# afiaka87/clip-guided-diffusion

Hardware: AMD Instinct MI355X
Metric: diffusion steps/sec (UNet+CLIP+grad) at 256x256 cutn=16 (higher is better)
Workload: dtype bf16x3 (split-bf16 MFMA, fp32 accumulate, fp32 storage); 1 GPU; BASELINE configs[1]: 256x256 class-cond UNet (554M), respace 250, cutn 16, batch 1/GPU, CLIP ViT-B/32, cgs 1000 tv 150 range 50, randomize_class, p_sample; global_batch=1, world_size_checked=1, collectives=none (single process)

## Files before the change

### clip-guided-diffusion_amd/csrc/capi.hip

```cpp
#include "../../include/cgd_mi355x.h"
#include "common.h"
#include "guidance.h"
#include "kernels.h"
#include "mfma_stage.h"

#define S(stream) ((hipStream_t)(stream))

extern "C" {

const char* cgd_version(void) { return "cgd_mi355x 0.1 (gfx950)"; }

int cgd_ctx_create(cgd_ctx** out, int device) {
  if (!out) return -3;
  cgd_ctx* ctx = new cgd_ctx();
  ctx->device = device;
  int prev = -1;
  (void)hipGetDevice(&prev);
  if (hipSetDevice(device) != hipSuccess) {
    delete ctx;
    return -1;
  }
  struct Restore {
    int d;
    ~Restore() {
      if (d >= 0) (void)hipSetDevice(d);
    }
  } restore{prev};
  hipDeviceProp_t prop;
  if (hipGetDeviceProperties(&prop, device) == hipSuccess) {
    ctx->num_cu = prop.multiProcessorCount;
    if (std::string(prop.gcnArchName).find("gfx950") == std::string::npos) {
      fprintf(stderr, "cgd_mi355x: device %d is %s, this library is built for gfx950 only\n", device, prop.gcnArchName);
      delete ctx;
      return -4;
    }
  }
  if (const char* e = getenv("CGD_DEFER")) ctx->defer_mode = atoi(e);
  if (const char* e = getenv("CGD_HGEMM_VAR")) ctx->hgemm_var = atoi(e);
  if (const char* e = getenv("CGD_HGEMM_EPI")) ctx->hgemm_epi = atoi(e);
  if (const char* e = getenv("CGD_TILE_ORDER")) ctx->tile_order = atoi(e);
  if (const char* e = getenv("CGD_FUSE_GN")) sscanf(e, "%d,%d,%d,%d", &ctx->fuse_gn, &ctx->fuse_gn_max_m, &ctx->fuse_gn_min_m, &ctx->fuse_gn_skip_m);
  if (const char* e = getenv("CGD_FUSE_ACT")) ctx->fuse_act = atoi(e);
  if (const char* e = getenv("CGD_HCONV_W8")) ctx->hconv_w8 = atoi(e);
  if (const char* e = getenv("CGD_ATTN_X3")) ctx->attn_x3 = atoi(e);
  if (const char* e = getenv("CGD_ATTN_FLASH")) ctx->attn_flash = atoi(e);
  int wino_env_mode = -1;
  if (const char* e = getenv("CGD_WINO")) sscanf(e, "%d,%d", &wino_env_mode, &ctx->wino_min_m);
  if (const char* e = getenv("CGD_THIN")) ctx->thin_direct = atoi(e);
  if (const char* e = getenv("CGD_GEMV")) ctx->gemv_mode = atoi(e);
  if (const char* e = getenv("CGD_WINO_NC")) ctx->wino_nc = atoi(e);
  ctx->wino_nc_default = ctx->wino_nc;
  if (wino_env_mode >= 0) cgd_apply_wino_mode(ctx, wino_env_mode);
  if (const char* e = getenv("CGD_GN_EPI")) ctx->gn_epi = atoi(e);
  if (const char* e = getenv("CGD_HGEMM_KG")) ctx->hgemm_kg = atoi(e) < 0 || atoi(e) > 2 ? 1 : atoi(e);
  if (const char* e = getenv("CGD_HGEMM_TM96")) ctx->hgemm_tm96 = atoi(e);
  if (const char* e = getenv("CGD_NT")) ctx->weight_nt = atoi(e);
  if (const char* e = getenv("CGD_KGEMM")) sscanf(e, "%d,%d,%d,%d,%d", &ctx->kgemm_mode, &ctx->kgemm_max_m, &ctx->kgemm_var, &ctx->kgemm_big_m, &ctx->kgemm_big_n);
  if (const char* e = getenv("CGD_EMBED_FUSE")) ctx->embed_fuse = atoi(e);
  if (const char* e = getenv("CGD_KCONV")) sscanf(e, "%d,%d,%d,%d,%d,%d,%d", &ctx->kconv_mode, &ctx->kconv_max_m, &ctx->kconv_min_chunks, &ctx->kconv_tw8, &ctx->kconv_slots, &ctx->kconv_ring, &ctx->kconv_th16);
  if (const char* e = getenv("CGD_HCONV_SPLIT")) sscanf(e, "%d,%d", &ctx->hconv_slots, &ctx->hconv_min_chunks);
  if (ctx->kconv_min_chunks < 1) ctx->kconv_min_chunks = 1;
  if (ctx->hconv_min_chunks < 1) ctx->hconv_min_chunks = 1;
  if (const char* e = getenv("CGD_HCONV_SMALL")) sscanf(e, "%d,%d,%d", &ctx->hconv_small_m, &ctx->hconv_small_slots, &ctx->hconv_small_min_chunks);
  ctx->ws_bytes = (size_t)256 << 20;
  if (hipMalloc((void**)&ctx->ws, ctx->ws_bytes) != hipSuccess) {
    delete ctx;
    return -1;
  }
  *out = ctx;
  return 0;
}

void cgd_ctx_destroy(cgd_ctx* ctx) {
  if (!ctx) return;
  {
  DeviceScope dev_scope(ctx);
  if (ctx->ws) (void)hipFree(ctx->ws);
  cgd_frag_cache_clear(ctx);
  cgd_chanstats_clear(ctx);
  if (ctx->frag_tmp) (void)hipFree(ctx->frag_tmp);
  for (ProfRec& r : ctx->prof_recs) {
    (void)hipEventDestroy(r.a);
    (void)hipEventDestroy(r.b);
  }
  for (hipEvent_t e : ctx->prof_pool) (void)hipEventDestroy(e);
  }
  delete ctx;
}

const char* cgd_last_error(cgd_ctx* ctx) { return ctx ? ctx->err.c_str() : "null context"; }

#define CGD_NEED_CTX(ctx)   \
  if (!(ctx)) return -3;    \
  DeviceScope dev_scope__(ctx)

int cgd_set_precision(cgd_ctx* ctx, int mode) {
  CGD_NEED_CTX(ctx);
  if (mode < 0 || mode > 2) CGD_FAIL(ctx, "precision mode must be 0 (f32), 1 (bf16x3) or 2 (bf16)");
  ctx->precision = mode;
  return 0;
}
int cgd_get_precision(cgd_ctx* ctx) { return ctx ? ctx->precision : -3; }
int64_t cgd_ctx_device_allocs(cgd_ctx* ctx) { return ctx ? (int64_t)ctx->device_allocs : -3; }

int cgd_set_tiles(cgd_ctx* ctx, int large, int small) {
  CGD_NEED_CTX(ctx);
  ctx->tile_huge = large >= 1000000 ? large / 1000000 : ctx->tile_huge;
  ctx->tile_large = large % 1000000;
  ctx->tile_small = small;
  return 0;
}

int cgd_set_hgemm(cgd_ctx* ctx, int mode, int min_m, int min_chunks) {
  CGD_NEED_CTX(ctx);
  ctx->hgemm_mode = mode;
  if (min_m > 0) ctx->hgemm_min_m = min_m;
  if (min_chunks > 0) ctx->hgemm_min_chunks = min_chunks;
  return 0;
}

int cgd_profile(cgd_ctx* ctx, int enable) {
  CGD_NEED_CTX(ctx);
  ctx->prof_on = enable != 0;
  return 0;
}

int cgd_profile_read(cgd_ctx* ctx, double* out) {
  CGD_NEED_CTX(ctx);
  if (!out) CGD_FAIL(ctx, "cgd_profile_read: out is null");
  CGD_HIP(ctx, hipDeviceSynchronize());
  CGD_TRY(cgd_prof_fold(ctx, 0));
  for (int k = 0; k < CGD_PROF_KINDS; ++k) {
    out[3 * k + 0] = ctx->prof_ms[k];
    out[3 * k + 1] = ctx->prof_flops[k];
    out[3 * k + 2] = ctx->prof_n[k];
    ctx->prof_ms[k] = ctx->prof_flops[k] = ctx->prof_n[k] = 0.0;
  }
  return 0;
}

int cgd_profile_kinds(void) { return CGD_PROF_KINDS; }

int cgd_launch_counts(unsigned long long* out2) {
  if (!out2) return -3;
  out2[0] = g_cgd_launches.load(std::memory_order_relaxed);
  out2[1] = g_cgd_reduces.load(std::memory_order_relaxed);
  return 0;
}
}

int cgd_prof_fold(cgd_ctx* ctx, size_t keep_last) {
  CGD_NEED_CTX(ctx);
  if (ctx->prof_recs.size() <= keep_last) return 0;
  const size_t n = ctx->prof_recs.size() - keep_last;
  for (size_t i = 0; i < n; ++i) {
    ProfRec& r = ctx->prof_recs[i];
    float t = 0.f;
    CGD_HIP(ctx, hipEventSynchronize(r.b));
    CGD_HIP(ctx, hipEventElapsedTime(&t, r.a, r.b));
    ctx->prof_ms[r.kind] += t;
    ctx->prof_flops[r.kind] += r.flops;
    ctx->prof_n[r.kind] += 1.0;
    ctx->prof_pool.push_back(r.a);
    ctx->prof_pool.push_back(r.b);
  }
  ctx->prof_recs.erase(ctx->prof_recs.begin(), ctx->prof_recs.begin() + n);
  return 0;
}

int cgd_prof_begin(cgd_ctx* ctx, ProfRec* pr, int kind, double work, hipStream_t s) {
  pr->live = false;
  if (!ctx->prof_on) return 0;
  if (ctx->prof_recs.size() >= 3072) CGD_TRY(cgd_prof_fold(ctx, 1024));
  for (hipEvent_t* e : {&pr->a, &pr->b}) {
    if (!ctx->prof_pool.empty()) {
      *e = ctx->prof_pool.back();
      ctx->prof_pool.pop_back();
    } else {
      CGD_HIP(ctx, hipEventCreate(e));
    }
  }
  pr->flops = work;
  pr->kind = kind;
  pr->live = true;
  CGD_HIP(ctx, hipEventRecord(pr->a, s));
  return 0;
}
int cgd_prof_stamp(cgd_ctx* ctx, ProfRec* pr, hipStream_t s) {
  if (pr->live) CGD_HIP(ctx, hipEventRecord(pr->b, s));
  return 0;
}
void cgd_prof_push(cgd_ctx* ctx, ProfRec* pr) {
  if (pr->live) ctx->prof_recs.push_back(*pr);
  pr->live = false;
}

// ... 195 lines not shown
  GemmParams p;
  p.A = A; p.lda = lda; p.B = Wt; p.ldb = ldw; p.C = dx; p.ldc = lddx;
  p.M = Bn * HW; p.N = N; p.K = K; p.force_tile = 513; p.no_split = 1;
  p.gnf_x = x; p.gnf_ldx = ldx; p.gnf_dz = dz; p.gnf_lddz = lddz; p.gnf_add = add; p.gnf_ldadd = ldadd;
  p.gnf_coef = coef; p.gnf_bcoef = bcoef; p.gnf_hw = HW;
  return p;
}
int cgd_op_gemm_gn_bwd_accepts(int precision, int lda, int ldw, int lddx, int ldx, int lddz, int ldadd, int x_misalign, int Bn, int HW, int N, int K) {
  if (Bn <= 0 || HW <= 0 || (long)Bn * HW > 0x7fffffffL) return 0;
  cgd_ctx ctx;
  ctx.precision = precision;
  float* const dummy = (float*)(uintptr_t)4096;
  const float* xs = (const float*)((uintptr_t)4096 + (uintptr_t)x_misalign);
  return cgd_gemm_fuses_gnb(&ctx, gemm_gn_bwd_params(dummy, lda, dummy, ldw, dummy, lddx, xs, ldx, dummy, lddz, ldadd ? dummy : nullptr, ldadd, dummy, dummy,
                                                     Bn, HW, N, K)) ? 1 : 0;
}
int cgd_op_gemm_gn_bwd(cgd_ctx* ctx, const float* A, int lda, const float* Wt, int ldw, float* dx, int lddx, const float* x, int ldx,
                       const float* dz, int lddz, const float* add, int ldadd, const float* coef, const float* bcoef, int Bn, int HW, int N, int K,
                       void* stream) {
  CGD_NEED_CTX(ctx);
  if (Bn <= 0 || HW <= 0 || (long)Bn * HW > 0x7fffffffL) CGD_FAIL(ctx, "cgd_op_gemm_gn_bwd: bad sample count / rows per sample");
  const GemmParams p = gemm_gn_bwd_params(A, lda, Wt, ldw, dx, lddx, x, ldx, dz, lddz, add, ldadd, coef, bcoef, Bn, HW, N, K);
  if (!x || !dz || !coef || !bcoef) CGD_FAIL(ctx, "cgd_op_gemm_gn_bwd: x, dz, coef and bcoef are required");
  if (!cgd_gemm_fuses_gnb(ctx, p))
    CGD_FAIL(ctx, "cgd_op_gemm_gn_bwd: needs a bf16x3 context, K a multiple of 64, N of 32, row strides multiples of 4, 16-byte aligned operands and "
                  "samples of a multiple of 128 rows (or one sample)");
  return cgd_launch_gemm(ctx, p, S(stream));
}
int cgd_op_pack_conv3x3_frag(cgd_ctx* ctx, const float* w, float* out, int Co, int Ci, int dgrad, void* stream) {
  CGD_NEED_CTX(ctx);
  return cgd_pack_conv3x3_frag(ctx, w, out, Co, Ci, dgrad, S(stream));
}
int cgd_op_pack_conv3x3_wino(cgd_ctx* ctx, const float* w, float* out, int Co, int Ci, int dgrad, void* stream) {
  CGD_NEED_CTX(ctx);
  return cgd_pack_conv3x3_wino(ctx, w, out, Co, Ci, dgrad, S(stream));
}
int cgd_op_conv3x3_wino(cgd_ctx* ctx, const float* x, int ldx, const float* w_wino, float* y, int ldy, const float* bias, const float* R,
                        int ldr, const float* gn_ab, int Bn, int H, int W, int Cin, int Cout, int ups, void* stream) {
  CGD_NEED_CTX(ctx);
  GemmParams p;
  p.Bwk = w_wino;
  p.bwk_prec = ctx->precision;
  p.A = x; p.lda = ldx; p.B = x ; p.ldb = 9 * Cin; p.C = y; p.ldc = ldy;
  p.bias = bias; p.R = R; p.ldr = ldr; p.gn_ab = gn_ab;
  p.M = Bn * H * W; p.N = Cout; p.conv = 1; p.H = H; p.W = W; p.Cin = Cin; p.ups = ups; p.force_tile = 515;
  return cgd_launch_gemm(ctx, p, S(stream));
}
int cgd_op_conv3x3_wino_ex(cgd_ctx* ctx, const float* x, int ldx, const float* w_wino, float* y, int ldy, const float* bias, const float* R,
                           int ldr, const float* gn_ab, int Bn, int H, int W, int Cin, int Cout, int ups, int stats, const float* gnb_x,
                           int gnb_ldx, const float* gnb_scratch, void* stream) {
  CGD_NEED_CTX(ctx);
  GemmParams p;
  p.Bwk = w_wino;
  p.bwk_prec = ctx->precision;
  p.A = x; p.lda = ldx; p.B = x ; p.ldb = 9 * Cin; p.C = y; p.ldc = ldy;
  p.bias = bias; p.R = R; p.ldr = ldr; p.gn_ab = gn_ab;
  p.M = Bn * H * W; p.N = Cout; p.conv = 1; p.H = H; p.W = W; p.Cin = Cin; p.ups = ups; p.force_tile = 515;
  p.stats = stats;
  if (gnb_x && gnb_scratch) {
    p.gnb_x = gnb_x; p.gnb_ldx = gnb_ldx; p.gnb_coef = cgd_gn_coef(gnb_scratch, Bn, H * W, Cout); p.gnb_act = 1;
  }
  return cgd_launch_gemm(ctx, p, S(stream));
}
}
namespace {
__global__ __launch_bounds__(256) void mfma_peak_kernel(float* out, int iters) {
  cgd_f32x16 acc[4];
  for (int a = 0; a < 4; ++a)
    for (int e = 0; e < 16; ++e) acc[a][e] = 0.f;
  cgd_bf16x8 x, y;
  for (int e = 0; e < 8; ++e) {
    x[e] = (__bf16)(float)((threadIdx.x * 7 + e) % 13 - 6);
    y[e] = (__bf16)(0.001f * (float)((threadIdx.x * 3 + e) % 11 - 5));
  }
  for (int it = 0; it < iters; ++it) {
#pragma unroll
    for (int r = 0; r < 3; ++r)
#pragma unroll
      for (int a = 0; a < 4; ++a) acc[a] = __builtin_amdgcn_mfma_f32_32x32x16_bf16(x, y, acc[a], 0, 0, 0);
  }
  float s = 0.f;
  for (int a = 0; a < 4; ++a)
    for (int e = 0; e < 16; ++e) s += acc[a][e];
  if (s == 12345.678f) out[blockIdx.x * blockDim.x + threadIdx.x] = s;
}
}
extern "C" {
int cgd_op_mfma_peak(cgd_ctx* ctx, int iters, double* flop_out, void* stream) {
  CGD_NEED_CTX(ctx);
  if (iters <= 0) CGD_FAIL(ctx, "cgd_op_mfma_peak: iters must be positive");
  const int blocks = ctx->num_cu;
  if (flop_out) *flop_out = 2.0 * 32 * 32 * 16 * 12.0 * iters * blocks * 4;
  CGD_LAUNCH(mfma_peak_kernel, dim3(blocks), dim3(256), 0, S(stream), ctx->ws, iters);
  CGD_HIP(ctx, hipGetLastError());
  return 0;
}
int cgd_op_new_pass(cgd_ctx* ctx) {
  CGD_NEED_CTX(ctx);
  ++ctx->stats_serial;
  return 0;
}
int64_t cgd_op_gn_stats_offset(int B, int HW, int C) { return (int64_t)cgd_gn_stats_offset(B, HW, C); }
int64_t cgd_op_gn_record_merges(cgd_ctx* ctx) { return ctx ? (int64_t)ctx->gn_record_merges : -3; }
int cgd_op_gn_records(cgd_ctx* ctx, const float* y, int ldy, int64_t rows, int C, int kind, float* out, int64_t cap, int* pixels, void* stream) {
  CGD_NEED_CTX(ctx);
  if (!out || !pixels) return -3;
  *pixels = 0;
  ChanSrc cs;
  if (!(cgd_chanstats_find(ctx, y, ldy, (long)rows, C, S(stream), &cs, kind) && cs.n0 == C)) return 0;
  const int64_t n = rows / cs.c0 * C * 2;
  if (n > cap) CGD_FAIL(ctx, "cgd_op_gn_records: out is too small");
  CGD_HIP(ctx, hipMemcpyAsync(out, cs.p0, (size_t)n * sizeof(float), hipMemcpyDeviceToDevice, S(stream)));
  *pixels = cs.c0;
  return 0;
}
int cgd_set_wino(cgd_ctx* ctx, int mode, int min_m) {
  CGD_NEED_CTX(ctx);
  if (mode < 0 || (mode > 3 && mode != 5)) CGD_FAIL(ctx, "cgd_set_wino: mode must be 0, 1, 2, 3 or 5");
  cgd_apply_wino_mode(ctx, mode);
  if (min_m > 0) ctx->wino_min_m = min_m;
  return 0;
}
int cgd_set_hconv(cgd_ctx* ctx, int mode, int min_m) {
  CGD_NEED_CTX(ctx);
  ctx->hconv_mode = mode & 15;
  ctx->hconv_var = mode >> 4;
  ctx->hconv_min_m = min_m;
  return 0;
}
int cgd_op_conv3x3(cgd_ctx* ctx, const float* x, int ldx, const float* w, const float* w_frag, float* y, int ldy, const float* bias,
                   const float* R, int ldr, int Bn, int H, int W, int Cin, int Cout, int ups, int force_tile, int splitk, void* stream) {
  CGD_NEED_CTX(ctx);
  GemmParams p;
  p.Bpk = w_frag;
  p.A = x; p.lda = ldx; p.B = w; p.ldb = 9 * Cin; p.C = y; p.ldc = ldy; p.bias = bias; p.R = R; p.ldr = ldr;
  p.M = Bn * H * W; p.N = Cout; p.conv = 1; p.H = H; p.W = W; p.Cin = Cin; p.ups = ups; p.force_tile = force_tile; p.splitk = splitk;
  return cgd_launch_gemm(ctx, p, S(stream));
}
int cgd_op_conv3x3_ex(cgd_ctx* ctx, const float* x, int ldx, const float* w, const float* w_frag, float* y, int ldy, const float* bias,
                      const float* R, int ldr, const float* gn_ab, int Bn, int H, int W, int Cin, int Cout, int ups, int force_tile, int splitk,
                      int defer, int stats, const float* gnb_x, int gnb_ldx, const float* gnb_scratch, void* stream) {
  CGD_NEED_CTX(ctx);
  GemmParams p;
  p.Bpk = w_frag;
  p.A = x; p.lda = ldx; p.B = w; p.ldb = 9 * Cin; p.C = y; p.ldc = ldy; p.bias = bias; p.R = R; p.ldr = ldr; p.gn_ab = gn_ab;
  p.M = Bn * H * W; p.N = Cout; p.conv = 1; p.H = H; p.W = W; p.Cin = Cin; p.ups = ups; p.force_tile = force_tile; p.splitk = splitk;
  p.defer = defer;
  p.stats = stats;
  if (gnb_x && gnb_scratch) {
    p.gnb_x = gnb_x; p.gnb_ldx = gnb_ldx; p.gnb_coef = cgd_gn_coef(gnb_scratch, Bn, H * W, Cout); p.gnb_act = 1;
  }
  return cgd_launch_gemm(ctx, p, S(stream));
}
int cgd_op_conv_in(cgd_ctx* ctx, const float* x, const float* w, const float* bias, float* y, int Bn, int H, int W, int Cin, int Cout,
                   void* stream) {
  CGD_NEED_CTX(ctx);
  return cgd_launch_conv_in(ctx, x, w, bias, y, Bn, H, W, Cin, Cout, S(stream));
}
int cgd_op_sr_stem(cgd_ctx* ctx, const float* x, const float* low, int B_low, int h, int w, const float* wpacked, const float* bias, float* y,
                   int ldy, int B, int H, int W, int Cout, void* stream) {
  CGD_NEED_CTX(ctx);
  return cgd_launch_sr_stem(ctx, x, low, B_low, h, w, wpacked, bias, y, ldy, B, H, W, Cout, S(stream));
}
int cgd_op_conv_thin_out(cgd_ctx* ctx, const float* x, int ldx, const float* w, const float* bias, float* y, int Bn, int H, int W,
                         int Cin, int Cout, void* stream) {
  CGD_NEED_CTX(ctx);
  return cgd_launch_conv_thin_out(ctx, x, ldx, w, bias, y, Bn, H, W, Cin, Cout, S(stream));
}
int64_t cgd_op_gn_scratch_floats(int B, int HW, int C) { return (int64_t)cgd_gn_scratch_floats(B, HW, C); }
int cgd_op_gn_fwd(cgd_ctx* ctx, const float* x, int ldx, float* y, int ldy, int B, int HW, int C, const float* gamma, const float* beta,
                  const float* film, int act, float eps, float* scratch, void* stream) {
  CGD_NEED_CTX(ctx);
  return cgd_launch_gn_fwd(ctx, x, ldx, y, ldy, B, HW, C, gamma, beta, film, 2 * C, act, eps, scratch, S(stream));
}
int cgd_op_gn_bwd(cgd_ctx* ctx, const float* x, int ldx, const float* dz, int lddz, float* dx, int lddx, const float* add, int ldadd,
                  int B, int HW, int C, int act, float* scratch, void* stream) {
  CGD_NEED_CTX(ctx);
  return cgd_launch_gn_bwd(ctx, x, ldx, dz, lddz, dx, lddx, add, ldadd, B, HW, C, act, scratch, S(stream));
}
int cgd_op_ln_fwd(cgd_ctx* ctx, const float* x, float* y, int rows, int C, const float* gamma, const float* beta, float eps, float* stats,
                  void* stream) {
  CGD_NEED_CTX(ctx);
  return cgd_launch_ln_fwd(ctx, x, C, y, C, rows, C, gamma, beta, eps, stats, S(stream));
}
int cgd_op_ln_bwd(cgd_ctx* ctx, const float* x, const float* dy, float* dx, int rows, int C, const float* gamma, const float* stats,
                  void* stream) {
  CGD_NEED_CTX(ctx);
  return cgd_launch_ln_bwd(ctx, x, C, dy, C, dx, C, nullptr, 0, rows, C, gamma, stats, S(stream));
}
int cgd_op_pool2x2(cgd_ctx* ctx, const float* in, float* out, int B, int Ho, int Wo, int C, float scale, void* stream) {
  CGD_NEED_CTX(ctx);
  return cgd_launch_pool2x2(ctx, in, C, out, C, nullptr, 0, B, Ho, Wo, C, scale, S(stream));
}
int cgd_op_upsample2x(cgd_ctx* ctx, const float* in, float* out, int B, int Ho, int Wo, int C, float scale, void* stream) {
  CGD_NEED_CTX(ctx);
  return cgd_launch_upsample2x(ctx, in, C, out, C, nullptr, 0, B, Ho, Wo, C, scale, S(stream));
}
int cgd_op_act(cgd_ctx* ctx, const float* x, const float* dy, float* out, int64_t n, int act, void* stream) {
  CGD_NEED_CTX(ctx);
  if (dy) return cgd_launch_act_bwd(ctx, x, dy, out, n, act, S(stream));
  return cgd_launch_act_fwd(ctx, x, out, n, act, S(stream));
}
int64_t cgd_op_attn_buf_floats(int nb, int heads, int T, int d, int which) {
  const int64_t Tp = attn_tp(T), C = (int64_t)heads * d;
  switch (which) {
    case 0: return (int64_t)nb * 3 * C * Tp;
    case 4: return (int64_t)nb * C * Tp;
    default: return (int64_t)nb * heads * T * Tp;
  }
}
int cgd_op_attn_fwd(cgd_ctx* ctx, const float* qkv, float* out, int nb, int heads, int T, int d, int legacy, float* bufs[5],
                    void* stream) {
  CGD_NEED_CTX(ctx);
  AttnShape sh{nb, heads, T, d, heads * d, legacy};
  AttnBufs bf{bufs[0], bufs[1], bufs[2], bufs[3], bufs[4]};
  return cgd_attn_fwd(ctx, sh, qkv, 3 * heads * d, out, heads * d, bf, S(stream));
}
int cgd_op_attn_fwd_causal(cgd_ctx* ctx, const float* qkv, float* out, int nb, int heads, int T, int d, float* bufs[5], void* stream) {
  CGD_NEED_CTX(ctx);
  AttnShape sh{nb, heads, T, d, heads * d, 0, 1};
  AttnBufs bf{bufs[0], bufs[1], bufs[2], bufs[3], bufs[4]};
  return cgd_attn_fwd(ctx, sh, qkv, 3 * heads * d, out, heads * d, bf, S(stream));
}
int cgd_op_attn_bwd(cgd_ctx* ctx, const float* qkv, const float* dout, float* dqkv, int nb, int heads, int T, int d, int legacy,
                    float* bufs[5], void* stream) {
  CGD_NEED_CTX(ctx);
  AttnShape sh{nb, heads, T, d, heads * d, legacy};
  AttnBufs bf{bufs[0], bufs[1], bufs[2], bufs[3], bufs[4]};
  return cgd_attn_bwd(ctx, sh, qkv, 3 * heads * d, dout, heads * d, dqkv, 3 * heads * d, bf, S(stream));
}
}

void cgd_apply_wino_mode(cgd_ctx* ctx, int mode) {
  if (mode < 0 || (mode > 3 && mode != 5)) mode = 1;
  ctx->wino_mode = mode == 5 ? 3 : mode;
  ctx->wino_nc = mode == 5 ? 3 : ctx->wino_nc_default;
}
```

### clip-guided-diffusion_amd/csrc/common.h

```cpp
#pragma once
#include <hip/hip_runtime.h>
#include <stdint.h>
#include <stdio.h>
#include <atomic>
#include <string>
#include <utility>
#include <vector>

inline std::atomic<unsigned long long> g_cgd_launches{0}, g_cgd_reduces{0};
#define CGD_LAUNCH(...)                                          \
  do {                                                           \
    g_cgd_launches.fetch_add(1, std::memory_order_relaxed);      \
    hipLaunchKernelGGL(__VA_ARGS__);                             \
  } while (0)

enum { CGD_PREC_F32 = 0, CGD_PREC_BF16X3 = 1, CGD_PREC_BF16 = 2 };

enum { CGD_PROF_GEMM = 0, CGD_PROF_HCONV = 1, CGD_PROF_GN = 2, CGD_PROF_WCONV = 3, CGD_PROF_KCONV = 4, CGD_PROF_WCONV_GNB = 5, CGD_PROF_KINDS = 6 };

struct ProfRec {
  hipEvent_t a = nullptr, b = nullptr;
  double flops = 0.0;
  int kind = 0;
  bool live = false;
};

struct SplitSrc {
  const float* ws = nullptr;
  const float* bias = nullptr;
  const float* R = nullptr;
  long stride = 0;
  int n = 0;
  int N = 0, ldr = 0;
  float alpha = 1.f;
};
struct PendingReduce {
  bool valid = false;
  SplitSrc src;
  float* C = nullptr;
  int ldc = 0, M = 0;
  hipStream_t stream = nullptr;
};

struct ChanStatsEntry {
  const float* C = nullptr;
  int ldc = 0, N = 0;
  long M = 0;
  float* buf = nullptr;
  size_t cap = 0;
  hipStream_t stream = nullptr;
  unsigned long long serial = 0;
  int kind = 0;
  int cnt = 128;
};
struct ChanSrc {
  const float* p0 = nullptr;
  const float* p1 = nullptr;
  int n0 = 0, n1 = 0;
  int c0 = 128, c1 = 128;
};

struct FragEntry {
  const float* w;
  int N, K, ldw;
  void* packed;
};

struct cgd_ctx {
  int device = 0;
  int precision = CGD_PREC_BF16X3;
  std::string err;
  float* ws = nullptr;
  size_t ws_bytes = 0;
  int num_cu = 256;
  int tile_huge = 1256, tile_large = 128, tile_small = 64;
  int hconv_var = 0;
  int hconv_small_m = 0, hconv_small_slots = 512, hconv_small_min_chunks = 2;
  int hconv_slots = 0, hconv_min_chunks = 4;
  int hconv_w8 = 0;
  int hconv_mode = 1, hconv_min_m = 256;
  int embed_fuse = 1;
  int gemv_mode = 1;
  int thin_direct = 1;
  int kconv_tw8 = 1;
  int kconv_th16 = 0;
  int kconv_ring = 2;
  int kconv_slots = 0;
  int kconv_mode = 1, kconv_max_m = 1024, kconv_min_chunks = 4;
  int wino_mode = 1, wino_min_m = 16384;
  int wino_nc_default = 0;
  int wino_nc = 0;
  int attn_x3 = 1;
  int attn_flash = 3;
  int fuse_act = 1;
  int fuse_gn_skip_m = 0;
  int fuse_gn_max_m = 1 << 30, fuse_gn_min_m = 4096;
  int fuse_gn = 1;
  int tile_order = 0;
  int hgemm_epi = 1;
  int hgemm_kg = 1;
  int weight_nt = 0;
  int kgemm_var = 0;
  int kgemm_big_m = 0, kgemm_big_n = 0;
  int kgemm_mode = 2, kgemm_max_m = 256;
  int hgemm_tm96 = 1;
  int hgemm_var = 1;
  int hgemm_mode = 1, hgemm_min_m = 64, hgemm_min_chunks = 4;
  PendingReduce pending;
  int defer_mode = 2;
  std::vector<ChanStatsEntry> chanstats;
  std::vector<float*> chanstats_retired;
  unsigned long long stats_serial = 1;
  unsigned long long device_allocs = 0;
  unsigned long long gn_record_merges = 0;
  bool last_wconv_bstat = false;
  int gn_epi = 3;
  std::vector<std::pair<const float*, int>> attn_fwd_path;
  std::vector<FragEntry> frag_cache;
  void* frag_tmp = nullptr;
  size_t frag_tmp_bytes = 0;
  bool prof_on = false;
  std::vector<ProfRec> prof_recs;
  std::vector<hipEvent_t> prof_pool;
  double prof_ms[CGD_PROF_KINDS] = {}, prof_flops[CGD_PROF_KINDS] = {}, prof_n[CGD_PROF_KINDS] = {};
};

struct ExactScope {
  cgd_ctx* ctx;
  int saved;
  explicit ExactScope(cgd_ctx* c) : ctx(c), saved(c->precision) { c->precision = CGD_PREC_F32; }
  ~ExactScope() { ctx->precision = saved; }
};

struct DeviceScope {
  int prev = -1;
  bool switched = false;
  explicit DeviceScope(const cgd_ctx* c) {
    if (c && hipGetDevice(&prev) == hipSuccess && prev != c->device) switched = hipSetDevice(c->device) == hipSuccess;
  }
  ~DeviceScope() {
    if (switched) (void)hipSetDevice(prev);
  }
};

int cgd_prof_fold(cgd_ctx* ctx, size_t keep_last);
int cgd_prof_begin(cgd_ctx* ctx, ProfRec* pr, int kind, double work, hipStream_t s);
int cgd_prof_stamp(cgd_ctx* ctx, ProfRec* pr, hipStream_t s);
void cgd_prof_push(cgd_ctx* ctx, ProfRec* pr);

#define CGD_HIP(ctx, expr)                                                                   \
  do {                                                                                       \
    hipError_t e__ = (expr);                                                                 \
    if (e__ != hipSuccess) {                                                                 \
      (ctx)->err = std::string(#expr) + ": " + hipGetErrorString(e__) + " @" + __FILE__ + ":" + \
                   std::to_string(__LINE__);                                                 \
      return -1;                                                                             \
    }                                                                                        \
  } while (0)

#define CGD_FAIL(ctx, msg)        \
  do {                            \
    (ctx)->err = (msg);           \
    return -2;                    \
  } while (0)

#define CGD_TRY(expr)             \
  do {                            \
    int r__ = (expr);             \
    if (r__ != 0) return r__;     \
  } while (0)

static inline int cdiv(long a, long b) { return (int)((a + b - 1) / b); }
static inline int grid_for(long n, int cap = 1024) {
  const int g = cdiv(n, 256);
  return g < cap ? g : cap;
}

struct GemmParams {
  const float* A = nullptr;
  const float* B = nullptr;
  float* C = nullptr;
  const float* bias = nullptr;
  const float* R = nullptr;
  int M = 0, N = 0, K = 0;
  int lda = 0, ldb = 0, ldc = 0, ldr = 0;
  int nbatch = 1, bdiv = 1;
  long sA1 = 0, sA2 = 0, sB1 = 0, sB2 = 0, sC1 = 0, sC2 = 0, sR1 = 0, sR2 = 0;
  float alpha = 1.f;
  int conv = 0, H = 0, W = 0, Cin = 0, ups = 0;
  int splitk = 1;
  int no_split = 0;
  float* ws = nullptr;
  int force_tile = 0;
  int weight = 0;
  const void* Bpk = nullptr;
  const void* Bwk = nullptr;
  int bwk_prec = CGD_PREC_BF16X3;
  float* act_out = nullptr;
  const float* act_in = nullptr;
  int ld_act = 0, act = 0;
  int skip_group = 0;
  const float* gn_ab = nullptr;
  const float* gnb_x = nullptr;
  const float* gnb_coef = nullptr;
  int gnb_ldx = 0, gnb_act = 0;
  int stats = 0;
  int a_mode = 0;
  const float* a_t = nullptr;
  const float* a_freqs = nullptr;
  const float* a_table = nullptr;
  const int64_t* a_idx = nullptr;
  const float* gnf_x = nullptr;
  const float* gnf_dz = nullptr;
  const float* gnf_add = nullptr;
  const float* gnf_coef = nullptr;
  const float* gnf_bcoef = nullptr;
  int gnf_ldx = 0, gnf_lddz = 0, gnf_ldadd = 0, gnf_hw = 0;
  int defer = 0;
};

float* cgd_chanstats_register(cgd_ctx* ctx, const float* C, int ldc, int N, long M, hipStream_t s, int kind = 0, int cnt = 128);
bool cgd_chanstats_find(cgd_ctx* ctx, const float* x, int ldx, long M, int Cn, hipStream_t s, ChanSrc* out, int kind = 0);
void cgd_chanstats_clear(cgd_ctx* ctx);
void cgd_chanstats_invalidate(cgd_ctx* ctx, const float* C, long rows, int ld, int cols);
bool cgd_gn_merges_records(int HW);
void cgd_apply_wino_mode(cgd_ctx* ctx, int mode);

int cgd_flush_pending(cgd_ctx* ctx, hipStream_t s);
bool cgd_take_pending(cgd_ctx* ctx, const float* x, long rows, int cols, int ldx, hipStream_t s, SplitSrc* out);
static inline int cgd_sync_pending(cgd_ctx* ctx, hipStream_t s) { return ctx->pending.valid ? cgd_flush_pending(ctx, s) : 0; }

size_t cgd_hconv_packed_floats(int Co, int Ci);
int cgd_pack_conv3x3_frag(cgd_ctx* ctx, const float* w , float* out, int Co, int Ci, int dgrad, hipStream_t s);
bool cgd_hconv_supported(const cgd_ctx* ctx, const GemmParams& p);
int cgd_hconv_tile_m(const cgd_ctx* ctx, const GemmParams& p);
long cgd_hconv_tiles_m(const cgd_ctx* ctx, const GemmParams& p);
int cgd_launch_hconv(cgd_ctx* ctx, const GemmParams& p, hipStream_t s);

size_t cgd_wconv_packed_floats(int Co, int Ci);
int cgd_pack_conv3x3_wino(cgd_ctx* ctx, const float* w , float* out, int Co, int Ci, int dgrad, hipStream_t s);
bool cgd_wconv_supported(const cgd_ctx* ctx, const GemmParams& p);
int cgd_wconv_nb(const cgd_ctx* ctx, const GemmParams& p);
int cgd_wconv_nc(const cgd_ctx* ctx, const GemmParams& p);
long cgd_wconv_tiles_m(const cgd_ctx* ctx, const GemmParams& p);
int cgd_launch_wconv(cgd_ctx* ctx, const GemmParams& p, hipStream_t s);

bool cgd_kconv_supported(const cgd_ctx* ctx, const GemmParams& p);
long cgd_kconv_tiles_m(const cgd_ctx* ctx, const GemmParams& p);
int cgd_kconv_tw(const cgd_ctx* ctx, const GemmParams& p);
int cgd_kconv_th(const cgd_ctx* ctx, const GemmParams& p);
int cgd_launch_kconv(cgd_ctx* ctx, const GemmParams& p, hipStream_t s);

bool cgd_hgemm_supported(const cgd_ctx* ctx, const GemmParams& p);
int cgd_hgemm_tile_m(const cgd_ctx* ctx, const GemmParams& p);
int cgd_hgemm_tiles(const cgd_ctx* ctx, const GemmParams& p);
int cgd_hgemm_chunks(const GemmParams& p);
int cgd_launch_hgemm(cgd_ctx* ctx, const GemmParams& p, hipStream_t s);
void cgd_frag_cache_clear(cgd_ctx* ctx);
bool cgd_kgemm_supported(const cgd_ctx* ctx, const GemmParams& p);
bool cgd_kgemm_capable(const cgd_ctx* ctx, const GemmParams& p);
void cgd_frag_cache_evict(cgd_ctx* ctx, const float* w);
int cgd_kgemm_tiles(const cgd_ctx* ctx, const GemmParams& p);
int cgd_launch_kgemm(cgd_ctx* ctx, const GemmParams& p, hipStream_t s);

int cgd_launch_gemm(cgd_ctx* ctx, GemmParams p, hipStream_t s);
bool cgd_conv_uses_hconv(cgd_ctx* ctx, GemmParams p);
bool cgd_gemm_fuses_act(cgd_ctx* ctx, GemmParams p);
bool cgd_gemm_fuses_gnb(cgd_ctx* ctx, GemmParams p);
bool cgd_conv_takes_gnb(cgd_ctx* ctx, GemmParams p);
bool cgd_wconv_takes_gnb(const cgd_ctx* ctx, const GemmParams& g);
bool cgd_hconv_takes_gnb(const cgd_ctx* ctx, const GemmParams& g);
bool cgd_gemm_is_gemv(cgd_ctx* ctx, GemmParams p);

int cgd_launch_conv_in(cgd_ctx* ctx, const float* x_nchw, const float* w , const float* bias,
                       float* y_nhwc, int Bn, int H, int W, int Cin, int Cout, hipStream_t s, int ldy = 0 );
int cgd_launch_conv_thin_out(cgd_ctx* ctx, const float* x_nhwc, int ldx, const float* w , const float* bias,
                             float* y_nchw, int Bn, int H, int W, int Cin, int Cout, hipStream_t s);
int cgd_launch_sr_stem(cgd_ctx* ctx, const float* x_nchw, const float* low , int B_low, int lh, int lw,
                       const float* w , const float* bias, float* y_nhwc, int ldy , int Bn, int H,
                       int W, int Cout, hipStream_t s);
```

### clip-guided-diffusion_amd/csrc/hconv.hip

```cpp
#include "common.h"
#include "mfma_stage.h"

namespace {

constexpr int HB_M = 256, HB_N = 128, HPH = 40;

struct HConvParams {
  const float* A;
  const uint4* Bp;
  float* C;
  const float* bias;
  const float* R;
  float* ws;
  int lda, ldc, ldr;
  int M, N, H, W, Cin, ups, splitk;
  float alpha;
  const float* gn;
  float* stat;
  float* bstat;
  const float* bx;
  const float* bcoef;
  int ldbx, bact;
  int nmajor;
};

constexpr int PW2 = 18;
constexpr int HRS = 768;
constexpr int NPASS2 = 6;


template <int MODE, int TH, int NJ, bool GN>
__global__ __launch_bounds__(TH == 4 ? 256 : TH * 32) void hconv2_kernel(const float* __restrict__ Ag, const uint4* __restrict__ Bg, float* Cg,
                                                         const float* __restrict__ biasg, const float* Rg, float* __restrict__ wsg,
                                                         const float* __restrict__ gng, const HConvParams p) {
  constexpr int NPL = MODE == 1 ? 2 : 1;
  constexpr int NP2 = (TH + 2) * PW2;
  constexpr int PLANE = (TH + 2) * HRS;
  constexpr int NI = TH == 4 ? 2 : 4 / NJ;
  constexpr int NT = TH == 4 ? 256 : TH * 32;
  constexpr int RPP = NT / 8;
  constexpr int NPASS = TH == 4 ? 4 : NPASS2;
  static_assert(TH != 4 || NJ == 1, "the 4-row tile runs 64 pixels x 32 channels per wavefront");
  static_assert(NPASS * RPP >= NP2, "staging passes must cover the patch");
  __shared__ __attribute__((aligned(16))) __bf16 lds[2 * NPL * PLANE];
  const int tid = threadIdx.x, lane = tid & 63, wave = tid >> 6;
  const int wm = NJ == 2 ? wave >> 1 : wave >> 2, wn = NJ == 2 ? wave & 1 : wave & 3;
  const int l31 = lane & 31, hh = lane >> 5;

  const int ntn = (p.N + HB_N - 1) / HB_N;
  int bid = blockIdx.x;
  {
    const int nt = gridDim.x, q = nt >> 3, r = nt & 7, xcd = bid & 7, idx = bid >> 3;
    bid = (xcd < r ? xcd * (q + 1) : r * (q + 1) + (xcd - r) * q) + idx;
  }
  const int ntm = gridDim.x / ntn;
  const int mt = p.nmajor ? bid % ntm : bid / ntn, n0 = (p.nmajor ? bid / ntm : bid % ntn) * HB_N;
  const int tpr = (p.W + 15) >> 4, tpi = (p.H / TH) * tpr;
  const int img = mt / tpi, trem = mt - img * tpi;
  const int y0 = (trem / tpr) * TH, x0 = (trem % tpr) << 4;
  const int HW = p.H * p.W;
  const int Hs = p.ups ? (p.H >> 1) : p.H, Ws = p.ups ? (p.W >> 1) : p.W;
  const float* __restrict__ Aimg = Ag + (long)img * Hs * Ws * p.lda;

  const int c4 = tid & 7;
  int poff[NPASS], soff[NPASS];
#pragma unroll
  for (int j = 0; j < NPASS; ++j) {
    const int prow = (tid >> 3) + RPP * j;
    poff[j] = -2;
    soff[j] = PW2 * HPH + c4 * 4;
    if (prow < NP2) {
      const int py = prow / PW2, px = prow - py * PW2;
      soff[j] = py * HRS + px * HPH + c4 * 4;
      int yy = y0 + py - 1, xx = x0 + px - 1;
      const bool inb = (unsigned)yy < (unsigned)p.H && (unsigned)xx < (unsigned)p.W;
      if (p.ups) {
        yy >>= 1;
        xx >>= 1;
      }
      poff[j] = inb ? (yy * Ws + xx) * p.lda + c4 * 4 : -1;
    }
  }
  int poffb[NPASS];
#pragma unroll
  for (int j = 0; j < NPASS; ++j) poffb[j] = poff[j] >= 0 ? poff[j] * 4 : CGD_OOB;
  int fro[NI];
  long mrow[NI];
#pragma unroll
  for (int i = 0; i < NI; ++i) {
    const int pix = wm * (NI * 32) + i * 32 + l31;
    const int ty = pix >> 4, tx = pix & 15;
    fro[i] = ty * HRS + tx * HPH + hh * 8;
    mrow[i] = x0 + tx < p.W ? (long)img * HW + (long)(y0 + ty) * p.W + x0 + tx : -1L;
  }

  const int nchunk = p.Cin >> 5;
  int c0 = 0, c1 = nchunk;
  if (p.splitk > 1) {
    const int per = (nchunk + p.splitk - 1) / p.splitk;
    c0 = blockIdx.z * per;
    c1 = min(nchunk, c0 + per);
  }
  const int nb0 = (n0 >> 5) + wn * NJ;
  const int nbN = p.N >> 5;
  const long bstride_nb = (long)nchunk * 9 * 4 * 64;
  const int nbc = nb0 < nbN ? nb0 : nbN - 1;
  (void)nbc;
  const int nb0_s = (n0 >> 5) + __builtin_amdgcn_readfirstlane(wn) * NJ;
  const uint4* __restrict__ Bwb = Bg + (long)(nb0_s < nbN ? nb0_s : nbN - 1) * bstride_nb;
  const int bj1_b = (nb0_s + 1 < nbN) ? (int)(bstride_nb * 16) : 0;
  (void)bj1_b;

  cgd_f32x16 acc[NI][NJ];
#pragma unroll
  for (int i = 0; i < NI; ++i)
#pragma unroll
    for (int j = 0; j < NJ; ++j)
#pragma unroll
      for (int e = 0; e < 16; ++e) acc[i][j][e] = 0.f;

  constexpr bool SPLITQ = !(GN && NJ == 2 && TH == 8);
  cgd_f32x4 pr[NPASS];
  cgd_f32x4 ga[GN ? 2 : 1];
  const cgd_f32x4 z4 = cgd_f32x4{0.f, 0.f, 0.f, 0.f};
  const float* __restrict__ gnimg = GN ? gng + ((long)img * p.Cin + c4 * 4) * 2 : nullptr;

#define PATCH_LOAD2(CH, WANT)                                                                                      \
  {                                                                                                                \
    if constexpr (GN) {                                                                                            \
      const int cg_ = (WANT) < 0 ? (CH) : (CH) - 1;                                                                \
      ga[0] = *(const cgd_f32x4*)(gnimg + cg_ * 64);                                                               \
      ga[1] = *(const cgd_f32x4*)(gnimg + cg_ * 64 + 4);                                                           \
    }                                                                                                              \
    _Pragma("unroll") for (int j = 0; j < NPASS; ++j)                                                             \
        pr[j] = __builtin_bit_cast(cgd_f32x4, cgd_buf_load16_if(Aimg, 0x80000000u, (WANT), poffb[j], (CH) * 128)); \
  }
#define PATCH_STORE2(DSTB, J0, J1)                                                                                                            \
  {                                                                                                                                           \
    _Pragma("unroll") for (int j = J0; j < J1; ++j) {                                                                                         \
      cgd_f32x4 v = pr[j];                                                                                                                    \
      if constexpr (GN)                                                                                                                       \
        v = cgd_f32x4{cgd_silu_affine(v.x, ga[0].x, ga[0].y), cgd_silu_affine(v.y, ga[0].z, ga[0].w), cgd_silu_affine(v.z, ga[1].x, ga[1].y), \
                  cgd_silu_affine(v.w, ga[1].z, ga[1].w)};                                                                                    \
      if constexpr (GN) v = poff[j] >= 0 ? v : z4;                           \
      if constexpr (MODE == 1 && SPLITQ) {                                                                                                    \
        cgd_bf16x4 hi, lo;                                                                                                                    \
        cgd_split_quad(v, hi, lo);                                                                                                            \
        *(cgd_bf16x4*)&(DSTB)[soff[j]] = hi;                                                                                                  \
        *(cgd_bf16x4*)&(DSTB)[PLANE + soff[j]] = lo;                                                                                          \
      } else {                                                                                                                                \
        const cgd_bf16x4 hi = cgd_to_bf16x4(v);                                                                                               \
        *(cgd_bf16x4*)&(DSTB)[soff[j]] = hi;                                                                                                  \
        if constexpr (MODE == 1) *(cgd_bf16x4*)&(DSTB)[PLANE + soff[j]] = cgd_to_bf16x4(cgd_residual4(v, hi));                                \
      }                                                                                                                                       \
    }                                                                                                                                         \
  }
#define A_LOAD2(DST, SRCB, TAP, KS)                                                          \
  {                                                                                          \
    constexpr int o_ = ((TAP) / 3) * HRS + ((TAP) % 3) * HPH + (KS) * 16;                    \
    _Pragma("unroll") for (int i = 0; i < NI; ++i) {                                         \
      DST[i][0] = *(const cgd_bf16x8*)&(SRCB)[fro[i] + o_];                                  \
      if constexpr (MODE == 1) DST[i][1] = *(const cgd_bf16x8*)&(SRCB)[PLANE + fro[i] + o_]; \
    }                                                                                        \
  }
#define B_LOAD2(DST, BASE, WANT, TAP, KS)                                                                                                         \
  {                                                                                                                                               \
    const int so_ = ((BASE) * (9 * 4 * 64) + ((TAP) * 4 + (KS) * 2) * 64) * 16;                                                                   \
    DST[0][0] = __builtin_bit_cast(uint4, cgd_buf_load16_if(Bwb, 0xffffffffu, (WANT), lane * 16, so_));                                           \
    if constexpr (MODE == 1) DST[0][1] = __builtin_bit_cast(uint4, cgd_buf_load16_if(Bwb, 0xffffffffu, (WANT), lane * 16 + 1024, so_));           \
    if constexpr (NJ == 2) {                                                                                                                      \
      DST[1][0] = __builtin_bit_cast(uint4, cgd_buf_load16_if(Bwb, 0xffffffffu, (WANT), lane * 16, so_ + bj1_b));                                 \
      if constexpr (MODE == 1) DST[1][1] = __builtin_bit_cast(uint4, cgd_buf_load16_if(Bwb, 0xffffffffu, (WANT), lane * 16 + 1024, so_ + bj1_b)); \
    }                                                                                                                                             \
  }
#define MFMA12(AQ, BQ)                                                                                                                 \
  {                                                                                                                                    \
    if constexpr (MODE == 1) {                                                                                                         \
      _Pragma("unroll") for (int i = 0; i < NI; ++i) _Pragma("unroll") for (int j = 0; j < NJ; ++j)                                    \
          acc[i][j] = __builtin_amdgcn_mfma_f32_32x32x16_bf16(__builtin_bit_cast(cgd_bf16x8, BQ[j][0]), AQ[i][1], acc[i][j], 0, 0, 0); \
      _Pragma("unroll") for (int i = 0; i < NI; ++i) _Pragma("unroll") for (int j = 0; j < NJ; ++j)                                    \
          acc[i][j] = __builtin_amdgcn_mfma_f32_32x32x16_bf16(__builtin_bit_cast(cgd_bf16x8, BQ[j][1]), AQ[i][0], acc[i][j], 0, 0, 0); \
    }                                                                                                                                  \
    _Pragma("unroll") for (int i = 0; i < NI; ++i) _Pragma("unroll") for (int j = 0; j < NJ; ++j)                                      \
        acc[i][j] = __builtin_amdgcn_mfma_f32_32x32x16_bf16(__builtin_bit_cast(cgd_bf16x8, BQ[j][0]), AQ[i][0], acc[i][j], 0, 0, 0);   \
  }

  constexpr int RING = TH == 4 ? 9 : (TH == 8 || NJ == 1) ? 6 : 3, DIST = RING - 1;
  cgd_bf16x8 af[2][NI][NPL];
  uint4 bq[RING][NJ][NPL];
  if (c0 < c1) {
    PATCH_LOAD2(c0, -1);
#pragma unroll
    for (int q = 0; q < DIST; ++q) B_LOAD2(bq[q], c0, -1, q >> 1, q & 1);
    PATCH_STORE2(lds, 0, NPASS);
  }
  __syncthreads();
  for (int c = c0; c < c1; ++c) {
    const bool more = c + 1 < c1;
    const __bf16* cur = lds + ((c - c0) & 1) * (NPL * PLANE);
    __bf16* nxt = lds + (((c - c0) & 1) ^ 1) * (NPL * PLANE);
    const int want = c + 1 - c1;
    PATCH_LOAD2(c + 1, want);
    (void)more;
    A_LOAD2(af[0], cur, 0, 0);
#pragma unroll
    for (int q = 0; q < 18; ++q) {
      if (q + 1 < 18) {
        switch (q + 1) {
#define CASE_A(Q) case Q: A_LOAD2(af[(Q) & 1], cur, (Q) >> 1, (Q) & 1); break;
          CASE_A(1) CASE_A(2) CASE_A(3) CASE_A(4) CASE_A(5) CASE_A(6) CASE_A(7) CASE_A(8) CASE_A(9)
          CASE_A(10) CASE_A(11) CASE_A(12) CASE_A(13) CASE_A(14) CASE_A(15) CASE_A(16) CASE_A(17)
#undef CASE_A
        }
      }
      {
        const int q2 = (q + DIST) % 18;
        if (q + DIST < 18) { B_LOAD2(bq[(q + DIST) % RING], c, -1, q2 >> 1, q2 & 1); }
        else { B_LOAD2(bq[(q + DIST) % RING], c + 1, want, q2 >> 1, q2 & 1); }
      }
      MFMA12(af[q & 1], bq[q % RING]);
      if (q >= 6 && q < 6 + NPASS) PATCH_STORE2(nxt, q - 6, q - 5);
#pragma unroll
      for (int r = 0; r < (TH == 4 ? 6 : 12); ++r) {
        __builtin_amdgcn_sched_group_barrier(0x008, 1, 0);
        if constexpr (TH == 4) {
          if (r < 4) __builtin_amdgcn_sched_group_barrier(0x100, 1, 0);
          else __builtin_amdgcn_sched_group_barrier(0x020, 1, 0);
          __builtin_amdgcn_sched_group_barrier(0x002, 3, 0);
        } else if constexpr (NJ == 2) {
          if (r % 3 == 0) __builtin_amdgcn_sched_group_barrier(0x100, 1, 0);
          if (r % 3 == 1) __builtin_amdgcn_sched_group_barrier(0x020, 1, 0);
        } else {
          if (r % 3 != 2) __builtin_amdgcn_sched_group_barrier(0x100, 1, 0);
          if (r % 6 == 2) __builtin_amdgcn_sched_group_barrier(0x020, 1, 0);
        }
        __builtin_amdgcn_sched_group_barrier(0x002, 3, 0);
        if (r % 3 == 2) __builtin_amdgcn_sched_group_barrier(0x200, 1, 0);
      }
      __builtin_amdgcn_sched_barrier(0);
    }
    __syncthreads();
  }
#undef PATCH_LOAD2
#undef PATCH_STORE2
#undef A_LOAD2
#undef B_LOAD2
#undef MFMA12

  if (p.splitk > 1) {
    float* __restrict__ ws = wsg + (long)blockIdx.z * p.M * p.N;
#pragma unroll
    for (int i = 0; i < NI; ++i)
#pragma unroll
      for (int j = 0; j < NJ; ++j) {
        const int cb0 = (nb0 + j) * 32;
        if (cb0 < p.N && mrow[i] >= 0) {
#pragma unroll
          for (int g = 0; g < 4; ++g)
            *(cgd_f32x4*)&ws[mrow[i] * p.N + cb0 + 8 * g + 4 * hh] =
                cgd_f32x4{acc[i][j][4 * g], acc[i][j][4 * g + 1], acc[i][j][4 * g + 2], acc[i][j][4 * g + 3]};
        }
      }
    return;
  }
  if constexpr (TH == 4) {
    const int cb0 = nb0 * 32;
    if (cb0 >= p.N) return;
    cgd_f32x4 o[NI][4];
#pragma unroll
    for (int i = 0; i < NI; ++i) {
      cgd_f32x4 rv[4];
      if (Rg && mrow[i] >= 0) {
#pragma unroll
        for (int g = 0; g < 4; ++g) rv[g] = *(const cgd_f32x4*)&Rg[mrow[i] * p.ldr + cb0 + 8 * g + 4 * hh];
      }
#pragma unroll
      for (int g = 0; g < 4; ++g) {
        const int col = cb0 + 8 * g + 4 * hh;
        o[i][g] = cgd_f32x4{acc[i][0][4 * g], acc[i][0][4 * g + 1], acc[i][0][4 * g + 2], acc[i][0][4 * g + 3]} * p.alpha;
        if (biasg) o[i][g] += cgd_f32x4{biasg[col], biasg[col + 1], biasg[col + 2], biasg[col + 3]};
        if (Rg && mrow[i] >= 0) o[i][g] += rv[g];
        if (mrow[i] >= 0) *(cgd_f32x4*)&Cg[mrow[i] * p.ldc + col] = o[i][g];
      }
    }
    if (p.stat) {
#pragma unroll
      for (int g = 0; g < 4; ++g) {
        cgd_f32x4 kk, s1 = z4, s2 = z4;
#pragma unroll
        for (int e = 0; e < 4; ++e) kk[e] = __shfl(o[0][g][e], lane & 32, 64);
#pragma unroll
        for (int i = 0; i < NI; ++i) {
          const cgd_f32x4 d = o[i][g] - kk;
          s1 += d;
          s2 += d * d;
        }
#pragma unroll
        for (int off = 1; off < 32; off <<= 1)
#pragma unroll
          for (int e = 0; e < 4; ++e) {
            s1[e] += __shfl_xor(s1[e], off, 64);
            s2[e] += __shfl_xor(s2[e], off, 64);
          }
        if (l31 == 0) {
          float* so = p.stat + ((long)mt * p.N + cb0 + 8 * g + 4 * hh) * 2;
          const cgd_f32x4 mean = kk + s1 * (1.f / 64.f), m2 = s2 - s1 * s1 * (1.f / 64.f);
          *(cgd_f32x4*)so = cgd_f32x4{mean[0], m2[0], mean[1], m2[1]};
          *(cgd_f32x4*)(so + 4) = cgd_f32x4{mean[2], m2[2], mean[3], m2[3]};
        }
      }
    }
    if (p.bstat) {
#pragma unroll
      for (int g = 0; g < 4; ++g) {
        const int col = cb0 + 8 * g + 4 * hh;
        cgd_f32x4 cfa, cfb, cfg_, cfm, q1 = z4, q2 = z4;
#pragma unroll
        for (int e = 0; e < 4; ++e) {
          const cgd_f32x4 c_ = *(const cgd_f32x4*)(p.bcoef + ((long)img * p.N + col + e) * 4);
          cfa[e] = c_[0]; cfb[e] = c_[1]; cfg_[e] = c_[2]; cfm[e] = c_[3];
        }
#pragma unroll
        for (int i = 0; i < NI; ++i) {
          const cgd_f32x4 xv = *(const cgd_f32x4*)&p.bx[mrow[i] * p.ldbx + col];
          cgd_f32x4 d = o[i][g];
          if (p.bact) {
            const cgd_f32x4 uu = xv * cfa + cfb;
            cgd_f32x4 sg;
#pragma unroll
            for (int e = 0; e < 4; ++e) sg[e] = cgd_sigmoid_rcp(uu[e]);
            d *= sg * (1.f + uu * (1.f - sg));
          }
          q1 += d;
          q2 += d * (xv - cfm);
        }
#pragma unroll
        for (int off = 1; off < 32; off <<= 1)
#pragma unroll
          for (int e = 0; e < 4; ++e) {
            q1[e] += __shfl_xor(q1[e], off, 64);
            q2[e] += __shfl_xor(q2[e], off, 64);
          }
        if (l31 == 0) {
          float* so = p.bstat + ((long)mt * p.N + col) * 2;
          *(cgd_f32x4*)so = cgd_f32x4{cfg_[0] * q1[0], cfg_[0] * q2[0], cfg_[1] * q1[1], cfg_[1] * q2[1]};
          *(cgd_f32x4*)(so + 4) = cgd_f32x4{cfg_[2] * q1[2], cfg_[2] * q2[2], cfg_[3] * q1[3], cfg_[3] * q2[3]};
        }
      }
    }
    return;
  }
#pragma unroll
  for (int i = 0; i < NI; ++i)
#pragma unroll
    for (int j = 0; j < NJ; ++j) {
      const int cb0 = (nb0 + j) * 32;
      if (cb0 >= p.N || mrow[i] < 0) continue;
      cgd_f32x4 rv[4];
      if (Rg) {
#pragma unroll
        for (int g = 0; g < 4; ++g) rv[g] = *(const cgd_f32x4*)&Rg[mrow[i] * p.ldr + cb0 + 8 * g + 4 * hh];
      }
#pragma unroll
      for (int g = 0; g < 4; ++g) {
        const int col = cb0 + 8 * g + 4 * hh;
        cgd_f32x4 o = cgd_f32x4{acc[i][j][4 * g], acc[i][j][4 * g + 1], acc[i][j][4 * g + 2], acc[i][j][4 * g + 3]} * p.alpha;
        if (biasg) o += cgd_f32x4{biasg[col], biasg[col + 1], biasg[col + 2], biasg[col + 3]};
        if (Rg) o += rv[g];
        *(cgd_f32x4*)&Cg[mrow[i] * p.ldc + col] = o;
      }
    }
}

__global__ __launch_bounds__(256) void pack_frag_kernel(const float* __restrict__ w, __bf16* __restrict__ out, int Co, int Ci, int dgrad) {
  const int N = dgrad ? Ci : Co, K = dgrad ? Co : Ci;
  const int nchunk = K >> 5;
  const long total = (long)N * K * 9;
  for (long t = (long)blockIdx.x * blockDim.x + threadIdx.x; t < total; t += (long)gridDim.x * blockDim.x) {
    const int e = (int)(t & 7);
    long u = t >> 3;
    const int lane = (int)(u & 63);
    u >>= 6;
    const int ks = (int)(u & 1);
    u >>= 1;
    const int tap = (int)(u % 9);
    u /= 9;
    const int chunk = (int)(u % nchunk), nb = (int)(u / nchunk);
    const int n = nb * 32 + (lane & 31), k = chunk * 32 + ks * 16 + (lane >> 5) * 8 + e;
    const int ky = tap / 3, kx = tap % 3;
    const float v = dgrad ? w[(((long)k * Ci + n) * 3 + (2 - ky)) * 3 + (2 - kx)] : w[(((long)n * Ci + k) * 3 + ky) * 3 + kx];
    const __bf16 hi = (__bf16)v;
    const __bf16 lo = (__bf16)(v - (float)hi);
    const long blk = ((((long)nb * nchunk + chunk) * 9 + tap) * 2 + ks) * 2;
    out[(blk + 0) * 512 + lane * 8 + e] = hi;
    out[(blk + 1) * 512 + lane * 8 + e] = lo;
  }
}

}

size_t cgd_hconv_packed_floats(int Co, int Ci) { return (size_t)Co * Ci * 9; }

int cgd_pack_conv3x3_frag(cgd_ctx* ctx, const float* w, float* out, int Co, int Ci, int dgrad, hipStream_t s) {
  if ((Co & 31) || (Ci & 31)) CGD_FAIL(ctx, "pack_conv3x3_frag: channels must be multiples of 32");
  const long total = (long)Co * Ci * 9;
  CGD_LAUNCH(pack_frag_kernel, dim3((int)std::min<long>(cdiv(total, 256), 4096)), dim3(256), 0, s, w, (__bf16*)out, Co, Ci, dgrad);
  CGD_HIP(ctx, hipGetLastError());
  return 0;
}

bool cgd_hconv_supported(const cgd_ctx* ctx, const GemmParams& p) {
  if (!p.conv || !p.Bpk || ctx->precision == CGD_PREC_F32 || p.nbatch != 1) return false;
  if ((p.Cin & 31) || (p.N & 31) || (p.lda & 3)) return false;
  if (p.H <= 0 || p.W <= 0 || (p.H & 7) || ((p.W & 15) && p.W != 8)) return false;
  if ((p.H & 15) && ((ctx->hconv_var & 1) || ((ctx->hconv_var & 2) && p.M < 16384))) return false;
  if (p.ups && ((p.H | p.W) & 1)) return false;
  if ((p.ldc & 3) || ((uintptr_t)p.C & 15)) return false;
  if (p.R && ((p.ldr & 3) || ((uintptr_t)p.R & 15))) return false;
  if ((long)p.H * p.W * p.lda * 4 >= (1L << 31)) return false;
  return true;
}

static bool hconv_records_fwd(const cgd_ctx* ctx, const GemmParams& g) {
  return g.stats && (ctx->gn_epi & 1) && g.H > 0 && g.W > 0 && !(g.W & 15) && cgd_gn_merges_records(g.H * g.W);
}
static bool hconv_records_bwd(const cgd_ctx* ctx, const GemmParams& g) {
  return g.gnb_x && g.gnb_coef && (ctx->gn_epi & 2) && g.H > 0 && g.W > 0 && !(g.W & 15) && cgd_gn_merges_records(g.H * g.W) && !(g.gnb_ldx & 3) &&
         !((uintptr_t)g.gnb_x & 15) && !g.stats && !g.R;
}

int cgd_hconv_tile_m(const cgd_ctx* ctx, const GemmParams& p) {
  if (ctx->precision == CGD_PREC_BF16X3 && !(p.N & 127) && p.splitk <= 1 && p.H > 0 && p.W > 0 && !(p.H & 3) && p.M % (p.H * p.W) == 0) {
    if (ctx->hconv_var & 8) return 64;
    if (ctx->hconv_var == 0 && !(p.W & 15) && (hconv_records_fwd(ctx, p) || hconv_records_bwd(ctx, p))) {
      const long t64 = (long)(p.M / (p.H * p.W)) * (p.H / 4) * (p.W >> 4) * (p.N >> 7);
      if (t64 / 2 < ctx->num_cu && t64 >= ctx->num_cu) return 64;
    }
  }
  if (ctx->hconv_var & 1) return HB_M;
  if ((ctx->hconv_var & 2) && p.M < 16384) return HB_M;
  return 128;
}

bool cgd_hconv_takes_gnb(const cgd_ctx* ctx, const GemmParams& g) { return g.splitk <= 1 && cgd_hconv_tile_m(ctx, g) == 64 && hconv_records_bwd(ctx, g); }

long cgd_hconv_tiles_m(const cgd_ctx* ctx, const GemmParams& p) {
  const int th = cgd_hconv_tile_m(ctx, p) / 16;
  return (long)(p.M / (p.H * p.W)) * (p.H / th) * cdiv(p.W, 16);
}

int cgd_launch_hconv(cgd_ctx* ctx, const GemmParams& g, hipStream_t s) {
  HConvParams p;
  p.A = g.A; p.Bp = (const uint4*)g.Bpk; p.C = g.C; p.bias = g.bias; p.R = g.R; p.ws = g.ws;
  p.lda = g.lda; p.ldc = g.ldc; p.ldr = g.ldr;
  p.M = g.M; p.N = g.N; p.H = g.H; p.W = g.W; p.Cin = g.Cin; p.ups = g.ups; p.splitk = g.splitk; p.alpha = g.alpha;
  p.gn = g.gn_ab;
  p.stat = p.bstat = nullptr; p.bx = g.gnb_x; p.bcoef = g.gnb_coef; p.ldbx = g.gnb_ldx; p.bact = g.gnb_act;
  p.nmajor = (ctx->tile_order == 1 || (ctx->tile_order == 0 && 9L * g.N >= g.M)) ? 1 : 0;
  const int tm = cgd_hconv_tile_m(ctx, g);
  if (tm == 64 && g.splitk <= 1) {
    if (hconv_records_fwd(ctx, g)) p.stat = cgd_chanstats_register(ctx, g.C, g.ldc, g.N, g.M, s, 0, 64);
    if (hconv_records_bwd(ctx, g)) p.bstat = cgd_chanstats_register(ctx, g.C, g.ldc, g.N, g.M, s, 1, 64);
  }
  dim3 grid((int)cgd_hconv_tiles_m(ctx, g) * cdiv(g.N, HB_N), 1, g.splitk > 1 ? g.splitk : 1);
#define HC2_LAUNCH(M_, TH_, NJ_)                                                                                                   \
  {                                                                                                                                \
    if (p.gn)                                                                                                                      \
      CGD_LAUNCH((hconv2_kernel<M_, TH_, NJ_, true>), grid, dim3(TH_ == 4 ? 256 : TH_ * 32), 0, s, p.A, p.Bp, p.C, p.bias, p.R, p.ws, p.gn, p);  \
    else                                                                                                                           \
      CGD_LAUNCH((hconv2_kernel<M_, TH_, NJ_, false>), grid, dim3(TH_ == 4 ? 256 : TH_ * 32), 0, s, p.A, p.Bp, p.C, p.bias, p.R, p.ws, p.gn, p); \
  }
#define HC2_LAUNCH_T(M_, NJ_)  \
  {                            \
    if (tm == 128)             \
      HC2_LAUNCH(M_, 8, NJ_)   \
    else                       \
      HC2_LAUNCH(M_, 16, NJ_)  \
  }
  const bool nj1 = (ctx->hconv_var & 4) == 0;
  if (tm == 64) {
    HC2_LAUNCH(1, 4, 1)
  } else if (ctx->precision == CGD_PREC_BF16X3) {
    if (nj1) HC2_LAUNCH_T(1, 1) else HC2_LAUNCH_T(1, 2)
  } else {
    if (nj1) HC2_LAUNCH_T(2, 1) else HC2_LAUNCH_T(2, 2)
  }
#undef HC2_LAUNCH_T
#undef HC2_LAUNCH
  return 0;
}
```

### clip-guided-diffusion_amd/csrc/unet.hip

```cpp
#include <cmath>
#include <memory>

#include "../../include/cgd_mi355x.h"
#include "net.h"

namespace {

__global__ void pack_conv3x3_kernel(const float* __restrict__ w, float* __restrict__ wf, float* __restrict__ wd, int Co, int Ci) {
  const long total = (long)Co * Ci * 9;
  for (long i = (long)blockIdx.x * blockDim.x + threadIdx.x; i < total; i += (long)gridDim.x * blockDim.x) {
    const int kx = (int)(i % 3);
    long t = i / 3;
    const int ky = (int)(t % 3);
    t /= 3;
    const int ci = (int)(t % Ci), co = (int)(t / Ci);
    const float v = w[i];
    if (wf) wf[((long)co * 9 + ky * 3 + kx) * Ci + ci] = v;
    if (wd) wd[((long)ci * 9 + (2 - ky) * 3 + (2 - kx)) * Co + co] = v;
  }
}

}

int cgd_pack_conv3x3(cgd_ctx* ctx, const float* w, float* wf, float* wd, int Co, int Ci, hipStream_t s) {
  const long total = (long)Co * Ci * 9;
  CGD_LAUNCH(pack_conv3x3_kernel, dim3((int)std::min<long>(cdiv(total, 256), 4096)), dim3(256), 0, s, w, wf, wd, Co, Ci);
  CGD_HIP(ctx, hipGetLastError());
  return 0;
}

int cgd_plan_gemm(cgd_ctx* ctx, GemmParams& p, int* tile_out, int* kernel_out);

namespace {

struct UNet;

struct Module {
  TV dst;
  virtual ~Module() {}
  virtual int fwd(UNet& u, TV x, int B, int& H, int& W, TV* out, hipStream_t s) = 0;
  virtual int bwd(UNet& u, TV dout, TV* din, hipStream_t s) = 0;
};

struct ResBlock : Module {
  std::string pre;
  int cin = 0, cout = 0;
  bool up = false, down = false, skip_conv = false;
  long emb_off = 0;
  float *g1 = 0, *b1 = 0, *cw1f = 0, *cw1d = 0, *cb1 = 0, *g2 = 0, *b2 = 0, *cw2f = 0, *cw2d = 0, *cb2 = 0, *skw = 0, *skwT = 0,
        *skb = 0;
  float *cw1fp = 0, *cw1dp = 0, *cw2fp = 0, *cw2dp = 0;
  float *cw1wp = 0, *cw1wd = 0, *cw2wp = 0, *cw2wd = 0;
  int wino_prec = CGD_PREC_BF16X3;
  bool wino_ready = false;
  int B = 0, H = 0, W = 0, Ho = 0, Wo = 0;
  TV x;
  TV add_skip;
  DevBuf h1, h1p, xr, h2, h3, out, s1, s2;
  DevBuf d3, d2, d1, d1f, dx;
  int fwd(UNet& u, TV x, int B, int& H, int& W, TV* out, hipStream_t s) override;
  int bwd(UNet& u, TV dout, TV* din, hipStream_t s) override;
};

struct AttnBlock : Module {
  std::string pre;
  int C = 0, heads = 0, d = 0, legacy = 1;
  float *g = 0, *b = 0, *qkvw = 0, *qkvwT = 0, *qkvb = 0, *pw = 0, *pwT = 0, *pb = 0;
  int B = 0, T = 0;
  TV x;
  DevBuf n, qkv, a, out, sc, da, dqkv, dn, dx;
  AttnScratch att;
  int fwd(UNet& u, TV x, int B, int& H, int& W, TV* out, hipStream_t s) override;
  int bwd(UNet& u, TV dout, TV* din, hipStream_t s) override;
};

struct UNet : NetBase {
  int ensure_wino(ResBlock* rb, long pixels, hipStream_t s);
  cgd_unet_config cfg;
  bool encoder_only = false;
  int ted = 0, ch0 = 0, ch_last = 0;
  long emb_total = 0;
  std::vector<std::vector<std::unique_ptr<Module>>> in_blocks;
  std::vector<std::unique_ptr<Module>> mid;
  std::vector<std::vector<std::unique_ptr<Module>>> out_blocks;
  std::vector<int> in_chans;
  std::vector<int> in_ds;
  std::vector<ResBlock*> resblocks;
  float *stem_wf = 0, *stem_wd = 0, *head_wf = 0, *head_wd = 0;
  float *emb_w_all = 0, *emb_b_all = 0, *freqs = 0;
  int B = 0, H = 0, W = 0;
  bool have_fwd = false;
  int fwd_prec = 0;
  DevBuf temb, e1, e1s, e2, e2s, emb_all, h0, headn, head_s, dheadn, dhead;
  DevBuf emb_slot1;
  const float* emb_cur = nullptr;
  int emb_B[2] = {0, 0};
  std::vector<DevBuf> cats;
  std::vector<TV> hs;
  std::vector<std::pair<int, int>> hs_hw;
  std::vector<TV> cat_in;
  std::vector<int> cat_c1;
  std::vector<std::pair<int, int>> cat_hw;
  TV head_in;
  DevBuf low;
  int low_B = 0, low_h = 0, low_w = 0;

  int build();
  int finalize(hipStream_t s);
  int set_low_res(const float* img, int B_low, int h, int w, hipStream_t s);
  int embed(const float* t, const int64_t* y, int Bn, int slot, hipStream_t s, bool ahead = false);
  int forward(const float* x, const float* t, const int64_t* y, float* out, int B, int H, int W, hipStream_t s, int slot = -1);
  int dgrad(const float* gout, float* gx, hipStream_t s);
};

int UNet::ensure_wino(ResBlock* rb, long pixels, hipStream_t s) {
  if (rb->wino_ready && rb->wino_prec != ctx->precision) rb->wino_ready = false;
  if (!ctx->wino_mode || pixels < ctx->wino_min_m || rb->wino_ready) return 0;
  if (ctx->precision != CGD_PREC_BF16X3 && ctx->precision != CGD_PREC_F32) return 0;
  const std::string& p = rb->pre;
  if (!rb->cw1wp) CGD_TRY(alloc(&rb->cw1wp, cgd_wconv_packed_floats(rb->cout, rb->cin)));
  if (!rb->cw1wd) CGD_TRY(alloc(&rb->cw1wd, cgd_wconv_packed_floats(rb->cout, rb->cin)));
  if (!rb->cw2wp) CGD_TRY(alloc(&rb->cw2wp, cgd_wconv_packed_floats(rb->cout, rb->cout)));
  if (!rb->cw2wd) CGD_TRY(alloc(&rb->cw2wd, cgd_wconv_packed_floats(rb->cout, rb->cout)));
  CGD_TRY(cgd_pack_conv3x3_wino(ctx, P(p + ".in_layers.2.weight"), rb->cw1wp, rb->cout, rb->cin, 0, s));
  CGD_TRY(cgd_pack_conv3x3_wino(ctx, P(p + ".in_layers.2.weight"), rb->cw1wd, rb->cout, rb->cin, 1, s));
  CGD_TRY(cgd_pack_conv3x3_wino(ctx, P(p + ".out_layers.3.weight"), rb->cw2wp, rb->cout, rb->cout, 0, s));
  CGD_TRY(cgd_pack_conv3x3_wino(ctx, P(p + ".out_layers.3.weight"), rb->cw2wd, rb->cout, rb->cout, 1, s));
  rb->wino_ready = true;
  rb->wino_prec = ctx->precision;
  return 0;
}

int ResBlock::fwd(UNet& u, TV xin, int Bn, int& Hh, int& Ww, TV* o, hipStream_t s) {
  cgd_ctx* ctx = u.ctx;
  B = Bn; H = Hh; W = Ww;
  Ho = up ? 2 * H : (down ? H / 2 : H);
  Wo = up ? 2 * W : (down ? W / 2 : W);
  x = xin;
  const long npi = (long)B * H * W, npo = (long)B * Ho * Wo;
  CGD_TRY(u.ensure(s1, cgd_gn_scratch_floats(B, H * W, cin)));
  CGD_TRY(u.ensure(s2, cgd_gn_scratch_floats(B, Ho * Wo, cout)));
  CGD_TRY(u.ensure(h2, npo * cout));
  if (!dst.p) CGD_TRY(u.ensure(out, npo * cout));
  float* const outp = dst.p ? dst.p : out.p;
  const int ldo = dst.p ? dst.ld : cout;
  CGD_TRY(u.ensure_wino(this, npo, s));
  GemmParams c1;
  c1.B = cw1f; c1.Bpk = cw1fp; c1.Bwk = wino_ready ? cw1wp : nullptr; c1.bwk_prec = wino_prec; c1.ldb = 9 * cin; c1.C = h2.p; c1.ldc = cout; c1.bias = cb1;
  c1.M = (int)npo; c1.N = cout; c1.conv = 1; c1.H = Ho; c1.W = Wo; c1.Cin = cin; c1.ups = up ? 1 : 0;
  c1.defer = 1;
  c1.stats = 1;
  c1.A = x.p; c1.lda = x.ld;
  const bool fuse1 = !down && cgd_conv_uses_hconv(ctx, c1);
  const float* skip_src = x.p;
  int skip_ld = x.ld;
  if (fuse1) {
    CGD_TRY(cgd_launch_gn_fwd(ctx, x.p, x.ld, nullptr, 0, B, H * W, cin, g1, b1, nullptr, 0, 1, 1e-5f, s1.p, s));
    c1.gn_ab = cgd_gn_ab(s1.p, B, H * W, cin);
  } else {
    CGD_TRY(u.ensure(h1, npi * cin));
    CGD_TRY(cgd_launch_gn_fwd(ctx, x.p, x.ld, h1.p, cin, B, H * W, cin, g1, b1, nullptr, 0, 1, 1e-5f, s1.p, s));
    c1.A = h1.p; c1.lda = cin;
  }
  if (down) {
    CGD_TRY(u.ensure(h1p, npo * cin));
    CGD_TRY(u.ensure(xr, npo * cin));
    CGD_TRY(cgd_launch_resample2x_pair(ctx, 0, h1.p, cin, h1p.p, cin, x.p, x.ld, xr.p, cin, B, Ho, Wo, cin, 0.25f, s));
    c1.A = h1p.p; c1.lda = cin;
    skip_src = xr.p;
    skip_ld = cin;
  } else if (up) {
    CGD_TRY(u.ensure(xr, npo * cin));
    CGD_TRY(cgd_launch_upsample2x(ctx, x.p, x.ld, xr.p, cin, nullptr, 0, B, Ho, Wo, cin, 1.f, s));
    skip_src = xr.p;
    skip_ld = cin;
  }
  CGD_TRY(cgd_launch_gemm(ctx, c1, s));
  GemmParams c2;
  c2.A = h2.p; c2.lda = cout; c2.B = cw2f; c2.Bpk = cw2fp; c2.Bwk = wino_ready ? cw2wp : nullptr; c2.bwk_prec = wino_prec; c2.ldb = 9 * cout; c2.C = outp; c2.ldc = ldo; c2.bias = cb2;
  c2.M = (int)npo; c2.N = cout; c2.conv = 1; c2.H = Ho; c2.W = Wo; c2.Cin = cout;
  c2.defer = 1;
  c2.stats = 1;
  const bool fuse2 = cgd_conv_uses_hconv(ctx, c2);
  if (fuse2) {
    CGD_TRY(cgd_launch_gn_fwd(ctx, h2.p, cout, nullptr, 0, B, Ho * Wo, cout, g2, b2, u.emb_cur + emb_off, (int)u.emb_total, 1, 1e-5f,
                              s2.p, s));
    c2.gn_ab = cgd_gn_ab(s2.p, B, Ho * Wo, cout);
  } else {
    CGD_TRY(u.ensure(h3, npo * cout));
    CGD_TRY(cgd_launch_gn_fwd(ctx, h2.p, cout, h3.p, cout, B, Ho * Wo, cout, g2, b2, u.emb_cur + emb_off, (int)u.emb_total, 1, 1e-5f,
                              s2.p, s));
    c2.A = h3.p;
  }
  const float* R = skip_src;
  int ldr = skip_ld;
  if (skip_conv) {
    GemmParams sk;
    sk.A = skip_src; sk.lda = skip_ld; sk.B = skw; sk.ldb = cin; sk.C = outp; sk.ldc = ldo; sk.bias = skb;
    sk.M = (int)npo; sk.N = cout; sk.K = cin;
    sk.weight = 1;
    CGD_TRY(cgd_launch_gemm(ctx, sk, s));
    R = outp;
    ldr = ldo;
  }
  c2.R = R; c2.ldr = ldr;
  CGD_TRY(cgd_launch_gemm(ctx, c2, s));
  Hh = Ho; Ww = Wo;
  *o = TV{outp, ldo, cout};
  return 0;
}

int ResBlock::bwd(UNet& u, TV dout, TV* din, hipStream_t s) {
  cgd_ctx* ctx = u.ctx;
  const long npi = (long)B * H * W, npo = (long)B * Ho * Wo;
  CGD_TRY(u.ensure(d3, npo * cout));
  CGD_TRY(u.ensure(d2, npo * cout));
  CGD_TRY(u.ensure(d1, npo * cin));
  CGD_TRY(u.ensure(dx, npi * cin));
  GemmParams c2;
  c2.A = dout.p; c2.lda = dout.ld; c2.B = cw2d; c2.Bpk = cw2dp; c2.Bwk = wino_ready ? cw2wd : nullptr; c2.bwk_prec = wino_prec; c2.ldb = 9 * cout; c2.C = d3.p; c2.ldc = cout;
  c2.M = (int)npo; c2.N = cout; c2.conv = 1; c2.H = Ho; c2.W = Wo; c2.Cin = cout;
  c2.defer = 1;
  c2.gnb_x = h2.p; c2.gnb_ldx = cout; c2.gnb_coef = cgd_gn_coef(s2.p, B, Ho * Wo, cout); c2.gnb_act = 1;
  CGD_TRY(cgd_launch_gemm(ctx, c2, s));
  CGD_TRY(cgd_launch_gn_bwd(ctx, h2.p, cout, d3.p, cout, d2.p, cout, nullptr, 0, B, Ho * Wo, cout, 1, s2.p, s));
  const float* add = nullptr;
  int ldadd = 0;
  GemmParams sk;
  bool fuse_skip = false;
  if (down || up) {
    add = dx.p; ldadd = cin;
  } else if (skip_conv) {
    sk.A = dout.p; sk.lda = dout.ld; sk.B = skwT; sk.ldb = cout; sk.C = dx.p; sk.ldc = cin;
    sk.M = (int)npo; sk.N = cin; sk.K = cout;
    sk.weight = 1;
    GemmParams probe = sk;
    probe.gnf_x = x.p; probe.gnf_ldx = x.ld; probe.gnf_dz = d1.p; probe.gnf_lddz = cin; probe.gnf_add = add_skip.p; probe.gnf_ldadd = add_skip.ld;
    probe.gnf_coef = probe.gnf_bcoef = cgd_gn_coef(s1.p, B, H * W, cin); probe.gnf_hw = H * W;
    GemmParams c1p;
    c1p.A = d2.p; c1p.lda = cout; c1p.B = cw1d; c1p.Bpk = cw1dp; c1p.Bwk = wino_ready ? cw1wd : nullptr; c1p.bwk_prec = wino_prec; c1p.ldb = 9 * cout; c1p.C = d1.p; c1p.ldc = cin;
    c1p.M = (int)npo; c1p.N = cin; c1p.conv = 1; c1p.H = Ho; c1p.W = Wo; c1p.Cin = cout; c1p.defer = 1;
    c1p.gnb_x = x.p; c1p.gnb_ldx = x.ld; c1p.gnb_coef = cgd_gn_coef(s1.p, B, H * W, cin); c1p.gnb_act = 1;
    fuse_skip = !(H * W & 127) && cgd_gemm_fuses_gnb(ctx, probe) && cgd_conv_takes_gnb(ctx, c1p);
    if (!fuse_skip) CGD_TRY(cgd_launch_gemm(ctx, sk, s));
    add = dx.p; ldadd = cin;
  } else {
    add = dout.p; ldadd = dout.ld;
  }
  GemmParams c1;
  c1.A = d2.p; c1.lda = cout; c1.B = cw1d; c1.Bpk = cw1dp; c1.Bwk = wino_ready ? cw1wd : nullptr; c1.bwk_prec = wino_prec; c1.ldb = 9 * cout; c1.C = d1.p; c1.ldc = cin;
  c1.M = (int)npo; c1.N = cin; c1.conv = 1; c1.H = Ho; c1.W = Wo; c1.Cin = cout;
  c1.defer = (up || down) ? 0 : 1;
  if (!up && !down) {
    c1.gnb_x = x.p; c1.gnb_ldx = x.ld; c1.gnb_coef = cgd_gn_coef(s1.p, B, H * W, cin); c1.gnb_act = 1;
  }
  CGD_TRY(cgd_launch_gemm(ctx, c1, s));
  const float* dh1 = d1.p;
  if (down) {
    CGD_TRY(u.ensure(d1f, npi * cin));
    CGD_TRY(cgd_launch_resample2x_pair(ctx, 1, d1.p, cin, d1f.p, cin, dout.p, dout.ld, dx.p, cin, B, H, W, cin, 0.25f, s));
    dh1 = d1f.p;
  } else if (up) {
    CGD_TRY(u.ensure(d1f, npi * cin));
    CGD_TRY(cgd_launch_resample2x_pair(ctx, 0, d1.p, cin, d1f.p, cin, dout.p, dout.ld, dx.p, cin, B, H, W, cin, 1.f, s));
    dh1 = d1f.p;
  }
  if (fuse_skip) {
    bool done = false;
    CGD_TRY(cgd_launch_gn_bwd_skip_gemm(ctx, sk, x.p, x.ld, d1.p, cin, add_skip.p, add_skip.ld, B, H * W, cin, s1.p, s, &done));
    if (done) {
      *din = TV{dx.p, cin, cin};
      return 0;
    }
    CGD_TRY(cgd_launch_gemm(ctx, sk, s));
  }
  CGD_TRY(cgd_launch_gn_bwd(ctx, x.p, x.ld, dh1, cin, dx.p, cin, add, ldadd, B, H * W, cin, 1, s1.p, s, add_skip.p, add_skip.ld));
  *din = TV{dx.p, cin, cin};
  return 0;
}

int AttnBlock::fwd(UNet& u, TV xin, int Bn, int& H, int& W, TV* o, hipStream_t s) {
  cgd_ctx* ctx = u.ctx;
  B = Bn; T = H * W;
  x = xin;
  const long rows = (long)B * T;
  CGD_TRY(u.ensure(sc, cgd_gn_scratch_floats(B, T, C)));
  CGD_TRY(u.ensure(n, rows * C));
  CGD_TRY(u.ensure(qkv, rows * 3 * C));
  CGD_TRY(u.ensure(a, rows * C));
  if (!dst.p) CGD_TRY(u.ensure(out, rows * C));
  float* const outp = dst.p ? dst.p : out.p;
  const int ldo = dst.p ? dst.ld : C;
  CGD_TRY(cgd_launch_gn_fwd(ctx, x.p, x.ld, n.p, C, B, T, C, g, b, nullptr, 0, 0, 1e-5f, sc.p, s));
  GemmParams q;
  q.A = n.p; q.lda = C; q.B = qkvw; q.ldb = C; q.C = qkv.p; q.ldc = 3 * C; q.bias = qkvb; q.M = (int)rows; q.N = 3 * C; q.K = C;
  q.weight = 1;
  CGD_TRY(cgd_launch_gemm(ctx, q, s));
  CGD_TRY(u.attn_fwd(att, AttnShape{B, heads, T, d, C, legacy, 0}, qkv.p, 3 * C, a.p, C, s));
  GemmParams p;
  p.A = a.p; p.lda = C; p.B = pw; p.ldb = C; p.C = outp; p.ldc = ldo; p.bias = pb; p.R = x.p; p.ldr = x.ld; p.M = (int)rows; p.N = C;
  p.K = C;
  p.weight = 1;
  p.defer = 1;
  CGD_TRY(cgd_launch_gemm(ctx, p, s));
  *o = TV{outp, ldo, C};
  return 0;
}

int AttnBlock::bwd(UNet& u, TV dout, TV* din, hipStream_t s) {
  cgd_ctx* ctx = u.ctx;
  const long rows = (long)B * T;
  CGD_TRY(u.ensure(da, rows * C));
  CGD_TRY(u.ensure(dqkv, rows * 3 * C));
  CGD_TRY(u.ensure(dn, rows * C));
  CGD_TRY(u.ensure(dx, rows * C));
  GemmParams p;
  p.A = dout.p; p.lda = dout.ld; p.B = pwT; p.ldb = C; p.C = da.p; p.ldc = C; p.M = (int)rows; p.N = C; p.K = C;
  p.weight = 1;
  CGD_TRY(cgd_launch_gemm(ctx, p, s));
  CGD_TRY(u.attn_bwd(att, AttnShape{B, heads, T, d, C, legacy, 0}, qkv.p, 3 * C, da.p, C, dqkv.p, 3 * C, s));
  GemmParams q;
  q.A = dqkv.p; q.lda = 3 * C; q.B = qkvwT; q.ldb = 3 * C; q.C = dn.p; q.ldc = C; q.M = (int)rows; q.N = C; q.K = 3 * C;
  q.weight = 1;
  q.defer = 1;
  CGD_TRY(cgd_launch_gemm(ctx, q, s));
  CGD_TRY(cgd_launch_gn_bwd(ctx, x.p, x.ld, dn.p, C, dx.p, C, dout.p, dout.ld, B, T, C, 0, sc.p, s));
  *din = TV{dx.p, C, C};
  return 0;
}

int UNet::build() {
  const int mc = cfg.model_channels;
  if ((cfg.in_channels != 3 && (cfg.in_channels != 6 || encoder_only)) || (!encoder_only && cfg.out_channels != 6 && cfg.out_channels != 3))
    CGD_FAIL(ctx, "unet: in_channels must be 3 (or 6: a super-resolution UNet), out_channels 3 or 6");
  if (cfg.n_mult < 1 || cfg.n_mult > 8) CGD_FAIL(ctx, "unet: bad channel_mult");
  if (cfg.n_att < 0 || cfg.n_att > 8) CGD_FAIL(ctx, "unet: at most 8 attention resolutions");
  if (mc <= 0 || mc % 32) CGD_FAIL(ctx, "unet: model_channels must be a positive multiple of 32 (GroupNorm32)");
  if (cfg.num_res_blocks < 1) CGD_FAIL(ctx, "unet: num_res_blocks must be >= 1");
  if (cfg.image_size <= 0 || cfg.image_size % (1 << (cfg.n_mult - 1))) CGD_FAIL(ctx, "unet: image_size must be divisible by 2^(levels-1)");
  if (cfg.num_classes < 0) CGD_FAIL(ctx, "unet: num_classes must be >= 0");
  if (cfg.num_head_channels == -1 ? cfg.num_heads <= 0 : cfg.num_head_channels <= 0) CGD_FAIL(ctx, "unet: num_heads / num_head_channels");
  for (int i = 0; i < cfg.n_mult; ++i) {
    const float w = cfg.channel_mult[i] * mc;
    const int wi = (int)w;
    if (!(w > 0.f) || (float)wi != w || wi % 32) CGD_FAIL(ctx, "unet: channel_mult * model_channels must be a positive multiple of 32 at every level");
    bool att = false;
    for (int a = 0; a < cfg.n_att; ++a) att = att || cfg.attention_ds[a] == (1 << i);
    if (att && (cfg.num_head_channels == -1 ? wi % cfg.num_heads : wi % cfg.num_head_channels))
      CGD_FAIL(ctx, "unet: the width of an attention level must be divisible by the head count / head width");
  }
  ted = mc * 4;
  add_param("time_embed.0.weight", (int64_t)ted * mc);
  add_param("time_embed.0.bias", ted);
  add_param("time_embed.2.weight", (int64_t)ted * ted);
  add_param("time_embed.2.bias", ted);
  if (cfg.num_classes > 0) add_param("label_emb.weight", (int64_t)cfg.num_classes * ted);

  auto is_att = [&](int ds) {
    for (int i = 0; i < cfg.n_att; ++i)
      if (cfg.attention_ds[i] == ds) return true;
    return false;
  };
  auto make_rb = [&](const std::string& pre, int cin, int cout, bool up, bool down) {
    auto rb = std::make_unique<ResBlock>();
    rb->pre = pre; rb->cin = cin; rb->cout = cout; rb->up = up; rb->down = down; rb->skip_conv = cin != cout;
    add_param(pre + ".in_layers.0.weight", cin);
    add_param(pre + ".in_layers.0.bias", cin);
    add_param(pre + ".in_layers.2.weight", (int64_t)cout * cin * 9);
    add_param(pre + ".in_layers.2.bias", cout);
    add_param(pre + ".emb_layers.1.weight", (int64_t)2 * cout * ted);
    add_param(pre + ".emb_layers.1.bias", 2 * cout);
    add_param(pre + ".out_layers.0.weight", cout);
    add_param(pre + ".out_layers.0.bias", cout);
    add_param(pre + ".out_layers.3.weight", (int64_t)cout * cout * 9);
    add_param(pre + ".out_layers.3.bias", cout);
    if (rb->skip_conv) {
      add_param(pre + ".skip_connection.weight", (int64_t)cout * cin);
      add_param(pre + ".skip_connection.bias", cout);
    }
    rb->emb_off = emb_total;
    emb_total += 2 * cout;
    resblocks.push_back(rb.get());
    return rb;
  };
  auto make_att = [&](const std::string& pre, int C) {
    auto ab = std::make_unique<AttnBlock>();
    ab->pre = pre; ab->C = C;
    ab->heads = cfg.num_head_channels == -1 ? cfg.num_heads : C / cfg.num_head_channels;
    ab->d = C / ab->heads;
    ab->legacy = cfg.use_new_attention_order ? 0 : 1;
    add_param(pre + ".norm.weight", C);
    add_param(pre + ".norm.bias", C);
    add_param(pre + ".qkv.weight", (int64_t)3 * C * C);
    add_param(pre + ".qkv.bias", 3 * C);
    add_param(pre + ".proj_out.weight", (int64_t)C * C);
    add_param(pre + ".proj_out.bias", C);
    return ab;
  };

  int ch = ch0 = (int)(cfg.channel_mult[0] * mc);
  add_param("input_blocks.0.0.weight", (int64_t)ch * cfg.in_channels * 9);
  add_param("input_blocks.0.0.bias", ch);
  in_blocks.emplace_back();
  in_chans.push_back(ch);
  in_ds.push_back(1);
  int ds = 1, idx = 1;
  for (int level = 0; level < cfg.n_mult; ++level) {
    const int co = (int)(cfg.channel_mult[level] * mc);
    for (int r = 0; r < cfg.num_res_blocks; ++r) {
      std::vector<std::unique_ptr<Module>> blk;
      const std::string pre = "input_blocks." + std::to_string(idx);
      blk.push_back(make_rb(pre + ".0", ch, co, false, false));
      ch = co;
      if (is_att(ds)) blk.push_back(make_att(pre + ".1", ch));
      in_blocks.push_back(std::move(blk));
      in_chans.push_back(ch);
      in_ds.push_back(ds);
      ++idx;
    }
    if (level != cfg.n_mult - 1) {
      std::vector<std::unique_ptr<Module>> blk;
      blk.push_back(make_rb("input_blocks." + std::to_string(idx) + ".0", ch, ch, false, true));
      in_blocks.push_back(std::move(blk));
      in_chans.push_back(ch);
      ++idx;
      ds *= 2;
      in_ds.push_back(ds);
    }
  }
  mid.push_back(make_rb("middle_block.0", ch, ch, false, false));
  mid.push_back(make_att("middle_block.1", ch));
  mid.push_back(make_rb("middle_block.2", ch, ch, false, false));
  if (encoder_only) {
    ch_last = ch;
    return 0;
  }
  std::vector<int> chans = in_chans;
  int oidx = 0;
  for (int level = cfg.n_mult - 1; level >= 0; --level) {
    const int co = (int)(cfg.channel_mult[level] * mc);
    for (int i = 0; i <= cfg.num_res_blocks; ++i) {
      const int ich = chans.back();
      chans.pop_back();
      std::vector<std::unique_ptr<Module>> blk;
      const std::string pre = "output_blocks." + std::to_string(oidx);
      int sub = 0;
      blk.push_back(make_rb(pre + "." + std::to_string(sub++), ch + ich, co, false, false));
      ch = co;
      if (is_att(ds)) blk.push_back(make_att(pre + "." + std::to_string(sub++), ch));
      if (level && i == cfg.num_res_blocks) {
        blk.push_back(make_rb(pre + "." + std::to_string(sub++), ch, ch, true, false));
        ds /= 2;
      }
      out_blocks.push_back(std::move(blk));
      ++oidx;
    }
  }
  ch_last = ch;
  add_param("out.0.weight", ch);
  add_param("out.0.bias", ch);
  add_param("out.2.weight", (int64_t)cfg.out_channels * ch0 * 9);
  add_param("out.2.bias", cfg.out_channels);
  if (ch_last != ch0) CGD_FAIL(ctx, "unet: channel bookkeeping mismatch");
  cats.resize(out_blocks.size());
  return 0;
}

int UNet::finalize(hipStream_t s) {
  CGD_TRY(check_all_set());
  if (!emb_w_all) {
    CGD_TRY(alloc(&emb_w_all, (size_t)emb_total * ted));
    CGD_TRY(alloc(&emb_b_all, (size_t)emb_total));
  }
  for (ResBlock* rb : resblocks) {
    const std::string& p = rb->pre;
    rb->g1 = P(p + ".in_layers.0.weight"); rb->b1 = P(p + ".in_layers.0.bias");
    rb->cb1 = P(p + ".in_layers.2.bias");
    rb->g2 = P(p + ".out_layers.0.weight"); rb->b2 = P(p + ".out_layers.0.bias");
    rb->cb2 = P(p + ".out_layers.3.bias");
    if (!rb->cw1f) {
      CGD_TRY(alloc(&rb->cw1f, (size_t)rb->cout * rb->cin * 9));
      CGD_TRY(alloc(&rb->cw1d, (size_t)rb->cout * rb->cin * 9));
      CGD_TRY(alloc(&rb->cw2f, (size_t)rb->cout * rb->cout * 9));
      CGD_TRY(alloc(&rb->cw2d, (size_t)rb->cout * rb->cout * 9));
      CGD_TRY(alloc(&rb->cw1fp, (size_t)rb->cout * rb->cin * 9));
      CGD_TRY(alloc(&rb->cw1dp, (size_t)rb->cout * rb->cin * 9));
      CGD_TRY(alloc(&rb->cw2fp, (size_t)rb->cout * rb->cout * 9));
      CGD_TRY(alloc(&rb->cw2dp, (size_t)rb->cout * rb->cout * 9));
    }
    CGD_TRY(cgd_pack_conv3x3_frag(ctx, P(p + ".in_layers.2.weight"), rb->cw1fp, rb->cout, rb->cin, 0, s));
    CGD_TRY(cgd_pack_conv3x3_frag(ctx, P(p + ".in_layers.2.weight"), rb->cw1dp, rb->cout, rb->cin, 1, s));
    CGD_TRY(cgd_pack_conv3x3_frag(ctx, P(p + ".out_layers.3.weight"), rb->cw2fp, rb->cout, rb->cout, 0, s));
    CGD_TRY(cgd_pack_conv3x3_frag(ctx, P(p + ".out_layers.3.weight"), rb->cw2dp, rb->cout, rb->cout, 1, s));
    rb->wino_ready = false;
    CGD_TRY(cgd_pack_conv3x3(ctx, P(p + ".in_layers.2.weight"), rb->cw1f, rb->cw1d, rb->cout, rb->cin, s));
    CGD_TRY(cgd_pack_conv3x3(ctx, P(p + ".out_layers.3.weight"), rb->cw2f, rb->cw2d, rb->cout, rb->cout, s));
    if (rb->skip_conv) {
      rb->skw = P(p + ".skip_connection.weight");
      rb->skb = P(p + ".skip_connection.bias");
      CGD_TRY(transpose_weight(rb->skw, &rb->skwT, rb->cout, rb->cin, s));
    }
    CGD_HIP(ctx, hipMemcpyAsync(emb_w_all + rb->emb_off * ted, P(p + ".emb_layers.1.weight"), (size_t)2 * rb->cout * ted * sizeof(float),
                                hipMemcpyDeviceToDevice, s));
    CGD_HIP(ctx, hipMemcpyAsync(emb_b_all + rb->emb_off, P(p + ".emb_layers.1.bias"), (size_t)2 * rb->cout * sizeof(float),
                                hipMemcpyDeviceToDevice, s));
  }
  auto fin_att = [&](Module* m) -> int {
    AttnBlock* ab = dynamic_cast<AttnBlock*>(m);
    if (!ab) return 0;
    const std::string& p = ab->pre;
    ab->g = P(p + ".norm.weight"); ab->b = P(p + ".norm.bias");
    ab->qkvw = P(p + ".qkv.weight"); ab->qkvb = P(p + ".qkv.bias");
    ab->pw = P(p + ".proj_out.weight"); ab->pb = P(p + ".proj_out.bias");
    CGD_TRY(transpose_weight(ab->qkvw, &ab->qkvwT, 3 * ab->C, ab->C, s));
    CGD_TRY(transpose_weight(ab->pw, &ab->pwT, ab->C, ab->C, s));
    return 0;
  };
  for (auto& blk : in_blocks)
    for (auto& m : blk) CGD_TRY(fin_att(m.get()));
  for (auto& m : mid) CGD_TRY(fin_att(m.get()));
  for (auto& blk : out_blocks)
    for (auto& m : blk) CGD_TRY(fin_att(m.get()));
  if (!stem_wf) {
    CGD_TRY(alloc(&stem_wf, (size_t)ch0 * cfg.in_channels * 9));
    CGD_TRY(alloc(&stem_wd, (size_t)ch0 * cfg.in_channels * 9));
    if (!encoder_only) {
      CGD_TRY(alloc(&head_wf, (size_t)ch0 * cfg.out_channels * 9));
      CGD_TRY(alloc(&head_wd, (size_t)ch0 * cfg.out_channels * 9));
    }
  }
  CGD_TRY(cgd_pack_conv3x3(ctx, P("input_blocks.0.0.weight"), stem_wf, stem_wd, ch0, cfg.in_channels, s));
  if (!encoder_only) CGD_TRY(cgd_pack_conv3x3(ctx, P("out.2.weight"), head_wf, head_wd, cfg.out_channels, ch0, s));
  if (!freqs) {
    const int half = cfg.model_channels / 2;
    std::vector<float> f(half);
    for (int i = 0; i < half; ++i) f[i] = (float)std::exp(-std::log(10000.0) * (double)i / (double)half);
    CGD_TRY(alloc(&freqs, half));
    CGD_HIP(ctx, hipMemcpy(freqs, f.data(), half * sizeof(float), hipMemcpyHostToDevice));
  }
  CGD_HIP(ctx, hipStreamSynchronize(s));
  finalized = true;
  have_fwd = false;
  emb_B[0] = emb_B[1] = 0;
  return 0;
}

int UNet::embed(const float* t, const int64_t* y, int Bn, int slot, hipStream_t s, bool ahead) {
  if (!finalized) CGD_FAIL(ctx, "unet: finalize() has not been called after the last set_param");
  if (slot < 0 || slot > 1) CGD_FAIL(ctx, "unet: embedding slot must be 0 or 1");
  if (cfg.num_classes > 0 && !y) CGD_FAIL(ctx, "unet: class-conditional model needs y");
  const int mc = cfg.model_channels;
  DevBuf& dst = slot ? emb_slot1 : emb_all;
  CGD_TRY(ensure(temb, (size_t)Bn * mc));
  CGD_TRY(ensure(e1, (size_t)Bn * ted));
  CGD_TRY(ensure(e1s, (size_t)Bn * ted));
  CGD_TRY(ensure(e2, (size_t)Bn * ted));
  CGD_TRY(ensure(e2s, (size_t)Bn * ted));
  CGD_TRY(ensure(dst, (size_t)Bn * emb_total));
  GemmParams g1;
  g1.A = temb.p; g1.lda = mc; g1.B = P("time_embed.0.weight"); g1.ldb = mc; g1.C = e1.p; g1.ldc = ted; g1.bias = P("time_embed.0.bias");
  g1.M = Bn; g1.N = ted; g1.K = mc; g1.no_split = ahead;
  GemmParams g2;
  g2.A = e1s.p; g2.lda = ted; g2.B = P("time_embed.2.weight"); g2.ldb = ted; g2.C = e2.p; g2.ldc = ted; g2.bias = P("time_embed.2.bias");
  g2.M = Bn; g2.N = ted; g2.K = ted; g2.no_split = ahead;
  GemmParams g3;
  g3.A = e2s.p; g3.lda = ted; g3.B = emb_w_all; g3.ldb = ted; g3.C = dst.p; g3.ldc = (int)emb_total; g3.bias = emb_b_all;
  g3.M = Bn; g3.N = (int)emb_total; g3.K = ted; g3.no_split = ahead;
  if (ctx->embed_fuse && cgd_gemm_is_gemv(ctx, g1) && cgd_gemm_is_gemv(ctx, g2) && cgd_gemm_is_gemv(ctx, g3)) {
    g1.a_mode = 3; g1.a_t = t; g1.a_freqs = freqs;
    g2.A = e1.p; g2.a_mode = 1;
    g3.A = e2.p; g3.a_mode = cfg.num_classes > 0 ? 2 : 1; g3.a_table = cfg.num_classes > 0 ? P("label_emb.weight") : nullptr; g3.a_idx = y;
    CGD_TRY(cgd_launch_gemm(ctx, g1, s));
    CGD_TRY(cgd_launch_gemm(ctx, g2, s));
    CGD_TRY(cgd_launch_gemm(ctx, g3, s));
  } else {
    CGD_TRY(cgd_launch_timestep_embedding(ctx, t, freqs, temb.p, Bn, mc, s));
    CGD_TRY(cgd_launch_gemm(ctx, g1, s));
    CGD_TRY(cgd_launch_act_fwd(ctx, e1.p, e1s.p, (long)Bn * ted, 1, s));
    CGD_TRY(cgd_launch_gemm(ctx, g2, s));
    if (cfg.num_classes > 0) CGD_TRY(cgd_launch_embedding_add(ctx, P("label_emb.weight"), y, e2.p, Bn, ted, s));
    CGD_TRY(cgd_launch_act_fwd(ctx, e2.p, e2s.p, (long)Bn * ted, 1, s));
    CGD_TRY(cgd_launch_gemm(ctx, g3, s));
  }
  emb_B[slot] = Bn;
  return 0;
}

int UNet::set_low_res(const float* img, int B_low, int h, int w, hipStream_t s) {
  if (cfg.in_channels != 6) CGD_FAIL(ctx, "unet: set_low_res needs a super-resolution handle (in_channels 6); this one takes 3 channels");
  if (!img) CGD_FAIL(ctx, "unet: set_low_res: the image is required");
  if (B_low <= 0 || h <= 0 || w <= 0) CGD_FAIL(ctx, "unet: set_low_res: the image must be (B_low,3,h,w) with B_low, h, w >= 1");
  const size_t n = (size_t)B_low * 3 * h * w;
  CGD_TRY(ensure(low, n));
  CGD_HIP(ctx, hipMemcpyAsync(low.p, img, n * sizeof(float), hipMemcpyDefault, s));
  low_B = B_low; low_h = h; low_w = w;
  return 0;
}

int UNet::forward(const float* x, const float* t, const int64_t* y, float* out, int Bn, int Hh, int Ww, hipStream_t s, int slot) {
  if (!finalized) CGD_FAIL(ctx, "unet: finalize() has not been called after the last set_param");
  const int levels = cfg.n_mult - 1;
  if ((Hh % (1 << levels)) || (Ww % (1 << levels))) CGD_FAIL(ctx, "unet: H and W must be divisible by 2^(levels-1)");
  if (slot > 1) CGD_FAIL(ctx, "unet: embedding slot must be 0 or 1");
  if (cfg.in_channels == 6) {
    if (!low_B) CGD_FAIL(ctx, "unet: a super-resolution handle needs its low-resolution image before forward(): call set_low_res first");
    if (low_B != 1 && low_B != Bn)
      CGD_FAIL(ctx, "unet: the low-resolution image has batch " + std::to_string(low_B) + ", forward() has " + std::to_string(Bn) + ": it must be 1 or equal");
  }
  if (slot < 0) {
    CGD_TRY(embed(t, y, Bn, 0, s));
    slot = 0;
  } else if (emb_B[slot] != Bn) {
    CGD_FAIL(ctx, "unet: forward(slot) needs a preceding embed() of the same batch size into that slot");
  }
  emb_cur = slot ? emb_slot1.p : emb_all.p;
  B = Bn; H = Hh; W = Ww;
  have_fwd = false;
  fwd_prec = ctx->precision;
  ++ctx->stats_serial;
  const int n_in = (int)in_blocks.size();
  cat_in.assign(out_blocks.size(), TV{});
  cat_c1.assign(out_blocks.size(), 0);
  cat_hw.assign(out_blocks.size(), {0, 0});
  for (size_t k = 0; k < out_blocks.size(); ++k) {
    const int i = n_in - 1 - (int)k;
    const ResBlock* rb = static_cast<const ResBlock*>(out_blocks[k][0].get());
    const int ct = rb->cin, c1 = ct - in_chans[i];
    const int hk = H / in_ds[i], wk = W / in_ds[i];
    CGD_TRY(ensure(cats[k], (size_t)B * hk * wk * ct));
    cat_in[k] = TV{cats[k].p, ct, ct};
    cat_c1[k] = c1;
    cat_hw[k] = {hk, wk};
    Module* skip_src = i == 0 ? nullptr : in_blocks[i].back().get();
    if (skip_src) skip_src->dst = TV{cats[k].p + c1, ct, in_chans[i]};
    Module* h_src = k == 0 ? mid.back().get() : out_blocks[k - 1].back().get();
    h_src->dst = TV{cats[k].p, ct, c1};
  }
  const size_t klast = out_blocks.size() - 1;
  float* const h0p = cats[klast].p + cat_c1[klast];
  const int h0ld = cat_in[klast].ld;
  if (cfg.in_channels == 6)
    CGD_TRY(cgd_launch_sr_stem(ctx, x, low.p, low_B, low_h, low_w, stem_wf, P("input_blocks.0.0.bias"), h0p, h0ld, B, H, W, ch0, s));
  else
    CGD_TRY(cgd_launch_conv_in(ctx, x, stem_wf, P("input_blocks.0.0.bias"), h0p, B, H, W, cfg.in_channels, ch0, s, h0ld));
  hs.clear(); hs_hw.clear();
  TV h{h0p, h0ld, ch0};
  int ch = H, cw = W;
// ... 246 lines not shown
```

### clip-guided-diffusion_amd/lib.py

```python
import ctypes as C
import os
import weakref

_HERE = os.path.dirname(os.path.abspath(__file__))
LIB_PATH = os.environ.get("CGD_LIB_PATH") or os.path.join(_HERE, "libcgd_mi355x.so")

F32P = C.POINTER(C.c_float)
vp = C.c_void_p
i32 = C.c_int
i64 = C.c_int64
f32 = C.c_float


class UNetConfig(C.Structure):
    _fields_ = [
        ("image_size", i32), ("model_channels", i32), ("num_res_blocks", i32), ("n_mult", i32),
        ("channel_mult", f32 * 8), ("n_att", i32), ("attention_ds", i32 * 8), ("num_classes", i32),
        ("num_heads", i32), ("num_head_channels", i32), ("use_new_attention_order", i32),
        ("in_channels", i32), ("out_channels", i32),
    ]


class ClassifierConfig(C.Structure):
    _fields_ = [
# ... 32 lines not shown
MASK_PRED_XSTART, MASK_N_KNOWN, MASK_RENOISE = 1, 2, 4


class ReverseCoef(C.Structure):
    _fields_ = [("sqrt_recip", f32), ("sqrt_recipm1", f32), ("sqrt_ab_next", f32), ("sqrt_one_minus_ab_next", f32),
                ("inv_sqrt_one_minus_ab_next", f32)]


class Dpmpp(C.Structure):
    _fields_ = [("c_x", f32), ("c_d", f32), ("c_r", f32), ("c_n", f32)]


MANIFEST_CB = C.CFUNCTYPE(None, C.c_char_p, i64, vp)

_SIGS = {
    "cgd_unet_manifest": (i32, [C.POINTER(UNetConfig), MANIFEST_CB, vp]),
    "cgd_vit_manifest": (i32, [C.POINTER(ViTConfig), MANIFEST_CB, vp]),
    "cgd_rn_manifest": (i32, [C.POINTER(RNConfig), MANIFEST_CB, vp]),
    "cgd_text_manifest": (i32, [C.POINTER(TextConfig), MANIFEST_CB, vp]),
    "cgd_lpips_manifest": (i32, [MANIFEST_CB, vp]),
    "cgd_version": (C.c_char_p, []),
    "cgd_ctx_create": (i32, [C.POINTER(vp), i32]),
    "cgd_ctx_destroy": (None, [vp]),
    "cgd_last_error": (C.c_char_p, [vp]),
    "cgd_set_precision": (i32, [vp, i32]),
    "cgd_get_precision": (i32, [vp]),
    "cgd_ctx_device_allocs": (i64, [vp]),
    "cgd_set_tiles": (i32, [vp, i32, i32]),
    "cgd_set_hgemm": (i32, [vp, i32, i32, i32]),
    "cgd_profile": (i32, [vp, i32]),
    "cgd_profile_read": (i32, [vp, C.POINTER(C.c_double)]),
    "cgd_profile_kinds": (i32, []),
    "cgd_launch_counts": (i32, [C.POINTER(C.c_uint64)]),
    "cgd_unet_create": (i32, [vp, C.POINTER(UNetConfig), C.POINTER(vp)]),
    "cgd_unet_destroy": (None, [vp]),
    "cgd_unet_num_params": (i32, [vp]),
    "cgd_unet_param_info": (i32, [vp, i32, C.c_char_p, i32, C.POINTER(i64)]),
    "cgd_unet_set_param": (i32, [vp, C.c_char_p, vp, i64]),
    "cgd_unet_finalize": (i32, [vp]),
    "cgd_unet_forward": (i32, [vp, vp, vp, vp, vp, i32, i32, i32, vp]),
    "cgd_unet_embed": (i32, [vp, vp, vp, i32, i32, vp]),
    "cgd_unet_forward_slot": (i32, [vp, vp, i32, vp, i32, i32, i32, vp]),
    "cgd_unet_dgrad": (i32, [vp, vp, vp, vp]),
    "cgd_unet_set_low_res": (i32, [vp, vp, i32, i32, i32, vp]),
    "cgd_vit_create": (i32, [vp, C.POINTER(ViTConfig), C.POINTER(vp)]),
    "cgd_vit_destroy": (None, [vp]),
    "cgd_vit_num_params": (i32, [vp]),
    "cgd_vit_param_info": (i32, [vp, i32, C.c_char_p, i32, C.POINTER(i64)]),
    "cgd_vit_set_param": (i32, [vp, C.c_char_p, vp, i64]),
    "cgd_vit_finalize": (i32, [vp]),
    "cgd_vit_set_activation": (i32, [vp, i32]),
    "cgd_vit_forward": (i32, [vp, vp, i32, i32, vp, vp]),
    "cgd_vit_dgrad": (i32, [vp, vp, vp, vp]),
    "cgd_text_create": (i32, [vp, C.POINTER(TextConfig), C.POINTER(vp)]),
    "cgd_text_destroy": (None, [vp]),
    "cgd_text_num_params": (i32, [vp]),
    "cgd_text_param_info": (i32, [vp, i32, C.c_char_p, i32, C.POINTER(i64)]),
    "cgd_text_set_param": (i32, [vp, C.c_char_p, vp, i64]),
    "cgd_text_finalize": (i32, [vp]),
    "cgd_text_set_activation": (i32, [vp, i32]),
    "cgd_text_forward": (i32, [vp, vp, i32, vp, vp]),
    "cgd_rn_create": (i32, [vp, C.POINTER(RNConfig), C.POINTER(vp)]),
    "cgd_rn_destroy": (None, [vp]),
    "cgd_rn_num_params": (i32, [vp]),
    "cgd_rn_param_info": (i32, [vp, i32, C.c_char_p, i32, C.POINTER(i64)]),
    "cgd_rn_set_param": (i32, [vp, C.c_char_p, vp, i64]),
    "cgd_rn_finalize": (i32, [vp]),
    "cgd_rn_forward": (i32, [vp, vp, i32, vp, vp]),
    "cgd_rn_dgrad": (i32, [vp, vp, vp, vp]),
    "cgd_rn_debug_relu_count": (i32, [vp]),
    "cgd_rn_debug_relu_info": (i32, [vp, i32, C.POINTER(i64), C.POINTER(i32)]),
    "cgd_rn_debug_relu_set": (i32, [vp, i32, vp, vp]),
    "cgd_lpips_create": (i32, [vp, C.POINTER(vp)]),
    "cgd_lpips_destroy": (None, [vp]),
    "cgd_lpips_num_params": (i32, [vp]),
    "cgd_lpips_param_info": (i32, [vp, i32, C.c_char_p, i32, C.POINTER(i64)]),
    "cgd_lpips_set_param": (i32, [vp, C.c_char_p, vp, i64]),
    "cgd_lpips_finalize": (i32, [vp]),
    "cgd_lpips_set_reference": (i32, [vp, vp, i32, i32, i32, vp]),
    "cgd_lpips_loss_grad": (i32, [vp, vp, f32, vp, vp, i32, vp]),
    "cgd_lpips_debug_replay": (i32, [vp, C.POINTER(vp)]),
    "cgd_lpips_set_style": (i32, [vp, vp, i32, i32, C.POINTER(f32), vp]),
    "cgd_lpips_style_loss_grad": (i32, [vp, vp, i32, i32, i32, f32, f32, vp, vp, vp, i32, vp]),
    "cgd_op_gram": (i32, [vp, vp, i32, i32, i32, i32, f32, vp, vp]),
    "cgd_secondary_manifest": (i32, [MANIFEST_CB, vp]),
    "cgd_secondary_create": (i32, [vp, C.POINTER(vp)]),
    "cgd_secondary_destroy": (None, [vp]),
    "cgd_secondary_num_params": (i32, [vp]),
    "cgd_secondary_param_info": (i32, [vp, i32, C.c_char_p, i32, C.POINTER(i64)]),
    "cgd_secondary_set_param": (i32, [vp, C.c_char_p, vp, i64]),
    "cgd_secondary_finalize": (i32, [vp]),
    "cgd_secondary_forward": (i32, [vp, vp, vp, i32, i32, i32, vp, vp]),
    "cgd_secondary_forward_blend": (i32, [vp, vp, vp, i32, i32, i32, f32, vp, vp, vp]),
    "cgd_secondary_dgrad": (i32, [vp, vp, vp, vp]),
    "cgd_secondary_debug_replay": (i32, [vp, C.POINTER(vp)]),
    "cgd_secondary_head": (i32, [vp, vp, vp, vp, f32, vp, vp, i32, i32, i32, vp]),
    "cgd_secondary_combine": (i32, [vp, vp, vp, vp, vp, vp, vp, i32, i32, i32, f32, f32, f32, f32, f32, f32, vp]),
    "cgd_op_secondary_pack": (i32, [vp, vp, vp, vp, vp, i32, i32, i32, vp]),
    "cgd_op_bilinear_up2x": (i32, [vp, vp, i32, vp, i32, i32, i32, i32, i32, i32, vp]),
    "cgd_classifier_manifest": (i32, [C.POINTER(ClassifierConfig), MANIFEST_CB, vp]),
    "cgd_classifier_create": (i32, [vp, C.POINTER(ClassifierConfig), C.POINTER(vp)]),
    "cgd_classifier_destroy": (None, [vp]),
    "cgd_classifier_num_params": (i32, [vp]),
    "cgd_classifier_param_info": (i32, [vp, i32, C.c_char_p, i32, C.POINTER(i64)]),
    "cgd_classifier_set_param": (i32, [vp, C.c_char_p, vp, i64]),
    "cgd_classifier_finalize": (i32, [vp]),
    "cgd_classifier_forward": (i32, [vp, vp, vp, vp, vp, vp, i32, i32, i32, vp]),
    "cgd_classifier_dgrad": (i32, [vp, f32, vp, i32, vp]),
    "cgd_op_attnpool_scratch_floats": (i64, [i32, i32, i32, i32, i32]),
    "cgd_op_attnpool_fwd": (i32, [vp, vp, vp, vp, vp, vp, vp, vp, vp, vp, vp, vp, i32, i32, i32, i32, i32, vp]),
    "cgd_op_attnpool_bwd": (i32, [vp, vp, vp, vp, vp, f32, vp, vp, i32, i32, i32, i32, i32, vp]),
    "cgd_cutouts_fwd": (i32, [vp, vp, vp, vp, i32, i32, i32, i32, i32, i32, i32, vp]),
    "cgd_cutouts_bwd": (i32, [vp, vp, vp, vp, i32, i32, i32, i32, i32, i32, i32, i32, vp]),
    "cgd_cutouts_aug_fwd": (i32, [vp, vp, vp, vp, vp, vp, vp, i32, i32, i32, i32, i32, i32, i32, vp]),
    "cgd_cutouts_aug_bwd": (i32, [vp, vp, vp, vp, vp, vp, i32, i32, i32, i32, i32, i32, i32, i32, vp]),
    "cgd_cutouts_aug_scratch_floats": (i64, [i32, i32, i32, i32]),
    "cgd_op_aug_sample_map": (i32, [vp, i32, i32, vp, vp, vp]),
    "cgd_cutouts_resize_fwd": (i32, [vp, vp, vp, vp, vp, i32, i32, i32, i32, i32, i32, i32, vp]),
    "cgd_cutouts_resize_bwd": (i32, [vp, vp, vp, vp, vp, vp, i32, i32, i32, i32, i32, i32, i32, i32, vp]),
    "cgd_cutouts_resize_scratch_floats": (i64, [i32, i32, i32, i32]),
    "cgd_cutouts_resize_weights": (i32, [i32, i32, vp, vp, C.POINTER(i32)]),
    "cgd_spherical_loss": (i32, [vp, vp, vp, vp, vp, vp, i32, i32, i32, i32, f32, vp]),
    "cgd_directional_loss": (i32, [vp, vp, vp, vp, vp, vp, vp, i32, i32, i32, i32, i32, f32, i32, vp]),
    "cgd_spherical_loss_regions": (i32, [vp, vp, vp, vp, vp, vp, i32, i32, i32, i32, f32, vp, vp, vp, vp, vp, i32, i32, i32, vp]),
    "cgd_directional_loss_regions": (i32, [vp, vp, vp, vp, vp, vp, vp, i32, i32, i32, i32, i32, f32, i32, vp, vp, vp, vp, vp, i32, i32, i32, vp]),
    "cgd_op_region_coverage": (i32, [vp, vp, vp, vp, vp, vp, vp, i32, i32, i32, i32, i32, vp]),
    "cgd_pmv_blend": (i32, [vp, vp, vp, vp, vp, vp, vp, i32, i32, i32, C.POINTER(StepCoef), vp]),
    "cgd_guidance_part_blocks": (i32, [i32, i32, i32]),
    "cgd_guidance_combine": (i32, [vp, vp, vp, vp, vp, vp, vp, i32, i32, i32, C.POINTER(StepCoef), f32, f32, f32, vp]),
    "cgd_grad_finish": (i32, [vp, vp, vp, vp, vp, i32, i32, i32, vp]),
    "cgd_scalars": (i32, [vp, vp, i32, vp, vp, i32, i32, i32, i32, vp, vp]),
    "cgd_sample_update": (i32, [vp, vp, vp, vp, vp, vp, vp, vp, vp, vp, i32, i32, i32, C.POINTER(StepCoef), i32, vp]),
    "cgd_multistep_update": (i32, [vp, vp, vp, vp, vp, vp, vp, C.POINTER(vp), vp, vp, vp, i32, i32, i32, C.POINTER(StepCoef),
                                    C.POINTER(StepCoef), C.POINTER(Multistep), vp]),
    "cgd_dpmpp_update": (i32, [vp, vp, vp, vp, vp, vp, vp, vp, vp, vp, i32, i32, i32, C.POINTER(StepCoef), C.POINTER(Dpmpp), vp]),
    "cgd_abs_quantile_scratch_bytes": (i64, [i32, i64]),
    "cgd_abs_quantile_slice": (i32, []),
    "cgd_op_abs_quantile": (i32, [vp, vp, i32, i64, i64, f32, f32, f32, vp, vp, vp]),
    "cgd_dpmpp_threshold": (i32, [vp, vp, vp, vp, vp, vp, i32, i32, i32, C.POINTER(StepCoef), i64, f32, f32, f32, vp, vp, vp]),
    "cgd_dpmpp_update_thr": (i32, [vp, vp, vp, vp, vp, vp, vp, vp, vp, vp, i32, i32, i32, C.POINTER(StepCoef), C.POINTER(Dpmpp), vp]),
    "cgd_masked_merge": (i32, [vp, vp, vp, vp, vp, vp, vp, vp, i32, i32, i32, i32, i32, i32, C.POINTER(MaskCoef), vp]),
    "cgd_ilvr_scratch_floats": (C.c_long, [i32, i32, i32, i32, i32]),
    "cgd_ilvr_refine": (i32, [vp, vp, vp, vp, vp, vp, i32, i32, i32, i32, i32, f32, f32, vp]),
    "cgd_window_gather": (i32, [vp, vp, vp, C.POINTER(i32), i32, C.POINTER(i32), i32, vp, vp, i32, i32, i32, i32, i32, i32, vp]),
    "cgd_window_merge": (i32, [vp, vp, vp, C.POINTER(i32), i32, C.POINTER(i32), i32, vp, vp, i32, i32, i32, i32, i32, i32, i32, vp]),
    "cgd_ddim_reverse_update": (i32, [vp, vp, vp, vp, vp, vp, vp, i32, i32, i32, i32, C.POINTER(ReverseCoef), vp]),
    "cgd_op_gemm": (i32, [vp, vp, i32, vp, i32, vp, i32, vp, vp, i32, i32, i32, i32, f32, i32, i32, vp]),
    "cgd_op_gemm_gn_bwd_accepts": (i32, [i32] * 12),
    "cgd_op_gemm_gn_bwd": (i32, [vp, vp, i32, vp, i32, vp, i32, vp, i32, vp, i32, vp, i32, vp, vp, i32, i32, i32, i32, vp]),
    "cgd_op_plan": (i32, [i32, i32, i32, i32, i32, i32, i32, i32, i32, i32, C.POINTER(i32)]),
    "cgd_op_plan_conv": (i32, [i32] * 10 + [C.POINTER(i32)]),
    "cgd_op_pack_conv3x3_frag": (i32, [vp, vp, vp, i32, i32, i32, vp]),
    "cgd_set_hconv": (i32, [vp, i32, i32]),
    "cgd_op_conv3x3": (i32, [vp, vp, i32, vp, vp, vp, i32, vp, vp, i32, i32, i32, i32, i32, i32, i32, i32, i32, vp]),
    "cgd_op_conv3x3_ex": (i32, [vp, vp, i32, vp, vp, vp, i32, vp, vp, i32, vp, i32, i32, i32, i32, i32, i32, i32, i32, i32, i32, vp, i32, vp, vp]),
    "cgd_op_pack_conv3x3_wino": (i32, [vp, vp, vp, i32, i32, i32, vp]),
    "cgd_op_conv3x3_wino": (i32, [vp, vp, i32, vp, vp, i32, vp, vp, i32, vp, i32, i32, i32, i32, i32, i32, vp]),
    "cgd_set_wino": (i32, [vp, i32, i32]),
    "cgd_op_conv3x3_wino_ex": (i32, [vp, vp, i32, vp, vp, i32, vp, vp, i32, vp, i32, i32, i32, i32, i32, i32, i32, vp, i32, vp, vp]),
    "cgd_op_new_pass": (i32, [vp]),
    "cgd_op_gn_record_merges": (i64, [vp]),
    "cgd_op_gn_records": (i32, [vp, vp, i32, i64, i32, i32, vp, i64, C.POINTER(i32), vp]),
    "cgd_op_gn_stats_offset": (i64, [i32, i32, i32]),
    "cgd_op_wconv_schedule": (i32, [i32, i32, C.POINTER(i32)]),
    "cgd_op_mfma_peak": (i32, [vp, i32, C.POINTER(C.c_double), vp]),
    "cgd_op_conv_in": (i32, [vp, vp, vp, vp, vp, i32, i32, i32, i32, i32, vp]),
    "cgd_op_conv_thin_out": (i32, [vp, vp, i32, vp, vp, vp, i32, i32, i32, i32, i32, vp]),
    "cgd_op_sr_stem": (i32, [vp, vp, vp, i32, i32, i32, vp, vp, vp, i32, i32, i32, i32, i32, vp]),
    "cgd_op_gn_scratch_floats": (i64, [i32, i32, i32]),
    "cgd_op_gn_fwd": (i32, [vp, vp, i32, vp, i32, i32, i32, i32, vp, vp, vp, i32, f32, vp, vp]),
    "cgd_op_gn_bwd": (i32, [vp, vp, i32, vp, i32, vp, i32, vp, i32, i32, i32, i32, i32, vp, vp]),
    "cgd_op_ln_fwd": (i32, [vp, vp, vp, i32, i32, vp, vp, f32, vp, vp]),
    "cgd_op_ln_bwd": (i32, [vp, vp, vp, vp, i32, i32, vp, vp, vp]),
    "cgd_op_pool2x2": (i32, [vp, vp, vp, i32, i32, i32, i32, f32, vp]),
    "cgd_op_upsample2x": (i32, [vp, vp, vp, i32, i32, i32, i32, f32, vp]),
    "cgd_op_act": (i32, [vp, vp, vp, vp, i64, i32, vp]),
    "cgd_op_attn_buf_floats": (i64, [i32, i32, i32, i32, i32]),
    "cgd_op_attn_fwd": (i32, [vp, vp, vp, i32, i32, i32, i32, i32, C.POINTER(vp), vp]),
    "cgd_op_attn_bwd": (i32, [vp, vp, vp, vp, i32, i32, i32, i32, i32, C.POINTER(vp), vp]),
    "cgd_op_attn_fwd_causal": (i32, [vp, vp, vp, i32, i32, i32, i32, C.POINTER(vp), vp]),
    "cgd_op_attn_plan": (i32, [i32, i32, i32, i32, i32, i32, C.POINTER(i32)]),
}

EXPORTED_SYMBOLS = tuple(_SIGS)

_lib = None


def load():
    global _lib
    if _lib is None:
        if not os.path.isfile(LIB_PATH):
            raise RuntimeError(
                f"{LIB_PATH} not found: build it with `python -c 'import __graft_entry__ as g; g.build()'` "
                "(hipcc --offload-arch=gfx950). The MI355X path has no fallback.")
        lib = C.CDLL(LIB_PATH)
        for name, (res, args) in _SIGS.items():
            fn = getattr(lib, name)
            fn.restype = res
            fn.argtypes = args
        _lib = lib
    return _lib


class CgdError(RuntimeError):
    pass


class Context:

    def __init__(self, device=0, precision=None):
        import torch
        self.lib = load()
        if not torch.cuda.is_available():
            raise RuntimeError("cgd_mi355x needs an MI355X (gfx950) GPU visible to PyTorch-ROCm")
        h = vp()
        rc = self.lib.cgd_ctx_create(C.byref(h), int(device))
        if rc != 0:
            raise CgdError(f"cgd_ctx_create failed with status {rc} (is device {device} a gfx950?)")
        self.h = h
        self.device = int(device)
        self._nets = weakref.WeakSet()
        if precision is not None:
            self.set_precision(precision)
        tiles = os.environ.get("CGD_TILES")
        if tiles:
            large, small = (int(v) for v in tiles.split(","))
            self.check(self.lib.cgd_set_tiles(self.h, large, small))
        hg = os.environ.get("CGD_HGEMM")
        if hg:
            self.check(self.lib.cgd_set_hgemm(self.h, *(int(v) for v in hg.split(","))))
        hv = os.environ.get("CGD_HCONV_VAR")
        if hv:
            self.check(self.lib.cgd_set_hconv(self.h, 1 + 16 * int(hv), 256))

    def check(self, rc):
        if rc != 0:
            what = {-1: "HIP runtime error", -2: "invalid argument or state", -3: "NULL handle or pointer", -4: "not a gfx950 device"}.get(rc, "error")
            msg = self.lib.cgd_last_error(self.h).decode() if rc in (-1, -2) else ""
            raise CgdError(f"{what} (status {rc})" + (f": {msg}" if msg else ""))

    def set_precision(self, mode):
        mode = {"f32": 0, "bf16x3": 1, "bf16": 2}.get(mode, mode)
        self.check(self.lib.cgd_set_precision(self.h, int(mode)))

    @property
    def precision(self):
        return self.lib.cgd_get_precision(self.h)

    def stream(self):
        import torch
        return torch.cuda.current_stream(self.device).cuda_stream

    def close(self):
        if getattr(self, "h", None):
            for net in list(self._nets):
                net.close()
            self.lib.cgd_ctx_destroy(self.h)
            self.h = None

    def __del__(self):
        try:
            self.close()
        except Exception:
            pass


def ptr(t):
    if t is None:
        return None
    assert t.is_contiguous(), "cgd_mi355x expects contiguous tensors"
    return t.data_ptr()


def stream_ptr(device=None):
    import torch
    return torch.cuda.current_stream(device).cuda_stream
```

### clip-guided-diffusion_amd/ops.py

```python
import ctypes as C

import torch as th

from . import lib as L

_DEVICE_TYPE = "cuda"


def _s():
    return L.stream_ptr()


def _check(t, name):
    if not isinstance(t, th.Tensor):
        raise ValueError(f"{name}: expected a torch.Tensor, got {type(t).__name__}")
    if t.device.type != _DEVICE_TYPE:
        raise ValueError(f"{name}: expected a GPU tensor, got one on {t.device}")
    if t.dtype != th.float32:
        raise ValueError(f"{name}: expected float32, got {t.dtype}")


def _dense(t, name):
    if t is None:
        return None
    _check(t, name)
    if not t.is_contiguous():
        raise ValueError(f"{name}: expected a contiguous tensor, got shape {tuple(t.shape)} strides {t.stride()}")
    return t.data_ptr()


def _rows(t, name):
    if t is None:
        return None, 0
    _check(t, name)
    if t.dim() == 0:
        raise ValueError(f"{name}: expected at least one dimension")
    shape, strides = tuple(t.shape), t.stride()
    width = shape[-1]
    if width > 1 and strides[-1] != 1:
        raise ValueError(f"{name}: the last dimension must be dense, got strides {strides}")
    lead = [(n, s) for n, s in zip(shape[:-1], strides[:-1]) if n != 1]
    ld = lead[-1][1] if lead else width
    expect = ld
    for n, s in reversed(lead):
        if s != expect:
            raise ValueError(f"{name}: leading dimensions do not collapse to one row stride (shape {shape}, strides {strides})")
        expect *= n
    if lead and ld < width:
        raise ValueError(f"{name}: row stride {ld} is smaller than the row width {width}")
    return t.data_ptr(), ld


def pack_conv3x3(w):
    co, ci = w.shape[:2]
    wf = w.permute(0, 2, 3, 1).reshape(co, 9 * ci).contiguous()
    wd = w.flip(2, 3).permute(1, 2, 3, 0).reshape(ci, 9 * co).contiguous()
    return wf, wd


def gemm(ctx, A, B, bias=None, R=None, alpha=1.0, force_tile=0, splitk=1, out=None):
    M, K = A.shape
    N = B.shape[0]
    pa, lda = _rows(A, "A")
    pb, ldb = _rows(B, "B")
    pbias = _dense(bias, "bias")
    pr, ldr = _rows(R, "R")
    if out is None:
        out = th.empty((M, N), device=A.device, dtype=th.float32)
    pc, ldc = _rows(out, "out")
    ctx.check(ctx.lib.cgd_op_gemm(ctx.h, pa, lda, pb, ldb, pc, ldc, pbias, pr, ldr, M, N, K, float(alpha), force_tile, splitk, _s()))
    return out


def gemm_gn_bwd(ctx, A, W, x, dz, coef, bcoef, add=None, out=None):
    B, HW, K = A.shape
    N = W.shape[0]
    pa, lda = _rows(A, "A")
    pw, ldw = _rows(W, "W")
    px, ldx = _rows(x, "x")
    pdz, lddz = _rows(dz, "dz")
    padd, ldadd = _rows(add, "add")
    pc, pbc = _dense(coef, "coef"), _dense(bcoef, "bcoef")
    if out is None:
        out = th.empty((B, HW, N), device=A.device, dtype=th.float32)
    po, ldo = _rows(out, "out")
    ctx.check(ctx.lib.cgd_op_gemm_gn_bwd(ctx.h, pa, lda, pw, ldw, po, ldo, px, ldx, pdz, lddz, padd, ldadd, pc, pbc, B, HW, N, K, _s()))
    return out


def pack_conv3x3_frag(ctx, w, dgrad=False):
    co, ci = w.shape[:2]
    wc = w.contiguous().float()
    pw = _dense(wc, "w")
    out = th.empty(co * ci * 9, device=w.device, dtype=th.float32)
    ctx.check(ctx.lib.cgd_op_pack_conv3x3_frag(ctx.h, pw, out.data_ptr(), co, ci, int(dgrad), _s()))
    return out


def conv3x3(ctx, x_nhwc, w_packed, bias=None, R=None, upsample_input=False, force_tile=0, splitk=1, w_frag=None):
    Bn, Hs, Ws, Cin = x_nhwc.shape
    H, W = (Hs * 2, Ws * 2) if upsample_input else (Hs, Ws)
    Cout = w_packed.shape[0]
    px, ldx = _rows(x_nhwc, "x")
    pw, pfrag, pbias = _dense(w_packed, "w_packed"), _dense(w_frag, "w_frag"), _dense(bias, "bias")
    pr, ldr = _rows(R, "R")
    y = th.empty((Bn, H, W, Cout), device=x_nhwc.device, dtype=th.float32)
    ctx.check(ctx.lib.cgd_op_conv3x3(ctx.h, px, ldx, pw, pfrag, y.data_ptr(), Cout, pbias, pr, ldr, Bn, H, W, Cin, Cout, int(upsample_input),
                                     force_tile, splitk, _s()))
    return y


def pack_conv3x3_wino(ctx, w, dgrad=False):
    co, ci = w.shape[:2]
    wc = w.contiguous().float()
    pw = _dense(wc, "w")
    out = th.empty(co * ci * 12, device=w.device, dtype=th.float32)
    ctx.check(ctx.lib.cgd_op_pack_conv3x3_wino(ctx.h, pw, out.data_ptr(), co, ci, int(dgrad), _s()))
    return out


def conv3x3_wino(ctx, x_nhwc, w_wino, cout, bias=None, R=None, upsample_input=False, gn_ab=None):
    Bn, Hs, Ws, Cin = x_nhwc.shape
    H, W = (Hs * 2, Ws * 2) if upsample_input else (Hs, Ws)
    px, ldx = _rows(x_nhwc, "x")
    pw, pbias, pab = _dense(w_wino, "w_wino"), _dense(bias, "bias"), _dense(gn_ab, "gn_ab")
    pr, ldr = _rows(R, "R")
    y = th.empty((Bn, H, W, cout), device=x_nhwc.device, dtype=th.float32)
    ctx.check(ctx.lib.cgd_op_conv3x3_wino(ctx.h, px, ldx, pw, y.data_ptr(), cout, pbias, pr, ldr, pab, Bn, H, W, Cin, cout, int(upsample_input),
                                          _s()))
    return y


def conv_in(ctx, x_nchw, w_packed, bias, cout):
    Bn, Cin, H, W = x_nchw.shape
    px, pw, pbias = _dense(x_nchw, "x"), _dense(w_packed, "w_packed"), _dense(bias, "bias")
    y = th.empty((Bn, H, W, cout), device=x_nchw.device, dtype=th.float32)
    ctx.check(ctx.lib.cgd_op_conv_in(ctx.h, px, pw, pbias, y.data_ptr(), Bn, H, W, Cin, cout, _s()))
    return y


def sr_stem(ctx, x_nchw, low, w_packed, bias=None, out=None):
    if x_nchw.dim() != 4 or x_nchw.shape[1] != 3:
        raise ValueError(f"x: expected (B,3,H,W), got {tuple(x_nchw.shape)}")
    Bn, _, H, W = x_nchw.shape
    if low.dim() != 4 or low.shape[1] != 3 or low.shape[0] not in (1, Bn) or 0 in low.shape:
        raise ValueError(f"low: expected (1 or {Bn},3,h,w), got {tuple(low.shape)}")
    if w_packed.dim() != 2 or w_packed.shape[1] != 54:
        raise ValueError(f"w_packed: expected [Cout, 54], got {tuple(w_packed.shape)}")
    cout = w_packed.shape[0]
    px, pl, pw, pbias = _dense(x_nchw, "x"), _dense(low, "low"), _dense(w_packed, "w_packed"), _dense(bias, "bias")
    if out is None:
        out = th.empty((Bn, H, W, cout), device=x_nchw.device, dtype=th.float32)
    elif tuple(out.shape) != (Bn, H, W, cout):
        raise ValueError(f"out: expected {(Bn, H, W, cout)}, got {tuple(out.shape)}")
    po, ldo = _rows(out, "out")
    ctx.check(ctx.lib.cgd_op_sr_stem(ctx.h, px, pl, low.shape[0], low.shape[2], low.shape[3], pw, pbias, po, ldo, Bn, H, W, cout, _s()))
    return out


def conv_thin_out(ctx, x_nhwc, w_packed, bias, cout):
    Bn, H, W, Cin = x_nhwc.shape
    px, ldx = _rows(x_nhwc, "x")
    pw, pbias = _dense(w_packed, "w_packed"), _dense(bias, "bias")
    y = th.empty((Bn, cout, H, W), device=x_nhwc.device, dtype=th.float32)
    ctx.check(ctx.lib.cgd_op_conv_thin_out(ctx.h, px, ldx, pw, pbias, y.data_ptr(), Bn, H, W, Cin, cout, _s()))
    return y


def gn_scratch(ctx, B, HW, C, device):
    n = ctx.lib.cgd_op_gn_scratch_floats(B, HW, C)
    return th.empty(n, device=device, dtype=th.float32)


def groupnorm_fwd(ctx, x, gamma, beta, film=None, act=1, eps=1e-5, scratch=None):
    B, HW, Cc = x.shape
    px, ldx = _rows(x, "x")
    pg, pb, pf = _dense(gamma, "gamma"), _dense(beta, "beta"), _dense(film, "film")
    if scratch is None:
        scratch = gn_scratch(ctx, B, HW, Cc, x.device)
    ps = _dense(scratch, "scratch")
    y = th.empty((B, HW, Cc), device=x.device, dtype=th.float32)
    ctx.check(ctx.lib.cgd_op_gn_fwd(ctx.h, px, ldx, y.data_ptr(), Cc, B, HW, Cc, pg, pb, pf, act, eps, ps, _s()))
    return y, scratch


def groupnorm_bwd(ctx, x, dz, scratch, act=1, add=None):
    B, HW, Cc = x.shape
    px, ldx = _rows(x, "x")
    pdz, lddz = _rows(dz, "dz")
    padd, ldadd = _rows(add, "add")
    ps = _dense(scratch, "scratch")
    dx = th.empty((B, HW, Cc), device=x.device, dtype=th.float32)
    ctx.check(ctx.lib.cgd_op_gn_bwd(ctx.h, px, ldx, pdz, lddz, dx.data_ptr(), Cc, padd, ldadd, B, HW, Cc, act, ps, _s()))
    return dx


def layernorm_fwd(ctx, x, gamma, beta, eps=1e-5):
    rows, Cc = x.shape
    px, pg, pb = _dense(x, "x"), _dense(gamma, "gamma"), _dense(beta, "beta")
    y = th.empty((rows, Cc), device=x.device, dtype=th.float32)
    stats = th.empty((rows, 2), device=x.device, dtype=th.float32)
    ctx.check(ctx.lib.cgd_op_ln_fwd(ctx.h, px, y.data_ptr(), rows, Cc, pg, pb, eps, stats.data_ptr(), _s()))
    return y, stats


def layernorm_bwd(ctx, x, dy, gamma, stats):
    rows, Cc = x.shape
    px, pdy, pg, pst = _dense(x, "x"), _dense(dy, "dy"), _dense(gamma, "gamma"), _dense(stats, "stats")
    dx = th.empty((rows, Cc), device=x.device, dtype=th.float32)
    ctx.check(ctx.lib.cgd_op_ln_bwd(ctx.h, px, pdy, dx.data_ptr(), rows, Cc, pg, pst, _s()))
    return dx


def pool2x2(ctx, x_nhwc, scale=0.25):
    B, H, W, Cc = x_nhwc.shape
    px = _dense(x_nhwc, "x")
    y = th.empty((B, H // 2, W // 2, Cc), device=x_nhwc.device, dtype=th.float32)
    ctx.check(ctx.lib.cgd_op_pool2x2(ctx.h, px, y.data_ptr(), B, H // 2, W // 2, Cc, scale, _s()))
    return y


def upsample2x(ctx, x_nhwc, scale=1.0):
    B, H, W, Cc = x_nhwc.shape
    px = _dense(x_nhwc, "x")
    y = th.empty((B, H * 2, W * 2, Cc), device=x_nhwc.device, dtype=th.float32)
    ctx.check(ctx.lib.cgd_op_upsample2x(ctx.h, px, y.data_ptr(), B, H * 2, W * 2, Cc, scale, _s()))
    return y


def act(ctx, x, kind, dy=None):
    px, pdy = _dense(x, "x"), _dense(dy, "dy")
    if dy is not None and dy.numel() != x.numel():
        raise ValueError(f"dy: {dy.numel()} elements, x has {x.numel()}")
    out = th.empty(x.shape, device=x.device, dtype=th.float32)
    ctx.check(ctx.lib.cgd_op_act(ctx.h, px, pdy, out.data_ptr(), x.numel(), kind, _s()))
    return out


class Attention:

    def __init__(self, ctx, nb, heads, T, d, legacy, device):
        self.ctx, self.nb, self.heads, self.T, self.d, self.legacy = ctx, nb, heads, T, d, int(legacy)
        self.bufs = [th.zeros(ctx.lib.cgd_op_attn_buf_floats(nb, heads, T, d, w), device=device, dtype=th.float32) for w in range(5)]
        self._arr = (C.c_void_p * 5)(*[b.data_ptr() for b in self.bufs])

    def forward(self, qkv):
        Cc = self.heads * self.d
        pq = _dense(qkv, "qkv")
        out = th.empty((self.nb * self.T, Cc), device=qkv.device, dtype=th.float32)
        self.ctx.check(self.ctx.lib.cgd_op_attn_fwd(self.ctx.h, pq, out.data_ptr(), self.nb, self.heads, self.T, self.d,
                                                    self.legacy, self._arr, _s()))
        return out

    def forward_causal(self, qkv):
        if self.legacy:
            raise ValueError("causal attention takes the [Q all heads | K | V] row layout (legacy=0)")
        Cc = self.heads * self.d
        pq = _dense(qkv, "qkv")
        out = th.empty((self.nb * self.T, Cc), device=qkv.device, dtype=th.float32)
        self.ctx.check(self.ctx.lib.cgd_op_attn_fwd_causal(self.ctx.h, pq, out.data_ptr(), self.nb, self.heads, self.T, self.d,
                                                           self._arr, _s()))
        return out

    def backward(self, qkv, dout):
# ... 6 lines not shown
```

### include/cgd_mi355x.h

```cpp
#ifndef CGD_MI355X_H
#define CGD_MI355X_H
#include <stdint.h>

#ifdef __cplusplus
extern "C" {
#endif

typedef struct cgd_ctx cgd_ctx;
typedef struct cgd_unet cgd_unet;
typedef struct cgd_vit cgd_vit;

enum { CGD_F32 = 0, CGD_BF16X3 = 1, CGD_BF16 = 2 };

int cgd_ctx_create(cgd_ctx** out, int device);
void cgd_ctx_destroy(cgd_ctx* ctx);
const char* cgd_last_error(cgd_ctx* ctx);
int cgd_set_precision(cgd_ctx* ctx, int mode);
int cgd_get_precision(cgd_ctx* ctx);
int64_t cgd_ctx_device_allocs(cgd_ctx* ctx);
const char* cgd_version(void);
int cgd_set_tiles(cgd_ctx* ctx, int large_tile, int small_tile);
int cgd_set_hgemm(cgd_ctx* ctx, int mode, int min_m, int min_chunks);
int cgd_profile(cgd_ctx* ctx, int enable);
int cgd_profile_read(cgd_ctx* ctx, double* out18);
// ... 138 lines not shown
                           int W, void* stream);
int cgd_classifier_dgrad(cgd_classifier* c, float scale, float* g_x, int accumulate, void* stream);
int64_t cgd_op_attnpool_scratch_floats(int B, int S, int C, int d, int out);
int cgd_op_attnpool_fwd(cgd_ctx* ctx, const float* h, const float* pos, const float* qkv_w, const float* qkv_b, const float* c_w, const float* c_b,
                        const int64_t* y, float* pooled, float* logits, float* logp, float* scratch, int B, int S, int C, int d, int out,
                        void* stream);
int cgd_op_attnpool_bwd(cgd_ctx* ctx, const float* qkv_w, const float* qkv_b, const float* c_w, const float* c_b, float scale, float* dh,
                        float* scratch, int B, int S, int C, int d, int out, void* stream);

int cgd_cutouts_fwd(cgd_ctx* ctx, const float* x_in, const int32_t* coords, float* out, int B, int H, int W, int cutn, int cut_size,
                    int layout, int patch, void* stream);
int cgd_cutouts_bwd(cgd_ctx* ctx, const float* d_out, const int32_t* coords, float* g_in, int B, int H, int W, int cutn,
                    int cut_size, int layout, int patch, int accumulate, void* stream);

int cgd_cutouts_aug_fwd(cgd_ctx* ctx, const float* x_in, const int32_t* coords, const float* params, const float* noise,
                        const int64_t* noise_off, float* out, int B, int H, int W, int cutn, int cut_size, int layout, int patch,
                        void* stream);
int cgd_cutouts_aug_bwd(cgd_ctx* ctx, const float* d_out, const int32_t* coords, const float* params, float* g_in, float* scratch, int B,
                        int H, int W, int cutn, int cut_size, int layout, int patch, int accumulate, void* stream);
int64_t cgd_cutouts_aug_scratch_floats(int B, int H, int W, int cutn);
int cgd_op_aug_sample_map(const float* params, int h, int w, int32_t* affine_src, int32_t* persp_idx, float* persp_w);

int cgd_cutouts_resize_fwd(cgd_ctx* ctx, const float* x_in, const int32_t* coords, const int32_t* flags, float* out, int B, int H, int W,
                           int cutn, int cut_size, int layout, int patch, void* stream);
int cgd_cutouts_resize_bwd(cgd_ctx* ctx, const float* d_out, const int32_t* coords, const int32_t* flags, float* g_in, float* scratch, int B,
                           int H, int W, int cutn, int cut_size, int layout, int patch, int accumulate, void* stream);
int64_t cgd_cutouts_resize_scratch_floats(int B, int H, int W, int cutn);
int cgd_cutouts_resize_weights(int n, int m, float* w, int32_t* left, int* taps);

int cgd_spherical_loss(cgd_ctx* ctx, const float* emb, const float* targets_n, const float* weights, float* d_emb, float* loss_part,
                       int cutn, int B, int P, int D, float clip_guidance_scale, void* stream);

int cgd_directional_loss(cgd_ctx* ctx, const float* emb, const float* src_emb, const float* dirs_n, const float* weights, float* d_emb,
                         float* loss_part, int cutn, int B, int Bs, int P, int D, float clip_guidance_scale, int accumulate, void* stream);

int cgd_spherical_loss_regions(cgd_ctx* ctx, const float* emb, const float* targets_n, const float* weights, float* d_emb, float* loss_part,
                               int cutn, int B, int P, int D, float clip_guidance_scale, const int32_t* sat, const int32_t* region_of,
                               const int32_t* region_of_host, const float* power, const int32_t* geo, int R, int H, int W, void* stream);
int cgd_directional_loss_regions(cgd_ctx* ctx, const float* emb, const float* src_emb, const float* dirs_n, const float* weights, float* d_emb,
                                 float* loss_part, int cutn, int B, int Bs, int P, int D, float clip_guidance_scale, int accumulate,
                                 const int32_t* sat, const int32_t* region_of, const int32_t* region_of_host, const float* power,
                                 const int32_t* geo, int R, int H, int W, void* stream);
int cgd_op_region_coverage(cgd_ctx* ctx, const int32_t* sat, const int32_t* region_of, const int32_t* region_of_host, const float* power,
                           const int32_t* geo, float* out, int cutn, int P, int R, int H, int W, void* stream);

typedef struct cgd_step_coef {
  float sqrt_recip;
  float sqrt_recipm1;
  float coef1, coef2;
  float min_log, max_log;
  float fac;
  float sqrt_one_minus_ab;
  float sqrt_ab_prev;
  float sqrt_one_minus_ab_prev;
  int nonzero;
} cgd_step_coef;

int cgd_pmv_blend(cgd_ctx* ctx, const float* x, const float* model_out6, float* pred_xstart, float* mean, float* log_variance,
                  float* x_in, int B, int H, int W, const cgd_step_coef* k, void* stream);
int cgd_guidance_part_blocks(int B, int H, int W);
int cgd_guidance_combine(cgd_ctx* ctx, const float* g_clip_in, const float* x_in, const float* pred_xstart, float* g_direct,
                         float* seed6, float* loss_part, int B, int H, int W, const cgd_step_coef* k, float tv_scale,
                         float range_scale, float sat_scale, void* stream);
int cgd_grad_finish(cgd_ctx* ctx, const float* g_direct, const float* g_unet, float* g, float* g_part, int B, int H, int W,
                    void* stream);
int cgd_scalars(cgd_ctx* ctx, const float* clip_part, int n_clip, const float* loss_part, const float* g_part, int B, int H, int W,
                int use_magnitude, float* scalars, void* stream);
int cgd_sample_update(cgd_ctx* ctx, const float* x, const float* pred_xstart, const float* mean, const float* log_variance,
                      const float* g, const float* noise, const float* scalars, float* sample, float* pred_xstart_out, int B, int H,
                      int W, const cgd_step_coef* k, int mode, void* stream);

typedef struct cgd_multistep {
  int phase;
  int order;
  float sigma;
  float dir;
} cgd_multistep;
int cgd_multistep_update(cgd_ctx* ctx, const float* x, const float* x_eval, const float* pred_xstart, const float* g,
                         const float* scalars, const float* noise, const float* const eps_hist[3], float* eps_out, float* sample,
                         float* pred_xstart_out, int B, int H, int W, const cgd_step_coef* k, const cgd_step_coef* k_step,
                         const cgd_multistep* m, void* stream);

typedef struct cgd_dpmpp {
  float c_x;
  float c_d;
  float c_r;
  float c_n;
} cgd_dpmpp;
int cgd_dpmpp_update(cgd_ctx* ctx, const float* x, const float* pred_xstart, const float* g, const float* scalars, const float* noise,
                     const float* x0_hist, float* x0c_out, float* sample, float* pred_xstart_out, int B, int H, int W,
                     const cgd_step_coef* k, const cgd_dpmpp* d, void* stream);

int64_t cgd_abs_quantile_scratch_bytes(int B, int64_t n);
int cgd_abs_quantile_slice(void);
int cgd_op_abs_quantile(cgd_ctx* ctx, const float* v, int B, int64_t n, int64_t k, float frac, float floor, float cap, float* out3,
                        void* scratch, void* stream);
int cgd_dpmpp_threshold(cgd_ctx* ctx, const float* x, const float* pred_xstart, const float* g, const float* scalars, float* x0c, int B,
                        int H, int W, const cgd_step_coef* k_coef, int64_t k, float frac, float floor, float cap, float* thr3, void* scratch,
                        void* stream);
int cgd_dpmpp_update_thr(cgd_ctx* ctx, const float* x, const float* pred_xstart, const float* x0c, const float* thr3, const float* noise,
                         const float* x0_hist, float* x0c_out, float* sample, float* pred_xstart_out, int B, int H, int W,
                         const cgd_step_coef* k_coef, const cgd_dpmpp* d, void* stream);

enum { CGD_MASK_PRED_XSTART = 1, CGD_MASK_N_KNOWN = 2, CGD_MASK_RENOISE = 4 };
typedef struct cgd_mask_coef {
  float sqrt_ab_prev;
  float sqrt_one_minus_ab_prev;
  float renoise_x;
  float renoise_n;
  int flags;
} cgd_mask_coef;
int cgd_masked_merge(cgd_ctx* ctx, float* sample, float* pred_xstart, const float* init, const float* mask, const float* n_known,
                     const float* n_re, float* x_re, int B, int H, int W, int init_batch, int mask_batch, int mask_channels,
                     const cgd_mask_coef* k, void* stream);

long cgd_ilvr_scratch_floats(int B, int H, int W, int factor, int with_pred_xstart);
int cgd_ilvr_refine(cgd_ctx* ctx, float* sample, float* pred_xstart, const float* ref, const float* noise, float* scratch, int B, int H,
                    int W, int ref_batch, int factor, float sa, float sb, void* stream);

int cgd_window_gather(cgd_ctx* ctx, const float* full, float* win, const int* oy, int ny, const int* ox, int nx, const float* ay, const float* ax,
                      int B, int C, int H, int W, int S, int wrap, void* stream);
int cgd_window_merge(cgd_ctx* ctx, const float* win, float* full, const int* oy, int ny, const int* ox, int nx, const float* ay, const float* ax,
                     int B, int C, int H, int W, int S, int wrap, int accumulate, void* stream);

typedef struct cgd_reverse_coef {
  float sqrt_recip;
  float sqrt_recipm1;
  float sqrt_ab_next;
  float sqrt_one_minus_ab_next;
  float inv_sqrt_one_minus_ab_next;
} cgd_reverse_coef;
int cgd_ddim_reverse_update(cgd_ctx* ctx, const float* x, const float* model_out6, const float* init, float* x_next, float* pred_xstart,
                            float* noise_out, int B, int H, int W, int init_batch, const cgd_reverse_coef* k, void* stream);

int cgd_op_gemm(cgd_ctx* ctx, const float* A, int lda, const float* B, int ldb, float* C, int ldc, const float* bias, const float* R,
                int ldr, int M, int N, int K, float alpha, int force_tile, int splitk, void* stream);
int cgd_op_gram(cgd_ctx* ctx, const float* A, int lda, int B, int N, int C, float scale, float* G_out , void* stream);
int cgd_op_gemm_gn_bwd(cgd_ctx* ctx, const float* A, int lda, const float* W, int ldw, float* dx, int lddx, const float* x, int ldx,
                       const float* dz, int lddz, const float* add, int ldadd, const float* coef, const float* bcoef, int B, int HW, int N, int K,
                       void* stream);
int cgd_op_gemm_gn_bwd_accepts(int precision, int lda, int ldw, int lddx, int ldx, int lddz, int ldadd, int x_misalign, int B, int HW, int N, int K);
int cgd_op_pack_conv3x3_frag(cgd_ctx* ctx, const float* w_torch, float* out , int Co, int Ci, int dgrad,
                             void* stream);
int cgd_op_plan(int conv, int M, int N, int K, int H, int W, int Cin, int weight, int precision, int num_cu, int* out4);
int cgd_op_plan_conv(int Bn, int H, int W, int Cin, int Cout, int precision, int num_cu, int hconv_var, int stats, int gnb, int* out5);
int cgd_set_hconv(cgd_ctx* ctx, int mode, int min_m);
int cgd_op_conv3x3(cgd_ctx* ctx, const float* x_nhwc, int ldx, const float* w_packed, const float* w_frag, float* y_nhwc, int ldy,
                   const float* bias, const float* R, int ldr, int Bn, int H, int W, int Cin, int Cout, int upsample_input, int force_tile,
                   int splitk, void* stream);
int cgd_op_conv3x3_ex(cgd_ctx* ctx, const float* x_nhwc, int ldx, const float* w_packed, const float* w_frag, float* y_nhwc, int ldy,
                      const float* bias, const float* R, int ldr, const float* gn_ab, int Bn, int H, int W, int Cin, int Cout,
                      int upsample_input, int force_tile, int splitk, int defer, int stats, const float* gnb_x, int gnb_ldx,
                      const float* gnb_scratch, void* stream);
int cgd_op_pack_conv3x3_wino(cgd_ctx* ctx, const float* w_torch, float* out, int Co, int Ci, int dgrad, void* stream);
int cgd_op_conv3x3_wino(cgd_ctx* ctx, const float* x_nhwc, int ldx, const float* w_wino, float* y_nhwc, int ldy, const float* bias,
                        const float* R, int ldr, const float* gn_ab, int Bn, int H, int W, int Cin, int Cout, int upsample_input,
                        void* stream);
int cgd_set_wino(cgd_ctx* ctx, int mode, int min_m);
int cgd_op_conv3x3_wino_ex(cgd_ctx* ctx, const float* x_nhwc, int ldx, const float* w_wino, float* y_nhwc, int ldy, const float* bias,
                           const float* R, int ldr, const float* gn_ab, int Bn, int H, int W, int Cin, int Cout, int upsample_input,
                           int stats, const float* gnb_x, int gnb_ldx, const float* gnb_scratch, void* stream);
int cgd_op_new_pass(cgd_ctx* ctx);
int64_t cgd_op_gn_record_merges(cgd_ctx* ctx);
int cgd_op_gn_records(cgd_ctx* ctx, const float* y, int ldy, int64_t rows, int C, int kind, float* out, int64_t cap, int* pixels, void* stream);
int64_t cgd_op_gn_stats_offset(int B, int HW, int C);
int cgd_op_wconv_schedule(int nb, int q, int* out7);
int cgd_op_mfma_peak(cgd_ctx* ctx, int iters, double* flop_out, void* stream);
int cgd_op_conv_in(cgd_ctx* ctx, const float* x_nchw, const float* w, const float* bias, float* y_nhwc, int Bn, int H, int W, int Cin,
                   int Cout, void* stream);
int cgd_op_conv_thin_out(cgd_ctx* ctx, const float* x_nhwc, int ldx, const float* w, const float* bias, float* y_nchw, int Bn, int H,
                         int W, int Cin, int Cout, void* stream);
int cgd_op_sr_stem(cgd_ctx* ctx, const float* x, const float* low, int B_low, int h, int w, const float* wpacked, const float* bias, float* y,
                   int ldy, int B, int H, int W, int Cout, void* stream);
int64_t cgd_op_gn_scratch_floats(int B, int HW, int C);
int cgd_op_gn_fwd(cgd_ctx* ctx, const float* x, int ldx, float* y, int ldy, int B, int HW, int C, const float* gamma,
                  const float* beta, const float* film, int act, float eps, float* scratch, void* stream);
int cgd_op_gn_bwd(cgd_ctx* ctx, const float* x, int ldx, const float* dz, int lddz, float* dx, int lddx, const float* add, int ldadd,
                  int B, int HW, int C, int act, float* scratch, void* stream);
int cgd_op_ln_fwd(cgd_ctx* ctx, const float* x, float* y, int rows, int C, const float* gamma, const float* beta, float eps,
                  float* stats, void* stream);
int cgd_op_ln_bwd(cgd_ctx* ctx, const float* x, const float* dy, float* dx, int rows, int C, const float* gamma, const float* stats,
                  void* stream);
int cgd_op_pool2x2(cgd_ctx* ctx, const float* in, float* out, int B, int Ho, int Wo, int C, float scale, void* stream);
int cgd_op_upsample2x(cgd_ctx* ctx, const float* in, float* out, int B, int Ho, int Wo, int C, float scale, void* stream);
int cgd_op_act(cgd_ctx* ctx, const float* x, const float* dy, float* out, int64_t n, int act, void* stream);
int64_t cgd_op_attn_buf_floats(int nb, int heads, int T, int d, int which);
int cgd_op_attn_fwd(cgd_ctx* ctx, const float* qkv, float* out, int nb, int heads, int T, int d, int legacy, float* bufs[5],
                    void* stream);
int cgd_op_attn_bwd(cgd_ctx* ctx, const float* qkv, const float* dout, float* dqkv, int nb, int heads, int T, int d, int legacy,
                    float* bufs[5], void* stream);
int cgd_op_attn_fwd_causal(cgd_ctx* ctx, const float* qkv, float* out, int nb, int heads, int T, int d, float* bufs[5], void* stream);
int cgd_op_attn_plan(int T, int d, int ldq, int ldo, int precision, int attn_flash, int* out2);

#ifdef __cplusplus
}
#endif
#endif
```

Baseline: 57.94 diffusion steps/sec.

## Add sub-pixel phase decomposition for nearest-upsample 3x3 convs in forward and dgrad

Result: no change. 58.35 diffusion steps/sec (median of 6 runs) (+0.7%).

```diff
diff --git a/clip-guided-diffusion_amd/csrc/capi.hip b/clip-guided-diffusion_amd/csrc/capi.hip
--- a/clip-guided-diffusion_amd/csrc/capi.hip
+++ b/clip-guided-diffusion_amd/csrc/capi.hip
@@ -42,6 +42,7 @@
   if (const char* e = getenv("CGD_FUSE_GN")) sscanf(e, "%d,%d,%d,%d", &ctx->fuse_gn, &ctx->fuse_gn_max_m, &ctx->fuse_gn_min_m, &ctx->fuse_gn_skip_m);
   if (const char* e = getenv("CGD_FUSE_ACT")) ctx->fuse_act = atoi(e);
   if (const char* e = getenv("CGD_HCONV_W8")) ctx->hconv_w8 = atoi(e);
+  if (const char* e = getenv("CGD_UPCONV_PHASE")) sscanf(e, "%d,%d,%d", &ctx->upconv_phase, &ctx->upconv_phase_min_m, &ctx->upconv_phase_min_m_bwd);
   if (const char* e = getenv("CGD_ATTN_X3")) ctx->attn_x3 = atoi(e);
   if (const char* e = getenv("CGD_ATTN_FLASH")) ctx->attn_flash = atoi(e);
   int wino_env_mode = -1;
@@ -543,6 +544,42 @@
   }
   return cgd_launch_gemm(ctx, p, S(stream));
 }
+int cgd_set_upconv_phase(cgd_ctx* ctx, int bits, int min_m_fwd, int min_m_bwd) {
+  CGD_NEED_CTX(ctx);
+  if (bits < 0 || bits > 7) CGD_FAIL(ctx, "cgd_set_upconv_phase: bits must be 0 .. 7");
+  ctx->upconv_phase = bits;
+  if (min_m_fwd > 0) ctx->upconv_phase_min_m = min_m_fwd;
+  if (min_m_bwd > 0) ctx->upconv_phase_min_m_bwd = min_m_bwd;
+  return 0;
+}
+int64_t cgd_op_phase_packed_floats(int Co, int Ci) { return (int64_t)cgd_hconv_phase_packed_floats(Co, Ci); }
+int cgd_op_pack_conv3x3_phase(cgd_ctx* ctx, const float* w, float* out, int Co, int Ci, int dgrad, void* stream) {
+  CGD_NEED_CTX(ctx);
+  return cgd_pack_conv3x3_phase(ctx, w, out, Co, Ci, dgrad, S(stream));
+}
+int cgd_op_upconv_phase(cgd_ctx* ctx, const float* x, int ldx, const float* w_phase, float* y, int ldy, const float* bias, const float* gn_ab, int Bn,
+                        int H, int W, int Cin, int Cout, int dgrad, int defer, int stats, void* stream) {
+  CGD_NEED_CTX(ctx);
+  GemmParams p;
+  p.A = x; p.lda = ldx; p.C = y; p.ldc = ldy; p.bias = bias; p.gn_ab = gn_ab;
+  p.M = Bn * H * W; p.N = Cout; p.conv = 1; p.H = H; p.W = W; p.Cin = Cin; p.defer = defer; p.stats = stats;
+  return cgd_launch_upconv_phase(ctx, p, w_phase, dgrad, S(stream));
+}
+int cgd_op_plan_upconv(int Bn, int H, int W, int Cin, int Cout, int precision, int num_cu, int bits, int dgrad, int* out2) {
+  if (!out2) return -3;
+  cgd_ctx ctx;
+  ctx.precision = precision;
+  if (num_cu > 0) ctx.num_cu = num_cu;
+  if (bits >= 0) ctx.upconv_phase = bits;
+  ctx.ws_bytes = (size_t)256 << 20;
+  GemmParams p;
+  float* const dummy = (float*)(uintptr_t)4096;
+  p.A = dummy; p.C = dummy;
+  p.M = Bn * H * W; p.N = Cout; p.lda = Cin; p.ldc = Cout; p.conv = 1; p.H = H; p.W = W; p.Cin = Cin;
+  out2[0] = cgd_upconv_phase_plan(&ctx, p, dummy, dgrad) ? 1 : 0;
+  out2[1] = out2[0] ? (int)cgd_upconv_phase_tiles(p) : 0;
+  return 0;
+}
 int cgd_op_conv_in(cgd_ctx* ctx, const float* x, const float* w, const float* bias, float* y, int Bn, int H, int W, int Cin, int Cout,
                    void* stream) {
   CGD_NEED_CTX(ctx);
diff --git a/clip-guided-diffusion_amd/csrc/common.h b/clip-guided-diffusion_amd/csrc/common.h
--- a/clip-guided-diffusion_amd/csrc/common.h
+++ b/clip-guided-diffusion_amd/csrc/common.h
@@ -79,6 +79,8 @@
   int hconv_slots = 0, hconv_min_chunks = 4;
   int hconv_w8 = 0;
   int hconv_mode = 1, hconv_min_m = 256;
+  int upconv_phase = 3;
+  int upconv_phase_min_m = 4096, upconv_phase_min_m_bwd = 4096;
   int embed_fuse = 1;
   int gemv_mode = 1;
   int thin_direct = 1;
@@ -236,6 +238,11 @@
 int cgd_hconv_tile_m(const cgd_ctx* ctx, const GemmParams& p);
 long cgd_hconv_tiles_m(const cgd_ctx* ctx, const GemmParams& p);
 int cgd_launch_hconv(cgd_ctx* ctx, const GemmParams& p, hipStream_t s);
+size_t cgd_hconv_phase_packed_floats(int Co, int Ci);
+int cgd_pack_conv3x3_phase(cgd_ctx* ctx, const float* w , float* out, int Co, int Ci, int dgrad, hipStream_t s);
+bool cgd_upconv_phase_plan(const cgd_ctx* ctx, const GemmParams& p, const void* Bph, int dgrad);
+long cgd_upconv_phase_tiles(const GemmParams& p);
+int cgd_launch_upconv_phase(cgd_ctx* ctx, GemmParams p, const void* Bph, int dgrad, hipStream_t s);
 
 size_t cgd_wconv_packed_floats(int Co, int Ci);
 int cgd_pack_conv3x3_wino(cgd_ctx* ctx, const float* w , float* out, int Co, int Ci, int dgrad, hipStream_t s);
diff --git a/clip-guided-diffusion_amd/csrc/hconv.hip b/clip-guided-diffusion_amd/csrc/hconv.hip
--- a/clip-guided-diffusion_amd/csrc/hconv.hip
+++ b/clip-guided-diffusion_amd/csrc/hconv.hip
@@ -29,7 +29,7 @@
 constexpr int NPASS2 = 6;
 
 
-template <int MODE, int TH, int NJ, bool GN>
+template <int MODE, int TH, int NJ, bool GN, int PH = 0>
 __global__ __launch_bounds__(TH == 4 ? 256 : TH * 32) void hconv2_kernel(const float* __restrict__ Ag, const uint4* __restrict__ Bg, float* Cg,
                                                          const float* __restrict__ biasg, const float* Rg, float* __restrict__ wsg,
                                                          const float* __restrict__ gng, const HConvParams p) {
@@ -40,7 +40,9 @@
   constexpr int NT = TH == 4 ? 256 : TH * 32;
   constexpr int RPP = NT / 8;
   constexpr int NPASS = TH == 4 ? 4 : NPASS2;
+  constexpr int NTAP = PH ? 4 : 9, NK = 2 * NTAP;
   static_assert(TH != 4 || NJ == 1, "the 4-row tile runs 64 pixels x 32 channels per wavefront");
+  static_assert(PH == 0 || (TH == 4 && MODE == 1), "the phase convs run on the unsplit tile in bf16x3");
   static_assert(NPASS * RPP >= NP2, "staging passes must cover the patch");
   __shared__ __attribute__((aligned(16))) __bf16 lds[2 * NPL * PLANE];
   const int tid = threadIdx.x, lane = tid & 63, wave = tid >> 6;
@@ -59,8 +61,10 @@
   const int img = mt / tpi, trem = mt - img * tpi;
   const int y0 = (trem / tpr) * TH, x0 = (trem % tpr) << 4;
   const int HW = p.H * p.W;
-  const int Hs = p.ups ? (p.H >> 1) : p.H, Ws = p.ups ? (p.W >> 1) : p.W;
-  const float* __restrict__ Aimg = Ag + (long)img * Hs * Ws * p.lda;
+  const int Hs = PH == 2 ? 2 * p.H : p.ups ? (p.H >> 1) : p.H, Ws = PH == 2 ? 2 * p.W : p.ups ? (p.W >> 1) : p.W;
+  const int ph_y = PH ? (int)(blockIdx.z >> 1) : 0, ph_x = PH ? (int)(blockIdx.z & 1) : 0;
+  const int gph = PH == 1 ? ph_y * HRS + ph_x * HPH : PH == 2 ? (1 - ph_y) * HRS + (1 - ph_x) * HPH : 0;
+  const float* __restrict__ Aimg = Ag + (long)img * Hs * Ws * p.lda + (PH == 2 ? (ph_y * Ws + ph_x) * p.lda : 0);
 
   const int c4 = tid & 7;
   int poff[NPASS], soff[NPASS];
@@ -74,7 +78,10 @@
       soff[j] = py * HRS + px * HPH + c4 * 4;
       int yy = y0 + py - 1, xx = x0 + px - 1;
       const bool inb = (unsigned)yy < (unsigned)p.H && (unsigned)xx < (unsigned)p.W;
-      if (p.ups) {
+      if (PH == 2) {
+        yy <<= 1;
+        xx <<= 1;
+      } else if (p.ups) {
         yy >>= 1;
         xx >>= 1;
       }
@@ -90,8 +97,11 @@
   for (int i = 0; i < NI; ++i) {
     const int pix = wm * (NI * 32) + i * 32 + l31;
     const int ty = pix >> 4, tx = pix & 15;
-    fro[i] = ty * HRS + tx * HPH + hh * 8;
-    mrow[i] = x0 + tx < p.W ? (long)img * HW + (long)(y0 + ty) * p.W + x0 + tx : -1L;
+    fro[i] = ty * HRS + tx * HPH + hh * 8 + gph;
+    if constexpr (PH == 1)
+      mrow[i] = x0 + tx < p.W ? (long)img * 4 * HW + (long)(2 * (y0 + ty) + ph_y) * (2 * p.W) + 2 * (x0 + tx) + ph_x : -1L;
+    else
+      mrow[i] = x0 + tx < p.W ? (long)img * HW + (long)(y0 + ty) * p.W + x0 + tx : -1L;
   }
 
   const int nchunk = p.Cin >> 5;
@@ -103,11 +113,11 @@
   }
   const int nb0 = (n0 >> 5) + wn * NJ;
   const int nbN = p.N >> 5;
-  const long bstride_nb = (long)nchunk * 9 * 4 * 64;
+  const long bstride_nb = (long)nchunk * NTAP * 4 * 64;
   const int nbc = nb0 < nbN ? nb0 : nbN - 1;
   (void)nbc;
   const int nb0_s = (n0 >> 5) + __builtin_amdgcn_readfirstlane(wn) * NJ;
-  const uint4* __restrict__ Bwb = Bg + (long)(nb0_s < nbN ? nb0_s : nbN - 1) * bstride_nb;
+  const uint4* __restrict__ Bwb = Bg + ((PH ? (long)blockIdx.z * nbN : 0L) + (nb0_s < nbN ? nb0_s : nbN - 1)) * bstride_nb;
   const int bj1_b = (nb0_s + 1 < nbN) ? (int)(bstride_nb * 16) : 0;
   (void)bj1_b;
 
@@ -157,7 +167,7 @@
   }
 #define A_LOAD2(DST, SRCB, TAP, KS)                                                          \
   {                                                                                          \
-    constexpr int o_ = ((TAP) / 3) * HRS + ((TAP) % 3) * HPH + (KS) * 16;                    \
+    constexpr int o_ = PH ? ((TAP) >> 1) * HRS + ((TAP) & 1) * HPH + (KS) * 16 : ((TAP) / 3) * HRS + ((TAP) % 3) * HPH + (KS) * 16; \
     _Pragma("unroll") for (int i = 0; i < NI; ++i) {                                         \
       DST[i][0] = *(const cgd_bf16x8*)&(SRCB)[fro[i] + o_];                                  \
       if constexpr (MODE == 1) DST[i][1] = *(const cgd_bf16x8*)&(SRCB)[PLANE + fro[i] + o_]; \
@@ -165,7 +175,7 @@
   }
 #define B_LOAD2(DST, BASE, WANT, TAP, KS)                                                                                                         \
   {                                                                                                                                               \
-    const int so_ = ((BASE) * (9 * 4 * 64) + ((TAP) * 4 + (KS) * 2) * 64) * 16;                                                                   \
+    const int so_ = ((BASE) * (NTAP * 4 * 64) + ((TAP) * 4 + (KS) * 2) * 64) * 16;                                                                \
     DST[0][0] = __builtin_bit_cast(uint4, cgd_buf_load16_if(Bwb, 0xffffffffu, (WANT), lane * 16, so_));                                           \
     if constexpr (MODE == 1) DST[0][1] = __builtin_bit_cast(uint4, cgd_buf_load16_if(Bwb, 0xffffffffu, (WANT), lane * 16 + 1024, so_));           \
     if constexpr (NJ == 2) {                                                                                                                      \
@@ -185,7 +195,9 @@
         acc[i][j] = __builtin_amdgcn_mfma_f32_32x32x16_bf16(__builtin_bit_cast(cgd_bf16x8, BQ[j][0]), AQ[i][0], acc[i][j], 0, 0, 0);   \
   }
 
-  constexpr int RING = TH == 4 ? 9 : (TH == 8 || NJ == 1) ? 6 : 3, DIST = RING - 1;
+  constexpr int RING = PH ? 8 : TH == 4 ? 9 : (TH == 8 || NJ == 1) ? 6 : 3, DIST = RING - 1;
+  constexpr int PS0 = PH ? 4 : 6;
+  static_assert(NK % RING == 0 && PS0 + NPASS <= NK, "the ring and the patch conversion must fit a chunk's k-steps");
   cgd_bf16x8 af[2][NI][NPL];
   uint4 bq[RING][NJ][NPL];
   if (c0 < c1) {
@@ -204,8 +216,8 @@
     (void)more;
     A_LOAD2(af[0], cur, 0, 0);
 #pragma unroll
-    for (int q = 0; q < 18; ++q) {
-      if (q + 1 < 18) {
+    for (int q = 0; q < NK; ++q) {
+      if (q + 1 < NK) {
         switch (q + 1) {
 #define CASE_A(Q) case Q: A_LOAD2(af[(Q) & 1], cur, (Q) >> 1, (Q) & 1); break;
           CASE_A(1) CASE_A(2) CASE_A(3) CASE_A(4) CASE_A(5) CASE_A(6) CASE_A(7) CASE_A(8) CASE_A(9)
@@ -214,12 +226,12 @@
         }
       }
       {
-        const int q2 = (q + DIST) % 18;
-        if (q + DIST < 18) { B_LOAD2(bq[(q + DIST) % RING], c, -1, q2 >> 1, q2 & 1); }
+        const int q2 = (q + DIST) % NK;
+        if (q + DIST < NK) { B_LOAD2(bq[(q + DIST) % RING], c, -1, q2 >> 1, q2 & 1); }
         else { B_LOAD2(bq[(q + DIST) % RING], c + 1, want, q2 >> 1, q2 & 1); }
       }
       MFMA12(af[q & 1], bq[q % RING]);
-      if (q >= 6 && q < 6 + NPASS) PATCH_STORE2(nxt, q - 6, q - 5);
+      if (q >= PS0 && q < PS0 + NPASS) PATCH_STORE2(nxt, q - PS0, q - PS0 + 1);
 #pragma unroll
       for (int r = 0; r < (TH == 4 ? 6 : 12); ++r) {
         __builtin_amdgcn_sched_group_barrier(0x008, 1, 0);
@@ -247,7 +259,7 @@
 #undef B_LOAD2
 #undef MFMA12
 
-  if (p.splitk > 1) {
+  if (PH == 2 || p.splitk > 1) {
     float* __restrict__ ws = wsg + (long)blockIdx.z * p.M * p.N;
 #pragma unroll
     for (int i = 0; i < NI; ++i)
@@ -303,7 +315,8 @@
             s2[e] += __shfl_xor(s2[e], off, 64);
           }
         if (l31 == 0) {
-          float* so = p.stat + ((long)mt * p.N + cb0 + 8 * g + 4 * hh) * 2;
+          const long rec = PH == 1 ? ((long)img * 4 + blockIdx.z) * tpi + trem : (long)mt;
+          float* so = p.stat + (rec * p.N + cb0 + 8 * g + 4 * hh) * 2;
           const cgd_f32x4 mean = kk + s1 * (1.f / 64.f), m2 = s2 - s1 * s1 * (1.f / 64.f);
           *(cgd_f32x4*)so = cgd_f32x4{mean[0], m2[0], mean[1], m2[1]};
           *(cgd_f32x4*)(so + 4) = cgd_f32x4{mean[2], m2[2], mean[3], m2[3]};
@@ -397,9 +410,52 @@
   }
 }
 
+__global__ __launch_bounds__(256) void pack_phase_kernel(const float* __restrict__ w, __bf16* __restrict__ out, int Co, int Ci, int dgrad) {
+  const int N = dgrad ? Ci : Co, K = dgrad ? Co : Ci;
+  const int nchunk = K >> 5, nbN = N >> 5;
+  const long total = (long)N * K * 16;
+  for (long t = (long)blockIdx.x * blockDim.x + threadIdx.x; t < total; t += (long)gridDim.x * blockDim.x) {
+    const int e = (int)(t & 7);
+    long u = t >> 3;
+    const int lane = (int)(u & 63);
+    u >>= 6;
+    const int ks = (int)(u & 1);
+    u >>= 1;
+    const int tap = (int)(u & 3);
+    u >>= 2;
+    const int chunk = (int)(u % nchunk);
+    u /= nchunk;
+    const int nb = (int)(u % nbN), ph = (int)(u / nbN);
+    const int n = nb * 32 + (lane & 31), k = chunk * 32 + ks * 16 + (lane >> 5) * 8 + e;
+    const int py = ph >> 1, px = ph & 1;
+    const int a = dgrad ? 1 - (tap >> 1) : tap >> 1, b = dgrad ? 1 - (tap & 1) : tap & 1;
+    const int ky0 = a ? (py ? 2 : 1) : 0, ky1 = a ? 2 : (py ? 1 : 0);
+    const int kx0 = b ? (px ? 2 : 1) : 0, kx1 = b ? 2 : (px ? 1 : 0);
+    const float* wk = dgrad ? w + ((long)k * Ci + n) * 9 : w + ((long)n * Ci + k) * 9;
+    double sum = 0.0;
+    for (int ky = ky0; ky <= ky1; ++ky)
+      for (int kx = kx0; kx <= kx1; ++kx) sum += (double)wk[ky * 3 + kx];
+    const float v = (float)sum;
+    const __bf16 hi = (__bf16)v;
+    const __bf16 lo = (__bf16)(v - (float)hi);
+    const long blk = (((((long)ph * nbN + nb) * nchunk + chunk) * 4 + tap) * 2 + ks) * 2;
+    out[(blk + 0) * 512 + lane * 8 + e] = hi;
+    out[(blk + 1) * 512 + lane * 8 + e] = lo;
+  }
+}
+
 }
 
 size_t cgd_hconv_packed_floats(int Co, int Ci) { return (size_t)Co * Ci * 9; }
+size_t cgd_hconv_phase_packed_floats(int Co, int Ci) { return (size_t)Co * Ci * 16; }
+
+int cgd_pack_conv3x3_phase(cgd_ctx* ctx, const float* w, float* out, int Co, int Ci, int dgrad, hipStream_t s) {
+  if ((Co & 31) || (Ci & 31)) CGD_FAIL(ctx, "pack_conv3x3_phase: channels must be multiples of 32");
+  const long total = (long)Co * Ci * 16;
+  CGD_LAUNCH(pack_phase_kernel, dim3((int)std::min<long>(cdiv(total, 256), 4096)), dim3(256), 0, s, w, (__bf16*)out, Co, Ci, dgrad);
+  CGD_HIP(ctx, hipGetLastError());
+  return 0;
+}
 
 int cgd_pack_conv3x3_frag(cgd_ctx* ctx, const float* w, float* out, int Co, int Ci, int dgrad, hipStream_t s) {
   if ((Co & 31) || (Ci & 31)) CGD_FAIL(ctx, "pack_conv3x3_frag: channels must be multiples of 32");
@@ -489,3 +545,59 @@
 #undef HC2_LAUNCH
   return 0;
 }
+
+static bool upconv_phase_capable(const cgd_ctx* ctx, const GemmParams& p, const void* Bph, int dgrad) {
+  if (!p.conv || !Bph || ctx->precision != CGD_PREC_BF16X3 || p.nbatch != 1 || p.R || p.splitk > 1) return false;
+  if (p.H <= 0 || p.W <= 0 || (p.H & 7) || (p.W & 31) || p.M <= 0 || p.M % (p.H * p.W)) return false;
+  if ((p.Cin & 31) || (p.N & 127) || (p.lda & 3) || (p.ldc & 3) || ((uintptr_t)p.A & 15) || ((uintptr_t)p.C & 15)) return false;
+  if (p.bias && ((uintptr_t)p.bias & 3)) return false;
+  if ((long)p.H * p.W * p.lda * 4 >= (1L << 31)) return false;
+  if (dgrad && (p.bias || p.gn_ab || (size_t)p.M * p.N * sizeof(float) > ctx->ws_bytes)) return false;
+  return true;
+}
+
+long cgd_upconv_phase_tiles(const GemmParams& p) { return (long)(p.M / (p.H * p.W)) * (p.H / 8) * (p.W / 32) * (p.N >> 7) * 4; }
+
+bool cgd_upconv_phase_plan(const cgd_ctx* ctx, const GemmParams& p, const void* Bph, int dgrad) {
+  if (!(ctx->upconv_phase & (dgrad ? 2 : 1)) || !ctx->hconv_mode || ctx->hconv_var != 0) return false;
+  if (!upconv_phase_capable(ctx, p, Bph, dgrad)) return false;
+  if (ctx->upconv_phase & 4) return true;
+  return cgd_upconv_phase_tiles(p) >= ctx->num_cu && p.M >= (dgrad ? ctx->upconv_phase_min_m_bwd : ctx->upconv_phase_min_m);
+}
+
+int cgd_launch_upconv_phase(cgd_ctx* ctx, GemmParams g, const void* Bph, int dgrad, hipStream_t s) {
+  if (!upconv_phase_capable(ctx, g, Bph, dgrad)) CGD_FAIL(ctx, "cgd_launch_upconv_phase: the phase conv kernel does not support this problem");
+  const int Ml = g.M / 4, Hl = g.H / 2, Wl = g.W / 2;
+  CGD_TRY(cgd_flush_pending(ctx, s));
+  cgd_chanstats_invalidate(ctx, g.C, dgrad ? Ml : g.M, g.ldc, g.N);
+  HConvParams p;
+  p.A = g.A; p.Bp = (const uint4*)Bph; p.C = g.C; p.bias = g.bias; p.R = nullptr; p.ws = ctx->ws;
+  p.lda = g.lda; p.ldc = g.ldc; p.ldr = 0;
+  p.M = Ml; p.N = g.N; p.H = Hl; p.W = Wl; p.Cin = g.Cin; p.ups = 0; p.splitk = 1; p.alpha = g.alpha;
+  p.gn = g.gn_ab;
+  p.stat = p.bstat = nullptr; p.bx = nullptr; p.bcoef = nullptr; p.ldbx = 0; p.bact = 0;
+  p.nmajor = (ctx->tile_order == 1 || (ctx->tile_order == 0 && 9L * g.N >= Ml)) ? 1 : 0;
+  if (!dgrad && g.stats && (ctx->gn_epi & 1) && cgd_gn_merges_records(g.H * g.W))
+    p.stat = cgd_chanstats_register(ctx, g.C, g.ldc, g.N, g.M, s, 0, 64);
+  ProfRec pr;
+  CGD_TRY(cgd_prof_begin(ctx, &pr, CGD_PROF_HCONV, 2.0 * g.M * g.N * 9.0 * g.Cin, s));
+  const dim3 grid((int)(cgd_upconv_phase_tiles(g) / 4), 1, 4);
+  if (dgrad)
+    CGD_LAUNCH((hconv2_kernel<1, 4, 1, false, 2>), grid, dim3(256), 0, s, p.A, p.Bp, p.C, p.bias, p.R, p.ws, p.gn, p);
+  else if (p.gn)
+    CGD_LAUNCH((hconv2_kernel<1, 4, 1, true, 1>), grid, dim3(256), 0, s, p.A, p.Bp, p.C, p.bias, p.R, p.ws, p.gn, p);
+  else
+    CGD_LAUNCH((hconv2_kernel<1, 4, 1, false, 1>), grid, dim3(256), 0, s, p.A, p.Bp, p.C, p.bias, p.R, p.ws, p.gn, p);
+  CGD_TRY(cgd_prof_stamp(ctx, &pr, s));
+  if (dgrad) {
+    PendingReduce& q = ctx->pending;
+    q.valid = true;
+    q.src = SplitSrc();
+    q.src.ws = ctx->ws; q.src.stride = (long)Ml * g.N; q.src.n = 4; q.src.N = g.N; q.src.alpha = g.alpha;
+    q.C = g.C; q.ldc = g.ldc; q.M = Ml; q.stream = s;
+    if (!(g.defer && ctx->defer_mode)) CGD_TRY(cgd_flush_pending(ctx, s));
+  }
+  cgd_prof_push(ctx, &pr);
+  CGD_HIP(ctx, hipGetLastError());
+  return 0;
+}
diff --git a/clip-guided-diffusion_amd/csrc/unet.hip b/clip-guided-diffusion_amd/csrc/unet.hip
--- a/clip-guided-diffusion_amd/csrc/unet.hip
+++ b/clip-guided-diffusion_amd/csrc/unet.hip
@@ -53,6 +53,8 @@
   float *cw1wp = 0, *cw1wd = 0, *cw2wp = 0, *cw2wd = 0;
   int wino_prec = CGD_PREC_BF16X3;
   bool wino_ready = false;
+  float *cw1pf = 0, *cw1pd = 0;
+  bool phase_ready = false;
   int B = 0, H = 0, W = 0, Ho = 0, Wo = 0;
   TV x;
   TV add_skip;
@@ -76,6 +78,7 @@
 
 struct UNet : NetBase {
   int ensure_wino(ResBlock* rb, long pixels, hipStream_t s);
+  int ensure_phase(ResBlock* rb, hipStream_t s);
   cgd_unet_config cfg;
   bool encoder_only = false;
   int ted = 0, ch0 = 0, ch_last = 0;
@@ -131,6 +134,17 @@
   return 0;
 }
 
+int UNet::ensure_phase(ResBlock* rb, hipStream_t s) {
+  if (rb->phase_ready) return 0;
+  const size_t n = cgd_hconv_phase_packed_floats(rb->cout, rb->cin);
+  if (!rb->cw1pf) CGD_TRY(alloc(&rb->cw1pf, n));
+  if (!rb->cw1pd) CGD_TRY(alloc(&rb->cw1pd, n));
+  CGD_TRY(cgd_pack_conv3x3_phase(ctx, P(rb->pre + ".in_layers.2.weight"), rb->cw1pf, rb->cout, rb->cin, 0, s));
+  CGD_TRY(cgd_pack_conv3x3_phase(ctx, P(rb->pre + ".in_layers.2.weight"), rb->cw1pd, rb->cout, rb->cin, 1, s));
+  rb->phase_ready = true;
+  return 0;
+}
+
 int ResBlock::fwd(UNet& u, TV xin, int Bn, int& Hh, int& Ww, TV* o, hipStream_t s) {
   cgd_ctx* ctx = u.ctx;
   B = Bn; H = Hh; W = Ww;
@@ -152,6 +166,8 @@
   c1.stats = 1;
   c1.A = x.p; c1.lda = x.ld;
   const bool fuse1 = !down && cgd_conv_uses_hconv(ctx, c1);
+  const bool phase1 = up && fuse1 && cgd_upconv_phase_plan(ctx, c1, cw1f, 0);
+  if (phase1) CGD_TRY(u.ensure_phase(this, s));
   const float* skip_src = x.p;
   int skip_ld = x.ld;
   if (fuse1) {
@@ -175,7 +191,11 @@
     skip_src = xr.p;
     skip_ld = cin;
   }
-  CGD_TRY(cgd_launch_gemm(ctx, c1, s));
+  if (phase1) {
+    CGD_TRY(cgd_launch_upconv_phase(ctx, c1, cw1pf, 0, s));
+  } else {
+    CGD_TRY(cgd_launch_gemm(ctx, c1, s));
+  }
   GemmParams c2;
   c2.A = h2.p; c2.lda = cout; c2.B = cw2f; c2.Bpk = cw2fp; c2.Bwk = wino_ready ? cw2wp : nullptr; c2.bwk_prec = wino_prec; c2.ldb = 9 * cout; c2.C = outp; c2.ldc = ldo; c2.bias = cb2;
   c2.M = (int)npo; c2.N = cout; c2.conv = 1; c2.H = Ho; c2.W = Wo; c2.Cin = cout;
@@ -215,7 +235,7 @@
   const long npi = (long)B * H * W, npo = (long)B * Ho * Wo;
   CGD_TRY(u.ensure(d3, npo * cout));
   CGD_TRY(u.ensure(d2, npo * cout));
-  CGD_TRY(u.ensure(d1, npo * cin));
+  if (!up) CGD_TRY(u.ensure(d1, npo * cin));
   CGD_TRY(u.ensure(dx, npi * cin));
   GemmParams c2;
   c2.A = dout.p; c2.lda = dout.ld; c2.B = cw2d; c2.Bpk = cw2dp; c2.Bwk = wino_ready ? cw2wd : nullptr; c2.bwk_prec = wino_prec; c2.ldb = 9 * cout; c2.C = d3.p; c2.ldc = cout;
@@ -251,6 +271,21 @@
   c1.A = d2.p; c1.lda = cout; c1.B = cw1d; c1.Bpk = cw1dp; c1.Bwk = wino_ready ? cw1wd : nullptr; c1.bwk_prec = wino_prec; c1.ldb = 9 * cout; c1.C = d1.p; c1.ldc = cin;
   c1.M = (int)npo; c1.N = cin; c1.conv = 1; c1.H = Ho; c1.W = Wo; c1.Cin = cout;
   c1.defer = (up || down) ? 0 : 1;
+  if (up && cgd_upconv_phase_plan(ctx, c1, cw1d, 1)) {
+    CGD_TRY(u.ensure_phase(this, s));
+    CGD_TRY(u.ensure(d1f, npi * cin));
+    CGD_TRY(cgd_launch_pool2x2(ctx, dout.p, dout.ld, dx.p, cin, nullptr, 0, B, H, W, cin, 1.f, s));
+    c1.C = d1f.p;
+    c1.defer = 1;
+    CGD_TRY(cgd_launch_upconv_phase(ctx, c1, cw1pd, 1, s));
+    CGD_TRY(cgd_launch_gn_bwd(ctx, x.p, x.ld, d1f.p, cin, dx.p, cin, add, ldadd, B, H * W, cin, 1, s1.p, s, add_skip.p, add_skip.ld));
+    *din = TV{dx.p, cin, cin};
+    return 0;
+  }
+  if (up) {
+    CGD_TRY(u.ensure(d1, npo * cin));
+    c1.C = d1.p;
+  }
   if (!up && !down) {
     c1.gnb_x = x.p; c1.gnb_ldx = x.ld; c1.gnb_coef = cgd_gn_coef(s1.p, B, H * W, cin); c1.gnb_act = 1;
   }
@@ -493,6 +528,7 @@
     CGD_TRY(cgd_pack_conv3x3_frag(ctx, P(p + ".out_layers.3.weight"), rb->cw2fp, rb->cout, rb->cout, 0, s));
     CGD_TRY(cgd_pack_conv3x3_frag(ctx, P(p + ".out_layers.3.weight"), rb->cw2dp, rb->cout, rb->cout, 1, s));
     rb->wino_ready = false;
+    rb->phase_ready = false;
     CGD_TRY(cgd_pack_conv3x3(ctx, P(p + ".in_layers.2.weight"), rb->cw1f, rb->cw1d, rb->cout, rb->cin, s));
     CGD_TRY(cgd_pack_conv3x3(ctx, P(p + ".out_layers.3.weight"), rb->cw2f, rb->cw2d, rb->cout, rb->cout, s));
     if (rb->skip_conv) {
diff --git a/clip-guided-diffusion_amd/lib.py b/clip-guided-diffusion_amd/lib.py
--- a/clip-guided-diffusion_amd/lib.py
+++ b/clip-guided-diffusion_amd/lib.py
@@ -208,6 +208,11 @@
     "cgd_op_plan_conv": (i32, [i32] * 10 + [C.POINTER(i32)]),
     "cgd_op_pack_conv3x3_frag": (i32, [vp, vp, vp, i32, i32, i32, vp]),
     "cgd_set_hconv": (i32, [vp, i32, i32]),
+    "cgd_op_phase_packed_floats": (i64, [i32, i32]),
+    "cgd_op_pack_conv3x3_phase": (i32, [vp, vp, vp, i32, i32, i32, vp]),
+    "cgd_op_upconv_phase": (i32, [vp, vp, i32, vp, vp, i32, vp, vp, i32, i32, i32, i32, i32, i32, i32, i32, vp]),
+    "cgd_set_upconv_phase": (i32, [vp, i32, i32, i32]),
+    "cgd_op_plan_upconv": (i32, [i32] * 9 + [C.POINTER(i32)]),
     "cgd_op_conv3x3": (i32, [vp, vp, i32, vp, vp, vp, i32, vp, vp, i32, i32, i32, i32, i32, i32, i32, i32, i32, vp]),
     "cgd_op_conv3x3_ex": (i32, [vp, vp, i32, vp, vp, vp, i32, vp, vp, i32, vp, i32, i32, i32, i32, i32, i32, i32, i32, i32, i32, vp, i32, vp, vp]),
     "cgd_op_pack_conv3x3_wino": (i32, [vp, vp, vp, i32, i32, i32, vp]),
diff --git a/clip-guided-diffusion_amd/ops.py b/clip-guided-diffusion_amd/ops.py
--- a/clip-guided-diffusion_amd/ops.py
+++ b/clip-guided-diffusion_amd/ops.py
@@ -110,6 +110,26 @@
     return y
 
 
+def pack_conv3x3_phase(ctx, w, dgrad=False):
+    co, ci = w.shape[:2]
+    pw = _dense(w.contiguous().float(), "w")
+    out = th.empty(int(ctx.lib.cgd_op_phase_packed_floats(co, ci)), device=w.device, dtype=th.float32)
+    ctx.check(ctx.lib.cgd_op_pack_conv3x3_phase(ctx.h, pw, out.data_ptr(), co, ci, int(dgrad), _s()))
+    return out
+
+
+def upconv_phase(ctx, x_nhwc, w_phase, cout, bias=None, gn_ab=None, dgrad=False, defer=False, stats=False, out=None):
+    Bn, Hs, Ws, Cin = x_nhwc.shape
+    H, W = (Hs, Ws) if dgrad else (2 * Hs, 2 * Ws)
+    px, ldx = _rows(x_nhwc, "x")
+    pw, pbias, pab = _dense(w_phase, "w_phase"), _dense(bias, "bias"), _dense(gn_ab, "gn_ab")
+    if out is None:
+        out = th.empty((Bn, H // 2, W // 2, cout) if dgrad else (Bn, H, W, cout), device=x_nhwc.device, dtype=th.float32)
+    py, ldy = _rows(out, "out")
+    ctx.check(ctx.lib.cgd_op_upconv_phase(ctx.h, px, ldx, pw, py, ldy, pbias, pab, Bn, H, W, Cin, cout, int(dgrad), int(defer), int(stats), _s()))
+    return out
+
+
 def pack_conv3x3_wino(ctx, w, dgrad=False):
     co, ci = w.shape[:2]
     wc = w.contiguous().float()
diff --git a/include/cgd_mi355x.h b/include/cgd_mi355x.h
--- a/include/cgd_mi355x.h
+++ b/include/cgd_mi355x.h
@@ -314,6 +314,12 @@
                       const float* bias, const float* R, int ldr, const float* gn_ab, int Bn, int H, int W, int Cin, int Cout,
                       int upsample_input, int force_tile, int splitk, int defer, int stats, const float* gnb_x, int gnb_ldx,
                       const float* gnb_scratch, void* stream);
+int64_t cgd_op_phase_packed_floats(int Co, int Ci);
+int cgd_op_pack_conv3x3_phase(cgd_ctx* ctx, const float* w_torch, float* out, int Co, int Ci, int dgrad, void* stream);
+int cgd_op_upconv_phase(cgd_ctx* ctx, const float* x_nhwc, int ldx, const float* w_phase, float* y_nhwc, int ldy, const float* bias,
+                        const float* gn_ab, int Bn, int H, int W, int Cin, int Cout, int dgrad, int defer, int stats, void* stream);
+int cgd_set_upconv_phase(cgd_ctx* ctx, int bits, int min_m_fwd, int min_m_bwd);
+int cgd_op_plan_upconv(int Bn, int H, int W, int Cin, int Cout, int precision, int num_cu, int bits, int dgrad, int* out2);
 int cgd_op_pack_conv3x3_wino(cgd_ctx* ctx, const float* w_torch, float* out, int Co, int Ci, int dgrad, void* stream);
 int cgd_op_conv3x3_wino(cgd_ctx* ctx, const float* x_nhwc, int ldx, const float* w_wino, float* y_nhwc, int ldy, const float* bias,
                         const float* R, int ldr, const float* gn_ab, int Bn, int H, int W, int Cin, int Cout, int upsample_input,
```
